# denyingmxd/CFPNet

Measured on AMD Instinct MI355X. Metric: depth maps/sec @ 480x640 bf16 (whole job; per_gpu = value / n_gpus); abs_rel vs CPU oracle, higher is better.
Workload: dtype bf16; 1 GPU; batch=8 480x640 RGB + 8x8-zone ToF, eval forward incl. the prob output [B,256,H/2,W/2] written in the storage dtype (bf16: 2 bytes/element); layers=hist2image combine1 image x2 (CFPNet), parallelism=single GPU

## Files before the change

cfpnet_amd/csrc/attention.hip:

```cpp
#include "common.h"

namespace {

struct KvP {
  const void* k; const void* v;
  float* kv; float* ksum; float* ws;
  int k_ld, v_ld;
  int NB, Hk, Wk, th, tw, gy, gx;
  int cy0, cy1, cx0, cx1;
  int count_pad, heads, d, nsplit;
  float inv_len;
  const int* rec;
};

template <int D> struct KvCfg;
template <> struct KvCfg<4>  { static constexpr int IC = 1; };
template <> struct KvCfg<8>  { static constexpr int IC = 2; };
template <> struct KvCfg<16> { static constexpr int IC = 2; };
template <> struct KvCfg<32> { static constexpr int IC = 2; };

template <typename T, int D, bool DEV>
__global__ __launch_bounds__(64) void kv_reduce_kernel(KvP p) {
  constexpr int IC = KvCfg<D>::IC;
  constexpr int TPK = D / IC;
  constexpr int KL = 64 / TPK;
  const T* __restrict__ K = reinterpret_cast<const T*>(p.k);
  const T* __restrict__ V = reinterpret_cast<const T*>(p.v);
  const int g = blockIdx.x, h = blockIdx.y, sp = blockIdx.z;
  const int lane = threadIdx.x;
  const int ip = lane % TPK, kl = lane / TPK;

  const int gpb = p.gy * p.gx;
  const int b = g / gpb, gi = g % gpb;
  const int ty = gi / p.gx, tx = gi % p.gx;
  int cy0 = p.cy0, cy1 = p.cy1, cx0 = p.cx0, cx1 = p.cx1;
  float inv_len = p.inv_len;
  if constexpr (DEV) {
    const int* __restrict__ rec = p.rec;
    cy0 = rec[4]; cy1 = rec[5]; cx0 = rec[6]; cx1 = rec[7];
    inv_len = 1.0f / (float)max(rec[8], 1);
  }
  const int y0 = max(max(ty * p.th, cy0), 0), y1 = min(min((ty + 1) * p.th, cy1), p.Hk);
  const int x0 = max(max(tx * p.tw, cx0), 0), x1 = min(min((tx + 1) * p.tw, cx1), p.Wk);
  const int rh = max(y1 - y0, 0), rw = max(x1 - x0, 0);
  const int S = rh * rw;
  const int per = (S + p.nsplit - 1) / p.nsplit;
  const int s_begin = sp * per, s_end = min(S, s_begin + per);

  float acc[IC][D];
  float ks[IC];
#pragma unroll
  for (int i = 0; i < IC; ++i) {
    ks[i] = 0.f;
#pragma unroll
    for (int j = 0; j < D; ++j) acc[i][j] = 0.f;
  }
  constexpr int KU = 4;
  const int rwd = max(rw, 1);
  const int step_q = KL / rwd, step_r = KL - step_q * rwd;
  const int s_first = min(s_begin + kl, max(s_end - 1, 0));
  int cy = s_first / rwd, cx = s_first - cy * rwd;
  const int ly = max(s_end - 1, 0) / rwd, lx = max(s_end - 1, 0) - ly * rwd;
  for (int s0 = s_begin + kl; s0 < s_end; s0 += KL * KU) {
    float kf[KU][IC], vf[KU][D];
#pragma unroll
    for (int u = 0; u < KU; ++u) {
      const bool in = s0 + u * KL < s_end;
      const int yy = y0 + (in ? cy : ly), xx = x0 + (in ? cx : lx);
      cx += step_r; cy += step_q;
      if (cx >= rwd) { cx -= rwd; ++cy; }
      const long long row = ((long long)b * p.Hk + yy) * p.Wk + xx;
      const T* kp = K + row * p.k_ld + h * D + ip * IC;
      const T* vp = V + row * p.v_ld + h * D;
#pragma unroll
      for (int i = 0; i < IC; ++i) kf[u][i] = to_f32<T>(kp[i]);
#pragma unroll
      for (int j = 0; j < D; ++j) vf[u][j] = to_f32<T>(vp[j]);
    }
#pragma unroll
    for (int u = 0; u < KU; ++u) {
      if (s0 + u * KL >= s_end) continue;
#pragma unroll
      for (int j = 0; j < D; ++j) vf[u][j] *= inv_len;
#pragma unroll
      for (int i = 0; i < IC; ++i) {
        const float kk = elu1(kf[u][i]);
        ks[i] += kk;
#pragma unroll
        for (int j = 0; j < D; ++j) acc[i][j] = fmaf(kk, vf[u][j], acc[i][j]);
      }
    }
  }
#pragma unroll
  for (int o = TPK; o < 64; o <<= 1) {
#pragma unroll
    for (int i = 0; i < IC; ++i) {
      ks[i] += __shfl_xor(ks[i], o, 64);
#pragma unroll
      for (int j = 0; j < D; ++j) acc[i][j] += __shfl_xor(acc[i][j], o, 64);
    }
  }
  if (kl == 0) {
    float padk = 0.f;
    if (p.count_pad && sp == 0) padk = (float)(p.th * p.tw - S);
    float* dkv; float* dks;
    if (p.nsplit == 1) {
      dkv = p.kv + ((long long)g * p.heads + h) * D * D;
      dks = p.ksum + ((long long)g * p.heads + h) * D;
    } else {
      float* base = p.ws + (((long long)g * p.heads + h) * p.nsplit + sp) * (D * D + D);
      dkv = base; dks = base + D * D;
    }
#pragma unroll
    for (int i = 0; i < IC; ++i) {
      dks[ip * IC + i] = ks[i] + padk;
#pragma unroll
      for (int j = 0; j < D; ++j) dkv[(ip * IC + i) * D + j] = acc[i][j];
    }
  }
}

__global__ __launch_bounds__(256) void kv_finalize_kernel(const float* __restrict__ ws, float* __restrict__ kv,
                                                          float* __restrict__ ksum, int nsplit, int d, long long items) {
  const int per = d * d + d;
  for (long long i = (long long)blockIdx.x * 256 + threadIdx.x; i < items * per; i += (long long)gridDim.x * 256) {
    const long long gh = (long long)((unsigned long long)i / (unsigned)per);
    const int e = (int)(i - gh * per);
    const float* base = ws + gh * nsplit * per + e;
    float s = 0.f;
    int j = 0;
    for (; j + 7 < nsplit; j += 8) {
      float t[8];
#pragma unroll
      for (int u = 0; u < 8; ++u) t[u] = base[(long long)(j + u) * per];
#pragma unroll
      for (int u = 0; u < 8; ++u) s += t[u];
    }
    for (; j < nsplit; ++j) s += base[(long long)j * per];
    if (e < d * d) kv[gh * d * d + e] = s; else ksum[gh * d + (e - d * d)] = s;
  }
}

struct ApP {
  const void* q; const float* kv; const float* ksum; void* out;
  int q_ld, out_ld, NB, Hq, Wq, qth, qtw, ggy, ggx;
  int ey0, ey1, ex0, ex1, heads;
  float v_length, eps;
  FastDiv fheads, fwq, fhq, fqth, fqtw;
  const int* rec;
};

template <typename T, int D, int JS, bool DEV>
__global__ __launch_bounds__(256) void attn_apply_kernel(ApP p) {
  constexpr int DJ = D / JS;
  const T* __restrict__ Q = reinterpret_cast<const T*>(p.q);
  T* __restrict__ O = reinterpret_cast<T*>(p.out);
  int ey0 = p.ey0, ey1 = p.ey1, ex0 = p.ex0, ex1 = p.ex1;
  float v_length = p.v_length;
  if constexpr (DEV) {
    const int* __restrict__ rec = p.rec;
    ey0 = rec[4]; ey1 = rec[5]; ex0 = rec[6]; ex1 = rec[7];
    v_length = (float)max(rec[8], 1);
  }
  const unsigned total = (unsigned)p.NB * p.Hq * p.Wq * p.heads * JS;
  for (unsigned i0 = blockIdx.x * 256u + threadIdx.x; i0 < total; i0 += gridDim.x * 256u) {
    const unsigned i = i0 / JS;
    const int js = (int)(i0 - i * JS);
    unsigned toku, hu, tu, xu, bu, yu;
    fd_rowcol(i, p.fheads, toku, hu);
    fd_rowcol(toku, p.fwq, tu, xu);
    fd_rowcol(tu, p.fhq, bu, yu);
    const int h = (int)hu, x = (int)xu, y = (int)yu, b = (int)bu;
    const long long tok = toku;
    T* op = O + tok * p.out_ld + h * D + js * DJ;
    float o[DJ];
    if (y >= ey0 && y < ey1 && x >= ex0 && x < ex1) {
#pragma unroll
      for (int j = 0; j < DJ; ++j) o[j] = 0.f;
    } else {
      const long long g = ((long long)b * p.ggy + fd_div((unsigned)y, p.fqth)) * p.ggx + fd_div((unsigned)x, p.fqtw);
      const float* kv = p.kv + (g * p.heads + h) * D * D + js * DJ;
      const float* ks = p.ksum + (g * p.heads + h) * D;
      const T* qp = Q + tok * p.q_ld + h * D;
      float z = 0.f;
#pragma unroll
      for (int j = 0; j < DJ; ++j) o[j] = 0.f;
#pragma unroll
      for (int ii = 0; ii < D; ++ii) {
        const float qv = elu1(to_f32<T>(qp[ii]));
        z = fmaf(qv, ks[ii], z);
#pragma unroll
        for (int j = 0; j < DJ; ++j) o[j] = fmaf(qv, kv[ii * D + j], o[j]);
      }
      const float zi = 1.f / (z + p.eps);
#pragma unroll
      for (int j = 0; j < DJ; ++j) o[j] = o[j] * zi * v_length;
    }
#pragma unroll
    for (int j = 0; j < DJ; ++j) op[j] = from_f32<T>(o[j]);
  }
}

int g_ap_split_below = 65536;
int g_kv_target_waves = 2048;
int pick_nsplit(int S, long long groups_heads) {
  long long want = (g_kv_target_waves + groups_heads - 1) / groups_heads;
  int by_keys = (S + 63) / 64;
  long long n = want < by_keys ? want : by_keys;
  if (n < 1) n = 1;
  if (n > 64) n = 64;
  return (int)n;
}

}

void cfp_attn_debug_set(int value) { g_kv_target_waves = value; }
void cfp_attn_apply_debug_set(int value) { g_ap_split_below = value; }

extern "C" size_t cfp_attn_kv_ws_floats(int NB, int Hk, int Wk, int th, int tw, int heads, int d) {
  if (NB <= 0 || Hk <= 0 || Wk <= 0 || th <= 0 || tw <= 0 || heads <= 0 || d <= 0) return 0;
  long long groups = (long long)NB * cdiv(Hk, th) * cdiv(Wk, tw);
  int S = (th < Hk ? th : Hk) * (tw < Wk ? tw : Wk);
  int ns = pick_nsplit(S, groups * heads);
  return (size_t)(groups * heads * ns * (d * d + d));
}

static int kv_reduce_impl(const void* k, int k_ld, const void* v, int v_ld, float* kv, float* ksum, float* ws,
                          int NB, int Hk, int Wk, int th, int tw, int cy0, int cy1, int cx0, int cx1,
                          int count_pad, float v_length, const int* rec, int heads, int d, int dtype, cfp_stream_t stream, const char* who) {
  CFP_REQUIRE(dtype_ok(dtype), CFP_EINVAL, std::string(who) + ": bad dtype");
  CFP_REQUIRE(k && v && kv && ksum, CFP_EINVAL, std::string(who) + ": null pointer");
  CFP_REQUIRE(NB > 0 && Hk > 0 && Wk > 0 && th > 0 && tw > 0 && heads > 0 && (d == 4 || d == 8 || d == 16 || d == 32) &&
                  k_ld >= heads * d && v_ld >= heads * d && v_length > 0.f,
              CFP_ESHAPE, std::string(who) + ": bad shape (head dim must be 4, 8, 16 or 32)");
  KvP p;
  p.rec = rec;
  p.k = k; p.v = v; p.kv = kv; p.ksum = ksum; p.ws = ws; p.k_ld = k_ld; p.v_ld = v_ld;
  p.NB = NB; p.Hk = Hk; p.Wk = Wk; p.th = th; p.tw = tw; p.gy = cdiv(Hk, th); p.gx = cdiv(Wk, tw);
  p.cy0 = cy0; p.cy1 = cy1; p.cx0 = cx0; p.cx1 = cx1; p.count_pad = count_pad; p.heads = heads; p.d = d;
  p.inv_len = 1.0f / v_length;
  long long groups = (long long)NB * p.gy * p.gx;
  int S = (th < Hk ? th : Hk) * (tw < Wk ? tw : Wk);
  p.nsplit = pick_nsplit(S, groups * heads);
  CFP_REQUIRE(p.nsplit == 1 || ws, CFP_EINVAL, std::string(who) + ": workspace required");
  CFP_REQUIRE(groups < (1ll << 31) && heads <= 65535, CFP_ESHAPE, std::string(who) + ": grid too large");
  hipStream_t s = reinterpret_cast<hipStream_t>(stream);
  dim3 grid((unsigned)groups, heads, p.nsplit);
#define KV_LAUNCH(T, D) do { if (rec) hipLaunchKernelGGL((kv_reduce_kernel<T, D, true>), grid, dim3(64), 0, s, p); \
                             else hipLaunchKernelGGL((kv_reduce_kernel<T, D, false>), grid, dim3(64), 0, s, p); } while (0)
#define KV_SWITCH(T) switch (d) { case 4: KV_LAUNCH(T, 4); break; case 8: KV_LAUNCH(T, 8); break; \
                                  case 16: KV_LAUNCH(T, 16); break; default: KV_LAUNCH(T, 32); break; }
  if (dtype == CFP_BF16) { KV_SWITCH(bf16_t) } else if (dtype == CFP_F16) { KV_SWITCH(f16_t) } else { KV_SWITCH(float) }
#undef KV_SWITCH
#undef KV_LAUNCH
  if (p.nsplit > 1) {
    long long items = groups * heads;
    long long total = items * (d * d + d);
    int blocks = (int)((total + 255) / 256 > 4096 ? 4096 : (total + 255) / 256);
    hipLaunchKernelGGL(kv_finalize_kernel, dim3(blocks), dim3(256), 0, s, ws, kv, ksum, p.nsplit, d, items);
  }
  return cfp_check_launch(who);
}

extern "C" int cfp_attn_kv_reduce(const void* k, int k_ld, const void* v, int v_ld, float* kv, float* ksum, float* ws,
                                  int NB, int Hk, int Wk, int th, int tw, int cy0, int cy1, int cx0, int cx1,
                                  int count_pad, float v_length, int heads, int d, int dtype, cfp_stream_t stream) {
  return kv_reduce_impl(k, k_ld, v, v_ld, kv, ksum, ws, NB, Hk, Wk, th, tw, cy0, cy1, cx0, cx1, count_pad, v_length, nullptr, heads, d, dtype,
                        stream, "cfp_attn_kv_reduce");
}

extern "C" int cfp_attn_kv_reduce_dev(const void* k, int k_ld, const void* v, int v_ld, float* kv, float* ksum, float* ws,
                                      int NB, int Hk, int Wk, int th, int tw, const int* rec, int count_pad, int heads, int d, int dtype,
                                      cfp_stream_t stream) {
  CFP_REQUIRE(rec && (reinterpret_cast<uintptr_t>(rec) & 3) == 0, CFP_EINVAL, "cfp_attn_kv_reduce_dev: bad record pointer");
  return kv_reduce_impl(k, k_ld, v, v_ld, kv, ksum, ws, NB, Hk, Wk, th, tw, 0, 0, 0, 0, count_pad, 1.f, rec, heads, d, dtype, stream,
                        "cfp_attn_kv_reduce_dev");
}

static int attn_apply_impl(const void* q, int q_ld, const float* kv, const float* ksum, void* out, int out_ld,
                           int NB, int Hq, int Wq, int qth, int qtw, int ey0, int ey1, int ex0, int ex1,
                           float v_length, const int* rec, float eps, int heads, int d, int dtype, cfp_stream_t stream, const char* who) {
  CFP_REQUIRE(dtype_ok(dtype), CFP_EINVAL, std::string(who) + ": bad dtype");
  CFP_REQUIRE(q && kv && ksum && out, CFP_EINVAL, std::string(who) + ": null pointer");
  CFP_REQUIRE(NB > 0 && Hq > 0 && Wq > 0 && qth > 0 && qtw > 0 && heads > 0 && (d == 4 || d == 8 || d == 16 || d == 32) &&
                  q_ld >= heads * d && out_ld >= heads * d, CFP_ESHAPE, std::string(who) + ": bad shape");
  ApP p;
  p.rec = rec;
  p.q = q; p.kv = kv; p.ksum = ksum; p.out = out; p.q_ld = q_ld; p.out_ld = out_ld;
  p.NB = NB; p.Hq = Hq; p.Wq = Wq; p.qth = qth; p.qtw = qtw; p.ggy = cdiv(Hq, qth); p.ggx = cdiv(Wq, qtw);
  p.ey0 = ey0; p.ey1 = ey1; p.ex0 = ex0; p.ex1 = ex1; p.heads = heads; p.v_length = v_length; p.eps = eps;
  long long total = (long long)NB * Hq * Wq * heads;
  CFP_REQUIRE(total < (1ll << 31), CFP_ESHAPE, std::string(who) + ": too many (token, head) pairs");
  p.fheads = make_fastdiv((unsigned)heads); p.fwq = make_fastdiv((unsigned)Wq); p.fhq = make_fastdiv((unsigned)Hq);
  p.fqth = make_fastdiv((unsigned)qth); p.fqtw = make_fastdiv((unsigned)qtw);
  const int js = total < g_ap_split_below ? (d >= 32 ? 8 : d >= 16 ? 4 : d >= 8 ? 2 : 1) : 1;
  CFP_REQUIRE(total * js < (1ll << 31), CFP_ESHAPE, std::string(who) + ": too many lanes");
  const long long lanes = total * js;
  int blocks = (int)((lanes + 255) / 256 > 8192 ? 8192 : (lanes + 255) / 256);
  hipStream_t s = reinterpret_cast<hipStream_t>(stream);
#define AP_LAUNCH(T, D, JS) do { if (rec) hipLaunchKernelGGL((attn_apply_kernel<T, D, JS, true>), dim3(blocks), dim3(256), 0, s, p); \
                                 else hipLaunchKernelGGL((attn_apply_kernel<T, D, JS, false>), dim3(blocks), dim3(256), 0, s, p); } while (0)
#define AP_SWITCH(T) switch (d) { case 4: AP_LAUNCH(T, 4, 1); break; \
                                  case 8: if (js > 1) AP_LAUNCH(T, 8, 2); else AP_LAUNCH(T, 8, 1); break; \
                                  case 16: if (js > 1) AP_LAUNCH(T, 16, 4); else AP_LAUNCH(T, 16, 1); break; \
                                  default: if (js > 1) AP_LAUNCH(T, 32, 8); else AP_LAUNCH(T, 32, 1); break; }
  if (dtype == CFP_BF16) { AP_SWITCH(bf16_t) } else if (dtype == CFP_F16) { AP_SWITCH(f16_t) } else { AP_SWITCH(float) }
#undef AP_SWITCH
#undef AP_LAUNCH
  return cfp_check_launch(who);
}

extern "C" int cfp_attn_apply(const void* q, int q_ld, const float* kv, const float* ksum, void* out, int out_ld,
                              int NB, int Hq, int Wq, int qth, int qtw, int ey0, int ey1, int ex0, int ex1,
                              float v_length, float eps, int heads, int d, int dtype, cfp_stream_t stream) {
  return attn_apply_impl(q, q_ld, kv, ksum, out, out_ld, NB, Hq, Wq, qth, qtw, ey0, ey1, ex0, ex1, v_length, nullptr, eps, heads, d, dtype,
                         stream, "cfp_attn_apply");
}

extern "C" int cfp_attn_apply_dev(const void* q, int q_ld, const float* kv, const float* ksum, void* out, int out_ld,
                                  int NB, int Hq, int Wq, int qth, int qtw, const int* rec, float eps, int heads, int d, int dtype,
                                  cfp_stream_t stream) {
  CFP_REQUIRE(rec && (reinterpret_cast<uintptr_t>(rec) & 3) == 0, CFP_EINVAL, "cfp_attn_apply_dev: bad record pointer");
  return attn_apply_impl(q, q_ld, kv, ksum, out, out_ld, NB, Hq, Wq, qth, qtw, 0, 0, 0, 0, 1.f, rec, eps, heads, d, dtype, stream,
                         "cfp_attn_apply_dev");
}
```

cfpnet_amd/csrc/loftr_tail.hip:

```cpp
#include "tail_core.h"

namespace {

template <typename H, int NT, int BSTAGE, int WAVES, typename AF>
__device__ __forceinline__ void tail_gemm(f32x4 (&acc)[NT], const H* __restrict__ W, int K, AF afrag, unsigned char* sB,
                                          int wave, int lane) {
  constexpr int N = NT * 16;
  constexpr int NBG = N / 8;
  constexpr int NBW = (NBG + WAVES - 1) / WAVES;
  constexpr int SST = N * 128;
  constexpr int STG = (3 * SST <= 2 * BSTAGE) ? 3 : 2;
  const int fr = lane & 15, fq = lane >> 4;
  const int rsub = lane >> 3;
  const int lc = (lane & 7) ^ rsub;
  const H* zsrc = reinterpret_cast<const H*>(g_zero16);
#pragma unroll
  for (int j = 0; j < NT; ++j) acc[j] = f32x4{0.f, 0.f, 0.f, 0.f};
  const int nk = (K + 63) >> 6;
  auto issue = [&](int ks, int st) {
    const int kk = ks * 64 + lc * 8;
    const bool kok = kk < K;
#pragma unroll
    for (int j = 0; j < NBW; ++j) {
      const int g = (j * WAVES + wave) % NBG;
      const int n = g * 8 + rsub;
      glds16(kok ? W + (long long)n * K + kk : zsrc, sB + st * SST + g * 1024);
    }
  };
  tail_ring_begin<STG, NBW>(nk, issue);
  for (int ks = 0; ks < nk; ++ks) {
    const unsigned char* cB = sB + tail_ring_step<STG, NBW>(ks, nk, issue) * SST;
#pragma unroll
    for (int sub = 0; sub < 2; ++sub) {
      const int k = ks * 64 + sub * 32;
      if (k < K) {
        const s16x8 a = afrag(k);
#pragma unroll
        for (int j = 0; j < NT; ++j) {
          const s16x8 b = *reinterpret_cast<const s16x8*>(cB + (j * 16 + fr) * 128 + (((sub * 4 + fq) ^ (fr & 7)) * 16));
          acc[j] = mfma16<H>(a, b, acc[j]);
        }
      }
    }
  }
}

template <typename H, int D, int HEADS, int WAVES>
__global__ __launch_bounds__(64 * WAVES) void loftr_tail_kernel(TailP<H, H> p) {
  constexpr int PA = D + 8, PH = 2 * D + 8;
  constexpr int WAVE_LDS = (2 * PA + PH) * 16 * 2;
  constexpr int BSTAGE = 2 * D * 128;
  extern __shared__ __attribute__((aligned(16))) unsigned char smem[];
  const int tid = threadIdx.x;
  const int lane = tid & 63;
  const int wave = __builtin_amdgcn_readfirstlane(tid >> 6);
  const int fr = lane & 15, fq = lane >> 4;
  unsigned char* sB = smem;
  H* tMsg = reinterpret_cast<H*>(smem + 2 * BSTAGE + wave * WAVE_LDS);
  H* tX = tMsg + 16 * PA;
  H* tH = tX + 16 * PA;
  const long long row0 = (long long)blockIdx.x * (16 * WAVES) + wave * 16;

  tail_tile_load<H, D, PA>(tX, p.x, p.x_ld, row0, p.rows, lane);

  const bool own_q = p.wq != nullptr;
  if (own_q) {
    asm volatile("s_waitcnt lgkmcnt(0)" ::: "memory");
    f32x4 acc[D / 16];
    tail_gemm<H, D / 16, BSTAGE, WAVES>(acc, p.wq, D, [&](int k) { return *reinterpret_cast<const s16x8*>(tX + fr * PA + k + fq * 8); }, sB, wave, lane);
#pragma unroll
    for (int j = 0; j < D / 16; ++j)
#pragma unroll
      for (int r = 0; r < 4; ++r) tH[(fq * 4 + r) * PH + j * 16 + fr] = from_f32<H>(acc[j][r]);
    asm volatile("s_waitcnt lgkmcnt(0)" ::: "memory");
  }

  tail_attn_apply<H, D, HEADS, PA, PH>(p, row0, tH, tMsg, fr, fq);
  asm volatile("s_waitcnt lgkmcnt(0)" ::: "memory");

  {
    f32x4 acc[D / 16];
    tail_gemm<H, D / 16, BSTAGE, WAVES>(acc, p.wm, D, [&](int k) { return *reinterpret_cast<const s16x8*>(tMsg + fr * PA + k + fq * 8); }, sB, wave, lane);
    tail_layernorm<D / 16, H>(acc, p.g1, p.b1, p.ln_eps, fr);
#pragma unroll
    for (int j = 0; j < D / 16; ++j)
#pragma unroll
      for (int r = 0; r < 4; ++r) tMsg[(fq * 4 + r) * PA + j * 16 + fr] = from_f32<H>(acc[j][r]);
  }
  asm volatile("s_waitcnt lgkmcnt(0)" ::: "memory");

  {
    f32x4 acc[2 * D / 16];
    tail_gemm<H, 2 * D / 16, BSTAGE, WAVES>(acc, p.w0, 2 * D, [&](int k) {
      const H* src = k < D ? tX + fr * PA + k : tMsg + fr * PA + (k - D);
      return *reinterpret_cast<const s16x8*>(src + fq * 8);
    }, sB, wave, lane);
#pragma unroll
    for (int j = 0; j < 2 * D / 16; ++j)
#pragma unroll
      for (int r = 0; r < 4; ++r) tH[(fq * 4 + r) * PH + j * 16 + fr] = from_f32<H>(fmaxf(acc[j][r], 0.f));
  }
  asm volatile("s_waitcnt lgkmcnt(0)" ::: "memory");

  {
    f32x4 acc[D / 16];
    tail_gemm<H, D / 16, BSTAGE, WAVES>(acc, p.w2, 2 * D, [&](int k) { return *reinterpret_cast<const s16x8*>(tH + fr * PH + k + fq * 8); }, sB, wave, lane);
    tail_layernorm<D / 16, H>(acc, p.g2, p.b2, p.ln_eps, fr);
#pragma unroll
    for (int j = 0; j < D / 16; ++j)
#pragma unroll
      for (int r = 0; r < 4; ++r) {
        const int row = fq * 4 + r, col = j * 16 + fr;
        tMsg[row * PA + col] = from_f32<H>(acc[j][r] + to_f32<H>(tX[row * PA + col]));
      }
  }
  asm volatile("s_waitcnt lgkmcnt(0)" ::: "memory");
  tail_tile_store<H, D, PA>(p.out, p.out_ld, tMsg, row0, p.rows, lane);
}

template <typename H, int D>
__global__ __launch_bounds__(256) void lkpm_tail_kernel(LkpmP<H, H> p) {
  constexpr int PA = D + 8, PH = 4 * D + 8;
  constexpr int WAVE_LDS = (PA + PH) * 16 * 2;
  constexpr int BSTAGE = 2 * D * 128;
  extern __shared__ __attribute__((aligned(16))) unsigned char smem[];
  const int tid = threadIdx.x;
  const int lane = tid & 63;
  const int wave = __builtin_amdgcn_readfirstlane(tid >> 6);
  const int fr = lane & 15, fq = lane >> 4;
  unsigned char* sB = smem;
  H* tA = reinterpret_cast<H*>(smem + 2 * BSTAGE + wave * WAVE_LDS);
  H* tH = tA + 16 * PA;
  const long long row0 = (long long)blockIdx.x * 64 + wave * 16;
  constexpr int XCH = D / 8;

  tail_tile_load<H, D, PA>(tA, p.t, p.t_ld, row0, p.rows, lane);
  asm volatile("s_waitcnt lgkmcnt(0)" ::: "memory");
  tail_row_layernorm<H, D, PA>(tA, p.lg, p.lb, p.ln_eps, fr, fq);
  asm volatile("s_waitcnt lgkmcnt(0)" ::: "memory");

#pragma unroll
  for (int half = 0; half < 2; ++half) {
    f32x4 acc[2 * D / 16];
    tail_gemm<H, 2 * D / 16, BSTAGE, 4>(acc, p.w1 + (long long)half * 2 * D * D, D,
                                     [&](int k) { return *reinterpret_cast<const s16x8*>(tA + fr * PA + k + fq * 8); }, sB, wave, lane);
#pragma unroll
    for (int j = 0; j < 2 * D / 16; ++j) {
      const float bj = p.b1[half * 2 * D + j * 16 + fr];
#pragma unroll
      for (int r = 0; r < 4; ++r)
        tH[(fq * 4 + r) * PH + half * 2 * D + j * 16 + fr] = from_f32<H>(act_c16<CFP_ACT_GELU>(acc[j][r] + bj));
    }
  }
  asm volatile("s_waitcnt lgkmcnt(0)" ::: "memory");

  constexpr int PF = D + 4;
  float* tF = reinterpret_cast<float*>(tH);
  {
    f32x4 acc[D / 16];
    tail_gemm<H, D / 16, BSTAGE, 4>(acc, p.w2, 4 * D, [&](int k) { return *reinterpret_cast<const s16x8*>(tH + fr * PH + k + fq * 8); }, sB, wave, lane);
    asm volatile("s_waitcnt lgkmcnt(0)" ::: "memory");
#pragma unroll
    for (int j = 0; j < D / 16; ++j) {
      const float bj = p.b2[j * 16 + fr];
#pragma unroll
      for (int r = 0; r < 4; ++r) tF[(fq * 4 + r) * PF + j * 16 + fr] = acc[j][r] + bj;
    }
  }
  asm volatile("s_waitcnt lgkmcnt(0)" ::: "memory");
  for (int i = lane; i < 16 * XCH; i += 64) {
    const int r = i / XCH, ch = i - r * XCH;
    const long long m = row0 + r;
    if (m < p.rows) {
      float a[8], b[8];
      Vec<float>::load(tF + r * PF + ch * 8, a);
      Vec<float>::load(tF + r * PF + ch * 8 + 4, a + 4);
      Vec<H>::load(p.xin + m * p.x_ld + ch * 8, b);
#pragma unroll
      for (int e = 0; e < 8; ++e) a[e] += b[e];
      Vec<H>::store(p.out + m * p.out_ld + ch * 8, a);
    }
  }
}

int g_tail16_waves = 0;

}

void cfp_tail16_debug_set(int value) { g_tail16_waves = value; }

extern "C" int cfp_loftr_tail(const void* q, int q_ld, const float* kv, const float* ksum, const void* x, int x_ld,
                              void* out, int out_ld, const void* w_q, const void* w_merge, const void* w_mlp0, const void* w_mlp2,
                              const float* ln1_g, const float* ln1_b, const float* ln2_g, const float* ln2_b, float ln_eps,
                              int NB, int Hq, int Wq, int qth, int qtw, float v_length, float eps, int heads, int D,
                              int dtype, cfp_stream_t stream) {
  const bool x3 = dtype == CFP_F32X3;
  const int vec = x3 ? 4 : 8;
  const bool rows_ok = (long long)NB * Hq * Wq < (1ll << 31);
  CFP_REQUIRE(x3 || is16(dtype), CFP_EINVAL, "cfp_loftr_tail: bf16 / f16 or CFP_F32X3 (the plain f32 parity mode uses the unfused kernels)");
  CFP_REQUIRE((q || w_q) && kv && ksum && x && out && w_merge && w_mlp0 && w_mlp2 && ln1_g && ln1_b && ln2_g && ln2_b, CFP_EINVAL,
              "cfp_loftr_tail: null pointer (q or w_q must be given)");
  CFP_REQUIRE(NB > 0 && Hq > 0 && Wq > 0 && qth > 0 && qtw > 0 && v_length > 0.f && (rows_ok || !x3), CFP_ESHAPE, "cfp_loftr_tail: bad grid");
  CFP_REQUIRE((D == 32 || D == 64 || D == 128) && (heads == 4 || heads == 8), CFP_ESHAPE, "cfp_loftr_tail: D must be 32/64/128 and heads 4/8");
  CFP_REQUIRE((w_q || (q_ld >= D && q_ld % vec == 0)) && x_ld >= D && out_ld >= D && x_ld % vec == 0 && out_ld % vec == 0, CFP_ESHAPE,
              "cfp_loftr_tail: pitches must be >= D and multiples of " + std::to_string(vec));
  CFP_REQUIRE(aligned16(q) && aligned16(w_q) && aligned16(x) && aligned16(out) && aligned16(w_merge) && aligned16(w_mlp0) && aligned16(w_mlp2) &&
                  aligned16(kv), CFP_EINVAL, "cfp_loftr_tail: pointers must be 16-byte aligned");
  CFP_REQUIRE(rows_ok, CFP_ESHAPE, "cfp_loftr_tail: too many rows");
  hipStream_t s = reinterpret_cast<hipStream_t>(stream);
  auto params = [&](auto t, auto w) {
    return tail_params<decltype(t), decltype(w)>(q, q_ld, kv, ksum, x, x_ld, out, out_ld, w_q, w_merge, w_mlp0, w_mlp2, ln1_g, ln1_b, ln2_g, ln2_b,
                                                 ln_eps, NB, Hq, Wq, qth, qtw, v_length, eps);
  };
  auto run = [&](auto tag) {
    using H = decltype(tag);
    const TailP<H, H> p = params(tag, tag);
    return tail_pick<32, 64, 128>(D, [&](auto d) { return tail_pick<4, 8>(heads, [&](auto h) {
      return tail_pick<1, 2, 4>(tail_waves(p.rows, g_tail16_waves), [&](auto w) {
        constexpr int D_ = d, W_ = w;
        constexpr size_t lds = 2 * (2 * D_ * 128) + W_ * ((2 * (D_ + 8) + 2 * D_ + 8) * 16 * 2);
        return tail_launch<loftr_tail_kernel<H, D_, h, W_>, lds>(p, W_, s);
      }); }); });
  };
  const int rc = x3 ? loftr_tail_x3_launch(params(float{}, f16_t{}), heads, D, s) : dtype == CFP_F16 ? run(f16_t{}) : run(bf16_t{});
  CFP_REQUIRE(rc == 0, CFP_EHIP, x3 ? "cfp_loftr_tail: f16x3 launch failed" : "cfp_loftr_tail: launch failed");
  return cfp_check_launch("cfp_loftr_tail");
}

extern "C" int cfp_lkpm_tail(const void* t, int t_ld, const void* xin, int x_ld, void* out, int out_ld, const void* w1, const float* b1,
                             const void* w2, const float* b2, const float* ln_g, const float* ln_b, float ln_eps, int rows, int D, int dtype,
                             cfp_stream_t stream) {
  const bool x3 = dtype == CFP_F32X3;
  const int vec = x3 ? 4 : 8;
  CFP_REQUIRE(x3 || is16(dtype), CFP_EINVAL, "cfp_lkpm_tail: bf16 / f16 or CFP_F32X3 (the plain f32 parity mode uses the unfused kernels)");
  CFP_REQUIRE(t && xin && out && w1 && b1 && w2 && b2 && ln_g && ln_b, CFP_EINVAL, "cfp_lkpm_tail: null pointer");
  CFP_REQUIRE(rows > 0 && (D == 32 || D == 64 || D == 128), CFP_ESHAPE, "cfp_lkpm_tail: D must be 32/64/128");
  CFP_REQUIRE(t_ld >= D && x_ld >= D && out_ld >= D && t_ld % vec == 0 && x_ld % vec == 0 && out_ld % vec == 0, CFP_ESHAPE,
              "cfp_lkpm_tail: pitches must be >= D and multiples of " + std::to_string(vec));
  CFP_REQUIRE(aligned16(t) && aligned16(xin) && aligned16(out) && aligned16(w1) && aligned16(w2), CFP_EINVAL, "cfp_lkpm_tail: pointers must be 16-byte aligned");
  hipStream_t s = reinterpret_cast<hipStream_t>(stream);
  auto params = [&](auto tt, auto w) {
    return lkpm_params<decltype(tt), decltype(w)>(t, t_ld, xin, x_ld, out, out_ld, w1, b1, w2, b2, ln_g, ln_b, ln_eps, rows);
  };
  auto run = [&](auto tag) {
    using H = decltype(tag);
    const LkpmP<H, H> p = params(tag, tag);
    return tail_pick<32, 64, 128>(D, [&](auto d) {
      constexpr int D_ = d;
      constexpr size_t lds = 2 * (2 * D_ * 128) + 4 * (((D_ + 8) + (4 * D_ + 8)) * 16 * 2);
      return tail_launch<lkpm_tail_kernel<H, D_>, lds>(p, 4, s);
    });
  };
  const int rc = x3 ? lkpm_tail_x3_launch(params(float{}, f16_t{}), D, s) : dtype == CFP_F16 ? run(f16_t{}) : run(bf16_t{});
  CFP_REQUIRE(rc == 0, CFP_EHIP, x3 ? "cfp_lkpm_tail: f16x3 launch failed" : "cfp_lkpm_tail: launch failed");
  return cfp_check_launch("cfp_lkpm_tail");
}
```

cfpnet_amd/csrc/tail_core.h:

```cpp
#pragma once
#include <type_traits>

#include "lds_dma.h"

template <int NST, int NBW, typename ISSUE>
__device__ __forceinline__ void tail_ring_begin(int n, ISSUE issue) {
  static_assert(NST == 2 || NST == 3, "wait ladder in tail_ring_step");
  asm volatile("s_waitcnt lgkmcnt(0)" ::: "memory");
  __builtin_amdgcn_s_barrier();
  asm volatile("" ::: "memory");
  issue(0, 0);
  if (NST > 2 && n > 1) issue(1, 1);
}
template <int NST, int NBW, typename ISSUE>
__device__ __forceinline__ int tail_ring_step(int i, int n, ISSUE issue) {
  constexpr int AHEAD = NST - 1;
  if (AHEAD > 1 && i + 1 < n) asm volatile("s_waitcnt vmcnt(%0)" ::"n"(NBW) : "memory");
  else asm volatile("s_waitcnt vmcnt(0)" ::: "memory");
  asm volatile("s_waitcnt lgkmcnt(0)" ::: "memory");
  __builtin_amdgcn_s_barrier();
  asm volatile("" ::: "memory");
  if (i + AHEAD < n) issue(i + AHEAD, (i + AHEAD) % NST);
  return i % NST;
}

template <int NT, typename ROUND_T>
__device__ __forceinline__ void tail_layernorm(f32x4 (&acc)[NT], const float* __restrict__ gamma, const float* __restrict__ beta, float eps, int fr) {
  constexpr float inv_n = 1.f / (float)(NT * 16);
  float g[NT], bt[NT];
#pragma unroll
  for (int j = 0; j < NT; ++j) { g[j] = gamma[j * 16 + fr]; bt[j] = beta[j * 16 + fr]; }
#pragma unroll
  for (int r = 0; r < 4; ++r) {
    float s = 0.f;
#pragma unroll
    for (int j = 0; j < NT; ++j) {
      if constexpr (!std::is_same<ROUND_T, float>::value) acc[j][r] = to_f32<ROUND_T>(from_f32<ROUND_T>(acc[j][r]));
      s += acc[j][r];
    }
    s = row16_sum(s);
    const float mean = s * inv_n;
    float qq = 0.f;
#pragma unroll
    for (int j = 0; j < NT; ++j) { const float dlt = acc[j][r] - mean; qq = fmaf(dlt, dlt, qq); }
    qq = row16_sum(qq);
    const float rstd = rsqrtf(qq * inv_n + eps);
#pragma unroll
    for (int j = 0; j < NT; ++j) acc[j][r] = (acc[j][r] - mean) * rstd * g[j] + bt[j];
  }
}

template <typename T, int D, int PA>
__device__ __forceinline__ void tail_tile_load(T* tile, const T* src, int ld, long long row0, int rows, int lane) {
  constexpr int E = 16 / sizeof(T), XCH = D / E;
  for (int i = lane; i < 16 * XCH; i += 64) {
    const int r = i / XCH, ch = i - r * XCH;
    const long long m = row0 + r;
    u32x4 v = {0u, 0u, 0u, 0u};
    if (m < rows) v = *reinterpret_cast<const u32x4*>(src + m * ld + ch * E);
    *reinterpret_cast<u32x4*>(tile + r * PA + ch * E) = v;
  }
}
template <typename T, int D, int PA>
__device__ __forceinline__ void tail_tile_store(T* dst, int ld, const T* tile, long long row0, int rows, int lane) {
  constexpr int E = 16 / sizeof(T), XCH = D / E;
  for (int i = lane; i < 16 * XCH; i += 64) {
    const int r = i / XCH, ch = i - r * XCH;
    const long long m = row0 + r;
    if (m < rows) *reinterpret_cast<u32x4*>(dst + m * ld + ch * E) = *reinterpret_cast<const u32x4*>(tile + r * PA + ch * E);
  }
}

template <typename T, int D, int PA>
__device__ __forceinline__ void tail_row_layernorm(T* tile, const float* gamma, const float* beta, float eps, int fr, int fq) {
  constexpr int Q = D / 4, E = Vec<T>::N;
  T* row = tile + fr * PA + fq * Q;
  float v[Q];
#pragma unroll
  for (int c = 0; c < Q; c += E) Vec<T>::load(row + c, v + c);
  float s = 0.f;
#pragma unroll
  for (int c = 0; c < Q; ++c) s += v[c];
  s += __shfl_xor(s, 16, 64); s += __shfl_xor(s, 32, 64);
  const float mean = s * (1.f / (float)D);
  float qq = 0.f;
#pragma unroll
  for (int c = 0; c < Q; ++c) { const float dl = v[c] - mean; qq = fmaf(dl, dl, qq); }
  qq += __shfl_xor(qq, 16, 64); qq += __shfl_xor(qq, 32, 64);
  const float rstd = rsqrtf(qq * (1.f / (float)D) + eps);
#pragma unroll
  for (int c = 0; c < Q; c += E) {
    float o[E];
#pragma unroll
    for (int e = 0; e < E; ++e) o[e] = (v[c + e] - mean) * rstd * gamma[fq * Q + c + e] + beta[fq * Q + c + e];
    Vec<T>::store(row + c, o);
  }
}

template <typename T, typename W> struct TailP {
  const T* q; const float* kv; const float* ksum; const T* x; T* out;
  const W* wq;
  const W* wm; const W* w0; const W* w2;
  const float* g1; const float* b1; const float* g2; const float* b2;
  int q_ld, x_ld, out_ld;
  int rows, Hq, Wq, qth, qtw, ggy, ggx;
  FastDiv fwq, fhq, fqth, fqtw;
  float v_length, eps, ln_eps;
};
template <typename T, typename W> struct LkpmP {
  const T* t; const T* xin; T* out;
  const W* w1; const W* w2;
  const float* lg; const float* lb; const float* b1; const float* b2;
  int t_ld, x_ld, out_ld, rows;
  float ln_eps;
};

template <typename T, int N, bool LDS>
__device__ __forceinline__ void tail_load_f32(const T* src, float* v) {
  constexpr int E = Vec<T>::N;
  if constexpr (N >= E) {
#pragma unroll
    for (int c = 0; c < N; c += E) {
      if constexpr (LDS) {
        const u32x4 raw = *(const __attribute__((address_space(3))) u32x4*)(src + c);
        Vec<T>::load(reinterpret_cast<const T*>(&raw), v + c);
      } else {
        Vec<T>::load(src + c, v + c);
      }
    }
  } else {
#pragma unroll
    for (int c = 0; c < N; ++c) v[c] = to_f32<T>(LDS ? *(const __attribute__((address_space(3))) T*)(src + c) : src[c]);
  }
}

template <typename T, int D, int HEADS, int PA, int PQ, typename W>
__device__ __forceinline__ void tail_attn_apply(const TailP<T, W>& p, long long row0, const T* tq, T* tMsg, int fr, int fq) {
  constexpr int d = D / HEADS;
  const bool own_q = p.wq != nullptr;
  const int r = fr;
  const long long m = row0 + r;
  const bool ok = m < p.rows;
  const long long mm = ok ? m : 0;
  const unsigned t = fd_div((unsigned)mm, p.fwq), xq = (unsigned)mm - t * (unsigned)p.Wq;
  const unsigned b = fd_div(t, p.fhq), yq = t - b * (unsigned)p.Hq;
  const long long g = ((long long)b * p.ggy + fd_div(yq, p.fqth)) * p.ggx + fd_div(xq, p.fqtw);
#pragma unroll
  for (int hs = 0; hs < HEADS / 4; ++hs) {
    const int h = fq + 4 * hs;
    const float* __restrict__ kv = p.kv + (g * HEADS + h) * d * d;
    const float* __restrict__ ks = p.ksum + (g * HEADS + h) * d;
    float qv[d];
    if (own_q) tail_load_f32<T, d, true>(tq + r * PQ + h * d, qv);
    else tail_load_f32<T, d, false>(p.q + mm * p.q_ld + h * d, qv);
    float o[d];
#pragma unroll
    for (int j = 0; j < d; ++j) o[j] = 0.f;
    float z = 0.f;
#pragma unroll
    for (int i = 0; i < d; ++i) {
      const float qe = elu1(qv[i]);
      z = fmaf(qe, ks[i], z);
#pragma unroll
      for (int j = 0; j < d; j += 4) {
        const f32x4 kk = *reinterpret_cast<const f32x4*>(kv + i * d + j);
        o[j] = fmaf(qe, kk[0], o[j]); o[j + 1] = fmaf(qe, kk[1], o[j + 1]);
        o[j + 2] = fmaf(qe, kk[2], o[j + 2]); o[j + 3] = fmaf(qe, kk[3], o[j + 3]);
      }
    }
    const float zi = 1.f / (z + p.eps);
#pragma unroll
    for (int j = 0; j < d; ++j) {
      const T v = from_f32<T>(o[j] * zi * p.v_length);
      tMsg[r * PA + h * d + j] = ok ? v : T(0);
    }
  }
}

template <typename T, typename W>
TailP<T, W> tail_params(const void* q, int q_ld, const float* kv, const float* ksum, const void* x, int x_ld, void* out, int out_ld, const void* w_q,
                        const void* w_merge, const void* w_mlp0, const void* w_mlp2, const float* ln1_g, const float* ln1_b, const float* ln2_g,
                        const float* ln2_b, float ln_eps, int NB, int Hq, int Wq, int qth, int qtw, float v_length, float eps) {
  TailP<T, W> p;
  p.q = (const T*)q; p.kv = kv; p.ksum = ksum; p.x = (const T*)x; p.out = (T*)out;
  p.wq = (const W*)w_q; p.wm = (const W*)w_merge; p.w0 = (const W*)w_mlp0; p.w2 = (const W*)w_mlp2;
  p.g1 = ln1_g; p.b1 = ln1_b; p.g2 = ln2_g; p.b2 = ln2_b;
  p.q_ld = q_ld; p.x_ld = x_ld; p.out_ld = out_ld;
  p.rows = NB * Hq * Wq; p.Hq = Hq; p.Wq = Wq; p.qth = qth; p.qtw = qtw; p.ggy = cdiv(Hq, qth); p.ggx = cdiv(Wq, qtw);
  p.fwq = make_fastdiv((unsigned)Wq); p.fhq = make_fastdiv((unsigned)Hq); p.fqth = make_fastdiv((unsigned)qth); p.fqtw = make_fastdiv((unsigned)qtw);
  p.v_length = v_length; p.eps = eps; p.ln_eps = ln_eps;
  return p;
}
template <typename T, typename W>
LkpmP<T, W> lkpm_params(const void* t, int t_ld, const void* xin, int x_ld, void* out, int out_ld, const void* w1, const float* b1, const void* w2,
                        const float* b2, const float* ln_g, const float* ln_b, float ln_eps, int rows) {
  LkpmP<T, W> p;
  p.t = (const T*)t; p.xin = (const T*)xin; p.out = (T*)out; p.w1 = (const W*)w1; p.w2 = (const W*)w2;
  p.lg = ln_g; p.lb = ln_b; p.b1 = b1; p.b2 = b2; p.t_ld = t_ld; p.x_ld = x_ld; p.out_ld = out_ld; p.rows = rows; p.ln_eps = ln_eps;
  return p;
}

inline int tail_waves(long long rows, int forced) {
  if (forced == 1 || forced == 2 || forced == 4) return forced;
  return rows <= 4800 ? 1 : rows < 8192 ? 2 : 4;
}

template <int... V, typename F>
int tail_pick(int v, F f) {
  int rc = -2;
  ((v == V ? (void)(rc = f(std::integral_constant<int, V>{})) : (void)0), ...);
  return rc;
}

template <auto KERNEL, size_t LDS, typename P>
int tail_launch(const P& p, int waves, hipStream_t s) {
  static_assert(LDS <= 160 * 1024, "LDS budget");
  static bool attr = false;
  if (!attr) { if (hipFuncSetAttribute((const void*)KERNEL, hipFuncAttributeMaxDynamicSharedMemorySize, 160 * 1024) != hipSuccess) return -1; attr = true; }
  hipLaunchKernelGGL(KERNEL, dim3((unsigned)cdiv(p.rows, 16 * waves)), dim3(64 * waves), LDS, s, p);
  return 0;
}

int loftr_tail_x3_launch(const TailP<float, f16_t>& p, int heads, int D, hipStream_t s);
int lkpm_tail_x3_launch(const LkpmP<float, f16_t>& p, int D, hipStream_t s);
```

cfpnet_amd/engine.py:

```python
from __future__ import annotations

import math
import os
from typing import Dict, List, Optional, Sequence, Tuple

import torch

from . import hip, ops, spec
from .geometry import FUSION_SCALES, FusionGeometry, gsa_keys, static_zone_key, zone_records as _zone_records
from .ops import Act

_BN_EPS = 1e-5


def _same_pad(size: int, k: int, s: int) -> Tuple[int, int]:
    total = max((math.ceil(size / s) - 1) * s + k - size, 0)
    return total // 2, total - total // 2


_STREAMS: Dict = {}
_CONCURRENT: Dict[str, list] = {}


def concurrent_streams(device, want: int = 4, pool: int = 16) -> list:
    import time
    key = str(torch.device(device))
    got = _CONCURRENT.get(key)
    if got is not None and len(got) >= want:
        return got[:want]
    cand = [torch.cuda.Stream(device=device) for _ in range(pool)]
    cycles = 1_000_000
    if not hasattr(torch.cuda, "_sleep"):
        _CONCURRENT[key] = cand[:max(want, 4)]
        return _CONCURRENT[key][:want]

    def spin(ids):
        torch.cuda.synchronize(device)
        t0 = time.perf_counter()
        for i in ids:
            with torch.cuda.stream(cand[i]):
                torch.cuda._sleep(cycles)
        torch.cuda.synchronize(device)
        return time.perf_counter() - t0

    spin([0])
    base = min(spin([0]) for _ in range(3))
    chosen = [0]
    for j in range(1, pool):
        if len(chosen) >= want:
            break
        if all(min(spin([k, j]) for _ in range(2)) < 1.5 * base for k in chosen):
            chosen.append(j)
    _CONCURRENT[key] = [cand[i] for i in chosen]
    return _CONCURRENT[key][:want]


def _shared_stream(device, role):
    key = (str(torch.device(device)), role)
    st = _STREAMS.get(key)
    if st is None:
        if isinstance(role, tuple) and role[0] == "lane":
            conc = concurrent_streams(device)
            st = conc[role[1] % len(conc)]
        else:
            st = torch.cuda.Stream(device=device)
        _STREAMS[key] = st
    return st


class Engine:
    def __init__(self, state_dict: Dict[str, torch.Tensor], *, layer_names: Sequence[str], n_bins: int = 256,
                 min_val: float = 1e-3, max_val: float = 10.0, norm: str = "linear", change_embedding: bool = True,
                 no_skip_inside: bool = False, stem_act: bool = False, dtype=None, device="cuda:0",
                 zone_sample_num: int = 16, base_resolution=spec.BASE_RESOLUTION, x3: Optional[bool] = None):
        if dtype is None:
            dtype, x3 = torch.float32, (True if x3 is None else x3)
        x3 = bool(x3)
        hip.load()
        self.base_resolution = tuple(base_resolution)
        self.fusion = spec.fusion_table(self.base_resolution)
        if not torch.cuda.is_available():
            raise RuntimeError("cfpnet_amd.Engine needs a GPU: the product path has no CPU fallback")
        assert dtype in (torch.bfloat16, torch.float16, torch.float32)
        self.layer_names = list(layer_names)
        self.n_bins, self.min_val, self.max_val = n_bins, float(min_val), float(max_val)
        self.norm = {"linear": 0, "softmax": 1, "sigmoid": 2}[norm]
        self.change_embedding, self.no_skip_inside, self.stem_act = change_embedding, no_skip_inside, stem_act
        self.dtype, self.device = dtype, torch.device(device)
        assert not x3 or dtype == torch.float32, "x3 is a matrix-math mode of float32 storage"
        self.x3 = bool(x3)
        self.cdt = hip.F32X3 if self.x3 else ops.DT[dtype]
        self.tickets = self.x3 and os.environ.get("CFP_SPLITK_TICKETS", "0") == "1"
        self.zone_sample_num = zone_sample_num
        self.weights2 = os.environ.get("CFP_WEIGHTS2", "0") == "1"
        self.diffuse_cin = os.environ.get("CFP_DIFFUSE_CIN", "1") == "1"
        self.mbconv_fused = os.environ.get("CFP_MBCONV_FUSED", "0") == "1"
        self.se2 = dtype in (torch.bfloat16, torch.float16) and os.environ.get("CFP_SE2", "1") == "1"
        self.se2_x3 = os.environ.get("CFP_SE2_X3", "1") if self.x3 else "0"
        self._dbg_round = {}
        for item in filter(None, os.environ.get("CFP_DEBUG_ROUND", "").split(",")):
            n, d = item.split(":")
            self._dbg_round[n] = {"f16": torch.float16, "bf16": torch.bfloat16}[d]
        self.up_fused = os.environ.get("CFP_UP_FUSED", "4")
        self.up_fused_x3 = os.environ.get("CFP_UP_FUSED_X3", "")
        self.cat_pad = os.environ.get("CFP_CAT_PAD", "1") == "1" and not self.up_fused_x3
        self.lkpm_fused = os.environ.get("CFP_LKPM_FUSED", "1") != "0"
        self.tail_q = os.environ.get("CFP_TAIL_Q", "1") == "1"
        self.lkpm_min_rows = int(os.environ.get("CFP_LKPM_MIN_ROWS", "30000"))
        self.sr_ln_fused = os.environ.get("CFP_SR_LN_FUSED", "1") == "1"
        self.head_fused = os.environ.get("CFP_HEAD_FUSED", "1") != "0"
        self.head_conv0 = os.environ.get("CFP_HEAD_CONV0", "1") != "0"
        self.er_fused = os.environ.get("CFP_ER_FUSED", "12")
        hl = os.environ.get("CFP_HEAD_HILO", "00")
        self.head_hilo = (hl[0] == "1", hl[1] == "1")
        self.half = dtype in (torch.bfloat16, torch.float16)
        self.ve = 8 if self.half else 4
        self.P: Dict[str, torch.Tensor] = {}
        self._plans: Dict[tuple, dict] = {}
        self._graph = None
        self._splitk_ws: Optional[torch.Tensor] = None
        self._capturing = False
        self._side = _shared_stream(self.device, "side")
        self._lane = 0
        self.use_side_stream = os.environ.get("CFP_NO_SIDE_STREAM", "0") != "1"
        self._lane_streams: Dict[int, Tuple[torch.cuda.Stream, torch.cuda.Stream]] = {}
        self._lanes_active = 1
        self._slots = None
        self._slot_next = 0
        self._lane_ws: Dict[int, torch.Tensor] = {}
        self.load_state_dict(state_dict)

    def _dev(self, t: torch.Tensor, dtype=None) -> torch.Tensor:
        return t.detach().to(device=self.device, dtype=dtype or torch.float32).contiguous()

    def _pack_conv(self, w: torch.Tensor, w2: bool = False) -> torch.Tensor:
        w = w.detach().float()
        if w.dim() == 2:
            w = w[:, :, None, None]
        elif w.dim() == 3:
            w = w[:, :, :, None]
        co, ci, kh, kw = w.shape
        if kh * kw > 1:
            w = ops.round_taps(w, self.dtype)
        cip = (ci + 7) // 8 * 8
        if cip != ci:
            w = torch.nn.functional.pad(w, (0, 0, 0, 0, 0, cip - ci))
        flat = w.permute(0, 2, 3, 1).reshape(co, kh * kw * cip)
        if w2 and self.weights2 and self.half and kh * kw == 1:
            return ops.pack_w2(flat, self.dtype).to(self.device)
        if kh * kw == 1 and self.diffuse_cin and self.dtype == torch.float16:
            flat = ops.round_taps(flat.reshape(co, 1, kh * kw * cip), self.dtype).reshape(co, -1)
        if self.x3:
            return ops.pack_w_x3(self._dev(flat))
        return self._dev(flat, self.dtype)

    def _fold_bn(self, sd, bn: Optional[str], bias: Optional[torch.Tensor], co: int, eps: float):
        if bn is None:
            scale = torch.ones(co)
            shift = bias.detach().float().clone() if bias is not None else torch.zeros(co)
        else:
            g, b = sd[bn + ".weight"].float(), sd[bn + ".bias"].float()
            m, v = sd[bn + ".running_mean"].float(), sd[bn + ".running_var"].float()
            scale = g / torch.sqrt(v + eps)
            shift = b - m * scale
            if bias is not None:
                shift = shift + bias.detach().float() * scale
        return self._dev(scale), self._dev(shift)

    def _conv(self, sd, name: str, wkey: str, bkey: Optional[str] = None, bn: Optional[str] = None, eps: float = _BN_EPS, w2: bool = True):
        w = sd[wkey]
        self.P[name + ".w"] = self._pack_conv(w, w2)
        s, t = self._fold_bn(sd, bn, sd[bkey] if bkey else None, w.shape[0], eps)
        self.P[name + ".s"], self.P[name + ".t"] = s, t

    def _loftr_pack(self, sd, p: str, self_attn: bool):
        D = sd[p + ".q_proj.weight"].shape[0]
        if self_attn:
            self.P[p + ".qkv"] = self._pack_conv(torch.cat([sd[p + ".q_proj.weight"], sd[p + ".k_proj.weight"], sd[p + ".v_proj.weight"]], 0), True)
        else:
            self.P[p + ".q"] = self._pack_conv(sd[p + ".q_proj.weight"], True)
        self.P[p + ".kv"] = self._pack_conv(torch.cat([sd[p + ".k_proj.weight"], sd[p + ".v_proj.weight"]], 0), True)
        self.P[p + ".q1"] = self._pack_conv(sd[p + ".q_proj.weight"])
        self.P[p + ".merge"] = self._pack_conv(sd[p + ".merge.weight"])
        self.P[p + ".mlp0"] = self._pack_conv(sd[p + ".mlp.0.weight"])
        self.P[p + ".mlp2"] = self._pack_conv(sd[p + ".mlp.2.weight"])
        for n in ("norm1", "norm2"):
            self.P[f"{p}.{n}.g"], self.P[f"{p}.{n}.b"] = self._dev(sd[f"{p}.{n}.weight"]), self._dev(sd[f"{p}.{n}.bias"])

    def load_state_dict(self, sd: Dict[str, torch.Tensor]):
        self.P.clear()
        self._graph = None
        e = "img_encoder"
        EPS = spec.ENC_BN_EPS
        self._conv(sd, "stem", f"{e}.conv0.0.weight", bn=f"{e}.conv0.1", eps=EPS)
        self.rgb_hilo = self.half and os.environ.get("CFP_RGB_HILO", "1") == "1"
        if self.rgb_hilo:
            w = self.P["stem.w"].reshape(-1, 9, 8).clone()
            w[:, :, 3:6] = w[:, :, 0:3]
            self.P["stem.w"] = w.reshape(w.shape[0], 72).contiguous()
        for b in spec.ENC_BLOCKS:
            q = f"{e}.{b.prefix}"
            if b.kind == "cn":
                self._conv(sd, q + ".conv", q + ".conv.weight", bn=q + ".bn1", eps=EPS)
            elif b.kind == "er":
                self._conv(sd, q + ".exp", q + ".conv_exp.weight", bn=q + ".bn1", eps=EPS)
                self._conv(sd, q + ".pwl", q + ".conv_pwl.weight", bn=q + ".bn2", eps=EPS)
                if self.half and not self.weights2:
                    self.P[q + ".pwl.wp"] = ops.pad_pw_w(self.P[q + ".pwl.w"])
            else:
                self._conv(sd, q + ".pw", q + ".conv_pw.weight", bn=q + ".bn1", eps=EPS)
                if self.half and self.mbconv_fused and b.stride == 1 and not self.weights2:
                    self.P[q + ".pw.wimg"] = ops.pack_mbconv_pw(self.P[q + ".pw.w"].float().cpu(), self.dtype).to(self.device)
                wd = ops.round_taps(sd[q + ".conv_dw.weight"].float(), self.dtype)
                self.P[q + ".dw.w"] = self._dev(wd.reshape(wd.shape[0], 9).t(), self.dtype)
                self.P[q + ".dw.s"], self.P[q + ".dw.t"] = self._fold_bn(sd, q + ".bn2", None, wd.shape[0], EPS)
                self.P[q + ".se.wr"] = self._dev(sd[q + ".se.conv_reduce.weight"].reshape(b.se_rd, b.mid))
                self.P[q + ".se.br"] = self._dev(sd[q + ".se.conv_reduce.bias"])
                self.P[q + ".se.we_t"] = self._dev(sd[q + ".se.conv_expand.weight"].reshape(b.mid, b.se_rd).t())
                self.P[q + ".se.be"] = self._dev(sd[q + ".se.conv_expand.bias"])
                self._conv(sd, q + ".pwl", q + ".conv_pwl.weight", bn=q + ".bn3", eps=EPS, w2=False)
                self.P[q + ".pwl.w32"] = self._dev(sd[q + ".conv_pwl.weight"].reshape(b.cout, b.mid))
        parts, layout, off = [], [], 0
        for ex in (1, 2, 3):
            q = f"hist_encoder.hist_extractor{ex}.pointnet_encoder"
            for j in (1, 2, 3):
                w = sd[f"{q}.conv{j}.weight"].detach().float()
                w = w.reshape(w.shape[0], -1)
                co, ci = w.shape
                sc, sh = self._fold_bn(sd, f"{q}.bn{j}", sd[f"{q}.conv{j}.bias"], co, _BN_EPS)
                row = []
                for t in (w.reshape(-1), sc.cpu(), sh.cpu()):
                    row.append(off)
                    parts.append(t.reshape(-1).cpu())
                    off += (t.numel() + 3) // 4 * 4
                    if t.numel() % 4:
                        parts.append(torch.zeros(4 - t.numel() % 4))
                layout.append((row[0], row[1], row[2], ci, co))
        self.P["hist.blob"] = self._dev(torch.cat(parts))
        self._hist_layout = layout
        d = "decoder"
        self._conv(sd, d + ".conv4", d + ".conv4.weight", d + ".conv4.bias")
        for i in (1, 2, 3, 4):
            q = f"{d}.up{i}._net"
            if self.x3 and self.cat_pad:
                wfull = sd[q + ".0.weight"]
                cpad = (wfull.shape[1] + 31) // 32 * 32
                self.P[f"{d}.up{i}.a.wpad"] = self._pack_conv(torch.nn.functional.pad(wfull.detach().float(), (0, 0, 0, 0, 0, cpad - wfull.shape[1])))
            self._conv(sd, f"{d}.up{i}.a", q + ".0.weight", q + ".0.bias", bn=q + ".1")
            if self.x3 and str(i) in self.up_fused_x3:
                wfull = sd[q + ".0.weight"].detach().float()
                cup = wfull.shape[1] - spec.DEC_ENC_CH[i]
                self.P[f"{d}.up{i}.a.wcat"] = ops.pack_w_x3_cat(self._dev(wfull.permute(0, 2, 3, 1).contiguous()), cup)
            self._conv(sd, f"{d}.up{i}.b", q + ".3.weight", q + ".3.bias", bn=q + ".4")
        for n in ("conv3", "conv2", "conv1", "conv0"):
            self._conv(sd, f"{d}.{n}", f"{d}.{n}.weight", f"{d}.{n}.bias")
        if self.half and not self.weights2:
            self.P[d + ".conv1.wp"] = ops.pad_pw_w(self.P[d + ".conv1.w"])
        for name in self.fusion:
            q = f"{d}.{name}"
            self.P[q + ".pe"] = self._dev(sd[q + ".positional_encodings"])
# ... 50 lines not shown
    def _buf(self, plan, key: str, shape, dtype, zero: bool = False) -> torch.Tensor:
        bufs = plan["bufs"]
        if key not in bufs:
            bufs[key] = (torch.zeros if zero else torch.empty)(shape, dtype=dtype, device=self.device)
        assert tuple(bufs[key].shape) == tuple(shape), key
        return bufs[key]

    def _f32(self, plan, key: str, n: int) -> torch.Tensor:
        bufs = plan["bufs"]
        if key not in bufs:
            bufs[key] = torch.empty(max(n, 1), dtype=torch.float32, device=self.device)
        assert bufs[key].numel() >= n, key
        return bufs[key]

    def _cv(self, name, x: Act, out: Act, B, H, W, k, stride=1, pads=None, act=hip.ACT_NONE, residual=None):
        if pads is None:
            p = (k - 1) // 2
            pt = pl = p
            Ho, Wo = (H + 2 * p - k) // stride + 1, (W + 2 * p - k) // stride + 1
        else:
            (pt, pb), (pl, pr) = pads
            Ho, Wo = (H + pt + pb - k) // stride + 1, (W + pl + pr - k) // stride + 1
        ops.conv2d(x, self.P[name + ".w"], self.P[name + ".s"], self.P[name + ".t"], out, B, H, W, k, k, stride, pt, pl,
                   Ho, Wo, act, residual, self._ws(B * Ho * Wo, out.C, k * k * x.C))
        return Ho, Wo

    def _lin(self, wname, x: Act, out: Act, rows, act=hip.ACT_NONE, residual=None, st: Optional[str] = None, ln=None):
        ops.linear(x, self.P[wname], self.P[st + ".s"] if st else None, self.P[st + ".t"] if st else None, out, rows, act, residual,
                   None if ln is not None else self._ws(rows, out.C, x.C), ln)

    def _ws(self, M: int, Cout: int, K: int) -> Optional[torch.Tensor]:
        need = ops.conv2d_ws_bytes(M, Cout, K, self.cdt)
        if need == 0:
            return None
        if self.tickets:
            need += hip.CONV_TICKET_BYTES
        ws = self._lane_ws.get(self._lane)
        if ws is None or ws.numel() * 4 < need:
            if self._capturing:
                raise RuntimeError("split-K workspace must be sized by a warm-up forward before graph capture")
            if self.tickets:
                ws = ops.ticket_ws(need - hip.CONV_TICKET_BYTES, self.device)
            else:
                ws = torch.empty((need + 3) // 4, dtype=torch.float32, device=self.device)
            self._lane_ws[self._lane] = ws
        return ws

    def _dbg(self, name: str, a: Act):
        if self._dbg_round:
            for pat, dt in self._dbg_round.items():
                if name == pat or (pat.endswith("*") and name.startswith(pat[:-1])):
                    t = a.torch()
                    t.copy_(t.to(dt).to(t.dtype))

    def _encoder(self, plan, rgb: torch.Tensor, B, H, W, taps):
        e = "img_encoder"
        x8 = self._act(plan, "rgb8", B * H * W, 8)
        (ops.rgb_to_nhwc8_hilo if self.rgb_hilo else ops.rgb_to_nhwc8)(rgb, x8, B, H, W)
        pads = (_same_pad(H, 3, 2), _same_pad(W, 3, 2))
        h, w = math.ceil(H / 2), math.ceil(W / 2)
        x = self._act(plan, "stem", B * h * w, spec.ENC_STEM_OUT)
        self._cv("stem", x8, x, B, H, W, 3, 2, pads, hip.ACT_SILU if self.stem_act else hip.ACT_NONE)
        self._dbg("stem", x)
        tap_acts: List[Act] = []
        for bi, b in enumerate(spec.ENC_BLOCKS):
            q = f"{e}.{b.prefix}"
            ho, wo = math.ceil(h / b.stride), math.ceil(w / b.stride)
            pads = (_same_pad(h, 3, b.stride), _same_pad(w, 3, b.stride))
            if bi in spec.ENC_TAPS:
                out = plan["tap_dst"][spec.ENC_TAPS[bi]]
            else:
                out = self._act(plan, f"enc{bi}", B * ho * wo, b.cout)
            res = x if b.skip else None
            if b.kind == "cn":
                self._cv(q + ".conv", x, out, B, h, w, 3, b.stride, pads, hip.ACT_SILU, res)
            elif b.kind == "er":
                if (self.half and (q + ".pwl.wp") in self.P and ("1" if b.stride == 1 else "2") in self.er_fused and taps is None
                        and not self._dbg_round and ops.conv3x3_pw_fused_variant(x.C, b.mid, b.cout, b.stride, ops.DT[self.dtype]) >= 0):
                    ops.conv3x3_pw_fused(x, self.P[q + ".exp.w"], self.P[q + ".exp.s"], self.P[q + ".exp.t"], hip.ACT_SILU, self.P[q + ".pwl.wp"],
                                         self.P[q + ".pwl.s"], self.P[q + ".pwl.t"], out, B, h, w, b.stride, pads[0][0], pads[1][0], ho, wo,
                                         hip.ACT_NONE, res)
                else:
                    mid = self._act(plan, f"enc{bi}.mid", B * ho * wo, b.mid)
                    self._cv(q + ".exp", x, mid, B, h, w, 3, b.stride, pads, hip.ACT_SILU)
                    self._dbg(f"enc{bi}.mid", mid)
                    self._cv(q + ".pwl", mid, out, B, ho, wo, 1, 1, None, hip.ACT_NONE, res)
            else:
                mid2 = self._act(plan, f"enc{bi}.dw", B * ho * wo, b.mid)
                mbp = ops.mbconv_plan(B, h, w, x.C, b.mid) if (q + ".pw.wimg") in self.P else None
                if mbp is not None:
                    ns = mbp[0]
                    part = self._f32(plan, f"enc{bi}.sum", B * ns * b.mid)
                    ops.mbconv_expand_dw(x, self.P[q + ".pw.wimg"], self.P[q + ".pw.s"], self.P[q + ".pw.t"], self.P[q + ".dw.w"],
                                         self.P[q + ".dw.s"], self.P[q + ".dw.t"], mid2, part, B, h, w)
                elif ((self.se2 or self.se2_x3 == "1" or (self.se2_x3 == "auto" and not ops.PLAN_IN_FLIGHT)) and b.se_rd <= 64
                      and ops.dwconv3x3_se_parts(B, ho, wo, b.mid, b.stride, ops.DT[self.dtype]) > 0):
                    mid = self._act(plan, f"enc{bi}.mid", B * h * w, b.mid)
                    self._cv(q + ".pw", x, mid, B, h, w, 1, 1, None, hip.ACT_SILU)
                    K = ops.dwconv3x3_se_parts(B, ho, wo, b.mid, b.stride, ops.DT[self.dtype])
                    hpart = self._f32(plan, f"enc{bi}.hpart", B * K * b.se_rd)
                    ops.dwconv3x3_se(mid, self.P[q + ".dw.w"], self.P[q + ".dw.s"], self.P[q + ".dw.t"], mid2, self.P[q + ".se.wr"], hpart,
                                     B, h, w, b.stride, pads[0][0], pads[1][0], ho, wo, hip.ACT_SILU)
                    if self.x3:
                        wb = self._buf(plan, f"enc{bi}.wb", (B, b.cout, (b.mid + 31) // 32 * 64), torch.float16, zero=True)
                    else:
                        wb = self._buf(plan, f"enc{bi}.wb", (B, b.cout, b.mid), self.dtype)
                    ops.se_gate_fold2(hpart, K, 1.0 / (ho * wo), self.P[q + ".se.br"], self.P[q + ".se.we_t"], self.P[q + ".se.be"],
                                      self.P[q + ".pwl.w32"], wb, B, b.cout, b.mid, b.se_rd, x3=self.x3)
                    ops.conv2d(mid2, wb, self.P[q + ".pwl.s"], self.P[q + ".pwl.t"], out, B, ho, wo, 1, 1, 1, 0, 0, ho, wo, hip.ACT_NONE,
                               res, self._piw_ws(plan, bi, B, ho * wo, b.cout, b.mid), per_image_weights=True)
                    x, h, w = out, ho, wo
                    if bi in spec.ENC_TAPS:
                        tap_acts.append(out)
                        if taps is not None:
                            taps[f"enc{spec.ENC_TAPS[bi]}"] = self._nchw(out, B, h, w)
                    continue
                else:
                    mid = self._act(plan, f"enc{bi}.mid", B * h * w, b.mid)
                    self._cv(q + ".pw", x, mid, B, h, w, 1, 1, None, hip.ACT_SILU)
                    ns = ops.dwconv3x3_strips(B, ho, wo, b.mid, b.stride, ops.DT[self.dtype])
                    part = self._f32(plan, f"enc{bi}.sum", B * ns * b.mid)
                    self._dbg(f"enc{bi}.mid", mid)
                    ops.dwconv3x3_sum(mid, self.P[q + ".dw.w"], self.P[q + ".dw.s"], self.P[q + ".dw.t"], mid2, part, B, h, w, b.stride,
                                      pads[0][0], pads[1][0], ho, wo, hip.ACT_SILU)
                    self._dbg(f"enc{bi}.dw", mid2)
                if self.x3:
                    wb = self._buf(plan, f"enc{bi}.wb", (B, b.cout, (b.mid + 31) // 32 * 64), torch.float16, zero=True)
                else:
                    wb = self._buf(plan, f"enc{bi}.wb", (B, b.cout, b.mid), self.dtype)
                ops.se_gate_fold(part, ns, 1.0 / (ho * wo), self.P[q + ".se.wr"], self.P[q + ".se.br"], self.P[q + ".se.we_t"],
                                 self.P[q + ".se.be"], self.P[q + (".pwl.w32" if self.x3 else ".pwl.w")], wb, B, b.cout, b.mid, b.se_rd)
                ops.conv2d(mid2, wb, self.P[q + ".pwl.s"], self.P[q + ".pwl.t"], out, B, ho, wo, 1, 1, 1, 0, 0, ho, wo, hip.ACT_NONE,
                           res, self._piw_ws(plan, bi, B, ho * wo, b.cout, b.mid), per_image_weights=True)
            self._dbg(f"enc{bi}", out)
            x, h, w = out, ho, wo
            if bi in spec.ENC_TAPS:
                tap_acts.append(out)
                if taps is not None:
                    taps[f"enc{spec.ENC_TAPS[bi]}"] = self._nchw(out, B, h, w)
        return tap_acts

    def _hist_encoder(self, plan, hist: torch.Tensor, R: int, taps):
        outs = [self._act(plan, f"hist.{ex}", R, c) for ex, c in zip((1, 2, 3), spec.HIST_CHANNELS)]
        self._hist_pe_fused = taps is None and os.environ.get("CFP_NO_PE_FUSE", "0") != "1"
        pe = [self.P[f"decoder.cross_atten{ex}.pe2"] for ex in (1, 2, 3)] if self._hist_pe_fused else (None, None, None)
        ops.hist_encoder(hist.reshape(-1), self.P["hist.blob"], self._hist_layout, outs, R, pe, self.zone_sample_num)
        if taps is not None:
            for ex, o in enumerate(outs):
                taps[f"hist{ex}"] = o.torch().float().cpu()
        return outs

    def _kv_state(self, plan, tag, p, src: Act, rows_s, D, heads, kvmode: dict):
        d = D // heads
        kvb = self._act(plan, f"{tag}.kvsrc", rows_s, 2 * D)
        self._lin(p + ".kv", src, kvb, rows_s)
        G = kvmode["groups"]
        kv = self._f32(plan, f"{tag}.kv", G * heads * d * d)
        ks = self._f32(plan, f"{tag}.ks", G * heads * d)
        nws = ops.attn_kv_ws_floats(kvmode["NB"], kvmode["Hk"], kvmode["Wk"], kvmode["th"], kvmode["tw"], heads, d)
        ws = self._f32(plan, f"{tag}.kvws", nws)
        ops.attn_kv_reduce(kvb.slice(0, D), kvb.slice(D, D), kv, ks, ws, kvmode["NB"], kvmode["Hk"], kvmode["Wk"], kvmode["th"], kvmode["tw"],
                           kvmode["clip"], kvmode["count_pad"], kvmode["v_length"], heads, d)
        return kv, ks

    def _loftr(self, plan, tag, p, xb: Act, rows_q, src: Optional[Act], rows_s, heads, out: Act, kvmode: dict, apmode: dict, pre=None):
        D = xb.C // 2
        d = D // heads
        x = xb.slice(0, D)
        qb = self._act(plan, f"{tag}.qkv", rows_q, 3 * D)
        fused_tail = self.half or (self.x3 and os.environ.get("CFP_X3_TAIL", "1") != "0")
        tail_q = fused_tail and self.tail_q
        if pre is not None and tail_q:
            kv, ks = pre
            ops.loftr_tail(None, kv, ks, x, out, self.P[p + ".q1"], self.P[p + ".merge"], self.P[p + ".mlp0"], self.P[p + ".mlp2"],
                           (self.P[p + ".norm1.g"], self.P[p + ".norm1.b"]), (self.P[p + ".norm2.g"], self.P[p + ".norm2.b"]),
                           apmode["NB"], apmode["Hq"], apmode["Wq"], apmode["qth"], apmode["qtw"], kvmode["v_length"], heads)
            return
        if src is None and tail_q:
            self._lin(p + ".kv", x, qb.slice(D, 2 * D), rows_q)
            kA, vA = qb.slice(D, D), qb.slice(2 * D, D)
        elif src is None:
            self._lin(p + ".qkv", x, qb, rows_q)
            kA, vA = qb.slice(D, D), qb.slice(2 * D, D)
        else:
            if not tail_q:
                self._lin(p + ".q", x, qb.slice(0, D), rows_q)
            kvb = self._act(plan, f"{tag}.kvsrc", rows_s, 2 * D)
            self._lin(p + ".kv", src, kvb, rows_s)
            kA, vA = kvb.slice(0, D), kvb.slice(D, D)
        G = kvmode["groups"]
        kv = self._f32(plan, f"{tag}.kv", G * heads * d * d)
        ks = self._f32(plan, f"{tag}.ks", G * heads * d)
        nws = ops.attn_kv_ws_floats(kvmode["NB"], kvmode["Hk"], kvmode["Wk"], kvmode["th"], kvmode["tw"], heads, d)
        ws = self._f32(plan, f"{tag}.kvws", nws)
        ops.attn_kv_reduce(kA, vA, kv, ks, ws, kvmode["NB"], kvmode["Hk"], kvmode["Wk"], kvmode["th"], kvmode["tw"],
                           kvmode["clip"], kvmode["count_pad"], kvmode["v_length"], heads, d)
        if fused_tail:
            ops.loftr_tail(None if tail_q else qb.slice(0, D), kv, ks, x, out, self.P[p + ".q1"] if tail_q else None,
                           self.P[p + ".merge"], self.P[p + ".mlp0"], self.P[p + ".mlp2"],
                           (self.P[p + ".norm1.g"], self.P[p + ".norm1.b"]), (self.P[p + ".norm2.g"], self.P[p + ".norm2.b"]),
                           apmode["NB"], apmode["Hq"], apmode["Wq"], apmode["qth"], apmode["qtw"], kvmode["v_length"], heads)
            return
        msg = self._act(plan, f"{tag}.msg", rows_q, D)
        ops.attn_apply(qb.slice(0, D), kv, ks, msg, apmode["NB"], apmode["Hq"], apmode["Wq"], apmode["qth"], apmode["qtw"],
                       (0, 0, 0, 0), kvmode["v_length"], heads, d)
        self._lin(p + ".merge", msg, xb.slice(D, D), rows_q, ln=(self.P[p + ".norm1.g"], self.P[p + ".norm1.b"], 1e-5))
        hid = self._act(plan, f"{tag}.hid", rows_q, 2 * D)
        self._lin(p + ".mlp0", xb, hid, rows_q, hip.ACT_RELU)
        self._lin(p + ".mlp2", hid, out, rows_q, residual=x, ln=(self.P[p + ".norm2.g"], self.P[p + ".norm2.b"], 1e-5))

    def _piw_ws(self, plan, bi: int, B: int, hw: int, cout: int, k: int):
        if not self.x3:
            return None
        _, sp = ops.conv2d_plan(B * hw, cout, k, hip.F32X3, hw, B, 1, 1)
        if sp <= 1:
            return None
        if not self.tickets:
            return self._f32(plan, f"enc{bi}.piw_ws", sp * B * hw * cout)
        bufs, key = plan["bufs"], f"enc{bi}.piw_ws"
        if key not in bufs:
            bufs[key] = ops.ticket_ws(sp * B * hw * cout * 4, self.device)
        return bufs[key]

    def _fusion(self, plan, name: str, x: Act, feat1: Act, zone_valid: torch.Tensor, geo: FusionGeometry, B, H, W, out: Act,
                pos_offset, taps, rec: Optional[torch.Tensor] = None):
        D, (Hm, Wm), lk = self.fusion[name]
        p = f"decoder.{name}"
        ws = spec.window_size((Hm, Wm))
        M = B * H * W
        Z = geo.zone_num * geo.zone_num
        N = self.zone_sample_num
        tok = [self._act(plan, f"{name}.tokA", M, 2 * D), self._act(plan, f"{name}.tokB", M, 2 * D)]
        cur = 0
        if torch.is_tensor(pos_offset):
            assert pos_offset.dtype == torch.int32 and pos_offset.numel() == 2 and pos_offset.is_cuda
            d0 = tok[0].slice(0, D)
            hip.call("cfp_add_rowtable_dev", x.ptr, x.ld, self.P[p + ".pe"].data_ptr(), d0.ptr, d0.ld, M, x.C, H, W, Hm, Wm,
                     pos_offset.data_ptr(), x.dt, hip.current_stream())
        else:
            oy, ox = pos_offset
            ops.add_rowtable(x, self.P[p + ".pe"], tok[0].slice(0, D), M, H, W, Wm, oy, ox)
        emb0 = None
        if not self.change_embedding:
            emb0 = self._act(plan, f"{name}.emb0", M, D)
            ops.copy_rows(tok[0].slice(0, D), emb0, M)
        if self._hist_pe_fused:
            src = feat1
        else:
            src = self._act(plan, f"{name}.src", B * Z * N, D)
            ops.add_rowtable(feat1, self.P[p + ".pe2"], src, B * Z * N, 1, N, N, 0, 0)
        gh, gw = geo.grid_h, geo.grid_w
        Mz = B * gh * gw
        y0, y1, x0, x1 = geo.clipped(H, W)
        rect = (geo.sy_wo, geo.sx_wo, geo.tzh, geo.tzw)

        last = len(self.layer_names) - 1
        direct_out = False
        for i, ln in enumerate(self.layer_names):
            l = f"{p}.layers.{i}"
            tag = f"{name}.L{i}"
            final_dst = out if (i == last and taps is None and os.environ.get("CFP_NO_DIRECT_OUT", "0") != "1") else None
            if ln == "hist2image":
                zin = self._act(plan, f"{name}.zin", Mz, 2 * D)
                zsrc = tok[cur].slice(0, D) if self.change_embedding else emb0
                if rec is None:
                    ops.resize_bilinear(zsrc, H, W, rect, zin.slice(0, D), gh, gw, (0, 0, gh, gw), B)
                else:
                    ops.resize_bilinear(zsrc, H, W, None, zin.slice(0, D), gh, gw, (0, 0, gh, gw), B, rec=rec, rec_side=0)
                zout = self._act(plan, f"{name}.zout", Mz, D)
                self._loftr(plan, f"{name}.x2i", l, zin, Mz, src, B * Z * N, spec.X2I_HEADS, zout,
                            dict(groups=B * Z, NB=B * Z, Hk=1, Wk=N, th=1, tw=N, clip=(0, 1, 0, N), count_pad=False, v_length=float(N)),
                            dict(NB=B, Hq=gh, Wq=gw, qth=geo.p1, qtw=geo.p2), pre=plan.get("x2i_kv", {}).get((name, i)))
                if rec is None:
                    ops.resize_bilinear(zout, gh, gw, (0, 0, gh, gw), tok[cur].slice(0, D), H, W, rect, B, zone_valid=zone_valid,
                                        zn=geo.zone_num, p1=geo.p1, p2=geo.p2, accumulate=not self.no_skip_inside)
                else:
                    ops.resize_bilinear(zout, gh, gw, (0, 0, gh, gw), tok[cur].slice(0, D), H, W, None, B, zone_valid=zone_valid,
                                        zn=geo.zone_num, p1=geo.p1, p2=geo.p2, accumulate=not self.no_skip_inside, rec=rec, rec_side=1)
            elif ln == "image":
                nh, nw = math.ceil(H / ws), math.ceil(W / ws)
                self._loftr(plan, f"{name}.lsa", l + ".lga.encoder_layer", tok[cur], M, None, 0, spec.TWINS_HEADS, tok[cur ^ 1].slice(0, D),
                            dict(groups=B * nh * nw, NB=B, Hk=H, Wk=W, th=ws, tw=ws, clip=(0, H, 0, W), count_pad=True, v_length=float(ws * ws)),
                            dict(NB=B, Hq=H, Wq=W, qth=ws, qtw=ws))
                cur ^= 1
                hk, wk = gsa_keys(H, W, ws)
                keys = self._act(plan, f"{name}.gsa.keys", B * hk * wk, D)
                if self.x3 and self.sr_ln_fused:
                    ops.conv2d(tok[cur].slice(0, D), self.P[l + ".gsa.sr.w"], self.P[l + ".gsa.sr.s"], self.P[l + ".gsa.sr.t"], keys,
                               B, H, W, ws, ws, ws, 0, 0, hk, wk, ws=self._ws(B * hk * wk, D, ws * ws * D),
                               ln=(self.P[l + ".gsa.norm.g"], self.P[l + ".gsa.norm.b"], 1e-5))
                else:
                    kraw = self._act(plan, f"{name}.gsa.kraw", B * hk * wk, D)
                    ops.conv2d(tok[cur].slice(0, D), self.P[l + ".gsa.sr.w"], self.P[l + ".gsa.sr.s"], self.P[l + ".gsa.sr.t"], kraw,
                               B, H, W, ws, ws, ws, 0, 0, hk, wk, ws=self._ws(B * hk * wk, D, ws * ws * D))
                    ops.layernorm(kraw, self.P[l + ".gsa.norm.g"], self.P[l + ".gsa.norm.b"], 1e-5, keys, B * hk * wk)
                S = hk * wk
                self._loftr(plan, f"{name}.gsa", l + ".gsa.encoder_layer", tok[cur], M, keys, B * S, spec.TWINS_HEADS,
                            final_dst if final_dst is not None else tok[cur ^ 1].slice(0, D),
                            dict(groups=B, NB=B, Hk=1, Wk=S, th=1, tw=S, clip=(0, 1, 0, S), count_pad=False, v_length=float(S)),
                            dict(NB=B, Hq=H, Wq=W, qth=H, qtw=W))
                cur ^= 1
                direct_out = final_dst is not None
            elif ln == "combine1":
                t = l + ".transformer_path"
                heads = spec.X2I_HEADS
                d = D // heads
                xin = tok[cur]
                qb = self._act(plan, f"{name}.dapm.qkv", M, 3 * D)
                self._lin(t + ".qkv", xin.slice(0, D), qb, M)
                n_in = (y1 - y0) * (x1 - x0)
                kv = self._f32(plan, f"{name}.dapm.kv", B * heads * d * d)
                ks = self._f32(plan, f"{name}.dapm.ks", B * heads * d)
                wsb = self._f32(plan, f"{name}.dapm.ws", ops.attn_kv_ws_floats(B, H, W, H, W, heads, d))
                if rec is None:
                    ops.attn_kv_reduce(qb.slice(D, D), qb.slice(2 * D, D), kv, ks, wsb, B, H, W, H, W, (y0, y1, x0, x1), False,
                                       float(max(n_in, 1)), heads, d)
                    ops.attn_apply(qb.slice(0, D), kv, ks, xin.slice(D, D), B, H, W, H, W, (y0, y1, x0, x1), float(max(n_in, 1)), heads, d)
                else:
                    ops.attn_kv_reduce(qb.slice(D, D), qb.slice(2 * D, D), kv, ks, wsb, B, H, W, H, W, None, False, None, heads, d, rec=rec)
                    ops.attn_apply(qb.slice(0, D), kv, ks, xin.slice(D, D), B, H, W, H, W, None, None, heads, d, rec=rec)
                c1 = self._act(plan, f"{name}.dapm.c1", M, D)
                self._cv(t + ".conv1", xin, c1, B, H, W, 3)
                self._cv(t + ".conv2", c1, tok[cur ^ 1].slice(0, D), B, H, W, 3, residual=xin.slice(0, D))
                cur ^= 1
                k = l + ".large_kernel_path"
                xin = tok[cur]
                t1 = self._act(plan, f"{name}.lk.t1", M, D)
                if (k + ".dw.tb") in self.P:
                    ops.dwconv_large_mfma(xin.slice(0, D), self.P[k + ".dw.tb"], self.P[k + ".dw.s"], self.P[k + ".dw.t"], t1, B, H, W, lk,
                                          hip.ACT_RELU)
                else:
                    ops.dwconv_large(xin.slice(0, D), self.P[k + ".dw.w"], self.P[k + ".dw.s"], self.P[k + ".dw.t"], t1, B, H, W, lk, hip.ACT_RELU)
                lk_dst = final_dst if final_dst is not None else tok[cur ^ 1].slice(0, D)
                if ((self.half and not self.weights2) or (self.x3 and os.environ.get("CFP_X3_TAIL", "1") != "0")) and self.lkpm_fused and D in (32, 64, 128) and M >= self.lkpm_min_rows:
                    ops.lkpm_tail(t1, xin.slice(0, D), lk_dst, self.P[k + ".pw1.w"], self.P[k + ".pw1.t"], self.P[k + ".pw2.w"], self.P[k + ".pw2.t"],
                                  self.P[k + ".norm.g"], self.P[k + ".norm.b"], M)
                else:
                    t2 = self._act(plan, f"{name}.lk.t2", M, D)
                    ops.layernorm(t1, self.P[k + ".norm.g"], self.P[k + ".norm.b"], 1e-6, t2, M)
                    h4 = self._act(plan, f"{name}.lk.h4", M, 4 * D)
                    self._lin(k + ".pw1.w", t2, h4, M, hip.ACT_GELU, None, k + ".pw1")
                    self._lin(k + ".pw2.w", h4, lk_dst, M, hip.ACT_NONE, xin.slice(0, D), k + ".pw2")
                cur ^= 1
                direct_out = final_dst is not None
            else:
                raise NotImplementedError(ln)
            if taps is not None:
                taps[f"{p}.layers.{i}"] = tok[cur].slice(0, D).torch().float().cpu().reshape(B, H * W, D)
        if not direct_out:
            ops.copy_rows(tok[cur].slice(0, D), out, M)

    def _nchw(self, a: Act, B, H, W) -> torch.Tensor:
        return a.torch().float().cpu().reshape(B, H, W, a.C).permute(0, 3, 1, 2).contiguous()

    @torch.no_grad()
    def forward_lanes(self, input_data: dict, lanes: int, *, return_prob: bool = True, pos_offsets: Optional[dict] = None,
                      uncertainty: bool = False):
        rgb = input_data["rgb"]
        B = rgb.shape[0]
        lanes = max(1, min(lanes, B))
        if lanes == 1:
            return self.forward(input_data, return_prob=return_prob, pos_offsets=pos_offsets, uncertainty=uncertainty)
        dev = self.device
        add = input_data["additional"]
        H, W = rgb.shape[-2:]
        edges = torch.empty(B, self.n_bins + 1, dtype=torch.float32, device=dev)
        pred = torch.empty(B, 1, H // 2, W // 2, dtype=torch.float32, device=dev)
        prob = torch.empty(B, self.n_bins, H // 2, W // 2, dtype=self.dtype, device=dev) if return_prob else None
        unc = torch.empty(B, 3, H // 2, W // 2, dtype=torch.float32, device=dev) if uncertainty else None
        main = torch.cuda.current_stream(dev)
        bounds = [B * i // lanes for i in range(lanes + 1)]
        for i in range(lanes):
            if i not in self._lane_streams and i > 0:
                self._lane_streams[i] = (_shared_stream(dev, ("lane", i)), _shared_stream(dev, ("lane-side", i)))
        rgb_d = rgb.to(device=dev, dtype=torch.float32).contiguous()
        hist_d = add["hist_data"].to(device=dev, dtype=torch.float32).contiguous()
        mask_d = add["mask"].to(device=dev).to(torch.uint8).contiguous()
        self._lanes_active = lanes
        for i in range(lanes):
            b0, b1 = bounds[i], bounds[i + 1]
            sub = {"rgb": rgb_d[b0:b1], "additional": {"hist_data": hist_d[b0:b1], "mask": mask_d[b0:b1],
                                                       "rect_data": add.get("rect_data"), "patch_info": add["patch_info"]}}
            outs = (edges[b0:b1], pred[b0:b1], prob[b0:b1] if prob is not None else None) + ((unc[b0:b1],) if uncertainty else ())
            if i == 0:
                self.forward(sub, return_prob=return_prob, pos_offsets=pos_offsets, lane=0, out=outs, uncertainty=uncertainty)
            else:
                st = self._lane_streams[i][0]
                st.wait_stream(main)
                with torch.cuda.stream(st):
                    self.forward(sub, return_prob=return_prob, pos_offsets=pos_offsets, lane=i, out=outs, uncertainty=uncertainty)
        for i in range(1, lanes):
            main.wait_stream(self._lane_streams[i][0])
        self._lane = 0
        self._lanes_active = 1
        return (edges, pred, prob, unc) if uncertainty else (edges, pred, prob)

    def capture(self, input_data: dict, *, return_prob: bool = True, pos_offsets: Optional[dict] = None, lanes: int = 1,
                inflight: int = 1, adopt_inputs: bool = False, uncertainty: bool = False, dynamic_zones: bool = False):
        if dynamic_zones and inflight > 1:
            raise ValueError("capture(dynamic_zones=True) with inflight > 1: each in-flight slot would need its own zone record; use inflight=1")
        dev = self.device
        add = input_data["additional"]
        B = input_data["rgb"].shape[0]
        H, W = input_data["rgb"].shape[-2:]
        lanes = max(1, min(lanes, B))
        zones = None
        if dynamic_zones:
            host = _zone_records(add["patch_info"], H, W)
            zones = {"buf": torch.from_numpy(host).to(dev), "host": host.tobytes(), "key": static_zone_key(add["patch_info"]), "hw": (H, W),
                     "seen": {}, "pinned": {}}
        zrec = zones["buf"] if zones else None
        self._slots = None
        self._slot_next = 0
        if inflight > 1:
            return self._capture_inflight(input_data, inflight, return_prob, pos_offsets, uncertainty)
        if adopt_inputs:
            assert lanes == 1, "adopt_inputs: single-graph capture only"
            m = add["mask"]
            for t, dts in ((input_data["rgb"], (torch.float32,)), (add["hist_data"], (torch.float32,)), (m, (torch.uint8, torch.bool))):
                assert t.device == dev and t.dtype in dts and t.is_contiguous(), "adopt_inputs: device tensors in the kernels' own types"
            static = {"rgb": input_data["rgb"], "additional": {"hist_data": add["hist_data"], "mask": m.view(torch.uint8) if m.dtype == torch.bool else m,
                                                               "rect_data": add.get("rect_data"), "patch_info": add["patch_info"]}}
        else:
            static = {"rgb": input_data["rgb"].to(device=dev, dtype=torch.float32).contiguous().clone(),
                      "additional": {"hist_data": add["hist_data"].to(device=dev, dtype=torch.float32).contiguous().clone(),
                                     "mask": add["mask"].to(device=dev).to(torch.uint8).contiguous().clone(),
                                     "rect_data": add.get("rect_data"), "patch_info": add["patch_info"]}}
        edges = torch.empty(B, self.n_bins + 1, dtype=torch.float32, device=dev)
        pred = torch.empty(B, 1, H // 2, W // 2, dtype=torch.float32, device=dev)
        prob = torch.empty(B, self.n_bins, H // 2, W // 2, dtype=self.dtype, device=dev) if return_prob else None
        unc = torch.empty(B, 3, H // 2, W // 2, dtype=torch.float32, device=dev) if uncertainty else None
# ... 386 lines not shown
```

cfpnet_amd/hip.py:

```python
from __future__ import annotations

import ctypes as C
import os
from typing import Optional

_HERE = os.path.dirname(os.path.abspath(__file__))
LIB_PATH = os.environ.get("CFP_HIP_LIB") or os.path.join(_HERE, "libcfpnet_hip.so")

F32, BF16, F16 = 0, 1, 2
F32X3 = 3
ACT_NONE, ACT_RELU, ACT_LRELU, ACT_SILU, ACT_GELU, ACT_SIGMOID = range(6)
TOF_SAMPLE_UNIFORM, TOF_SAMPLE_ICDF = 0, 1
HEAD_WOUT_HILO, HEAD_RAM_HILO = 1, 2
UNC_STD, UNC_ENTROPY, UNC_PMAX = 0, 1, 2
SPARS_STD, SPARS_ENTROPY, SPARS_PMAX, SPARS_ORACLE_RMSE, SPARS_ORACLE_ABSREL = range(5)
RENDER_DEPTH, RENDER_GT, RENDER_ABS_ERR, RENDER_REL_ERR = range(4)
REGION_ALL, REGION_FOV_IN, REGION_FOV_OUT, REGION_ZONE_VALID, REGION_ZONE_INVALID = range(5)
CONV_PER_IMAGE, CONV_W2, CONV_IN_FLIGHT, CONV_X3, CONV_WS_TICKETS = 1, 2, 4, 8, 16
CONV_TICKET_BYTES = 4096

_p, _i, _f, _sz, _ll = C.c_void_p, C.c_int, C.c_float, C.c_size_t, C.c_longlong

SIGNATURES = {
    "cfp_version": (_i, []),
    "cfp_last_error": (C.c_char_p, []),
    "cfp_conv2d_nhwc": (_i, [_p, _i, _p, _p, _p, _p, _i, _p, _i] + [_i] * 14 + [_p, _sz, _p]),
    "cfp_conv2d_nhwc_ex": (_i, [_p, _i, _p, _p, _p, _p, _i, _p, _i] + [_i] * 14 + [_p, _p, _f, _i, _p, _sz, _p]),
    "cfp_conv2d_nhwc_moments": (_i, [_p, _i, _p, _p, _p, _i] + [_i] * 13 + [_p, _sz, _p, _sz, _p, _p, _p]),
    "cfp_conv2d_ws_bytes": (_sz, [_i, _i, _i, _i]),
    "cfp_pack_w_x3_elems": (_sz, [_ll, _i]),
    "cfp_pack_w_x3": (_i, [_p, _p, _ll, _i, _p]),
    "cfp_conv2d_plan": (_i, [_i] * 8 + [_p, _p]),
    "cfp_debug_set": (_i, [_i, _i]),
    "cfp_conv2d_variant": (_i, [_i, _i]),
    "cfp_dwconv3x3_nhwc": (_i, [_p, _i, _p, _p, _p, _p, _i] + [_i] * 11 + [_p]),
    "cfp_dwconv3x3_strips": (_i, [_i] * 6),
    "cfp_dwconv3x3_launch_slots": (_i, [_i] * 10),
    "cfp_dwconv3x3_sum_nhwc": (_i, [_p, _i, _p, _p, _p, _p, _i, _p] + [_i] * 11 + [_p]),
    "cfp_se_fold": (_i, [_p, _p, _p, _p, _p, _i, _i, _i, _i, _i, _p]),
    "cfp_se_gate_fold": (_i, [_p, _i, _f, _p, _p, _p, _p, _p, _p, _i, _i, _i, _i, _i, _p]),
    "cfp_dwconv3x3_se_parts": (_i, [_i, _i, _i, _i, _i, _i]),
    "cfp_dwconv3x3_se_nhwc": (_i, [_p, _i, _p, _p, _p, _p, _i, _p, _i, _p] + [_i] * 11 + [_p]),
    "cfp_se_gate_fold2": (_i, [_p, _i, _f, _p, _p, _p, _p, _p, _i, _i, _i, _i, _i, _p]),
    "cfp_dwconv_large_nhwc": (_i, [_p, _i, _p, _p, _p, _p, _i] + [_i] * 7 + [_p]),
    "cfp_dwconv_large_toeplitz_elems": (_sz, [_i, _i]),
    "cfp_dwconv_large_toeplitz": (_i, [_p, _p, _i, _i, _i, _i, _p]),
    "cfp_dwconv_large_mfma_nhwc": (_i, [_p, _i, _p, _p, _p, _p, _i] + [_i] * 7 + [_p]),
    "cfp_channel_sum": (_i, [_p, _i, _p, _i, _i, _i, _i, _i, _p]),
    "cfp_se_hidden": (_i, [_p, _i, _f, _p, _p, _p, _i, _i, _i, _p]),
    "cfp_se_scale": (_i, [_p, _i, _p, _p, _p, _i, _i, _i, _i, _i, _p]),
    "cfp_scale_channels": (_i, [_p, _i, _p, _i, _i, _i, _i, _p]),
    "cfp_layernorm": (_i, [_p, _i, _p, _p, _f, _p, _i, _p, _i, _i, _i, _i, _p]),
    "cfp_attn_kv_ws_floats": (_sz, [_i] * 7),
    "cfp_attn_kv_reduce": (_i, [_p, _i, _p, _i, _p, _p, _p] + [_i] * 10 + [_f, _i, _i, _i, _p]),
    "cfp_attn_apply": (_i, [_p, _i, _p, _p, _p, _i] + [_i] * 9 + [_f, _f, _i, _i, _i, _p]),
    "cfp_loftr_tail": (_i, [_p, _i, _p, _p, _p, _i, _p, _i, _p, _p, _p, _p, _p, _p, _p, _p, _f] + [_i] * 5 + [_f, _f, _i, _i, _i, _p]),
    "cfp_resize_bilinear": (_i, [_p, _i] + [_i] * 6 + [_p, _i] + [_i] * 6 + [_p] + [_i] * 7 + [_p]),
    "cfp_resize_bilinear_dev": (_i, [_p, _i, _i, _i, _p, _i, _i, _i, _p, _i, _p] + [_i] * 6 + [_i, _p]),
    "cfp_attn_kv_reduce_dev": (_i, [_p, _i, _p, _i, _p, _p, _p] + [_i] * 5 + [_p, _i, _i, _i, _i, _p]),
    "cfp_attn_apply_dev": (_i, [_p, _i, _p, _p, _p, _i] + [_i] * 5 + [_p, _f, _i, _i, _i, _p]),
    "cfp_add_rowtable": (_i, [_p, _i, _p, _p, _i] + [_i] * 8 + [_p]),
    "cfp_upsample_cat_conv3x3": (_i, [_p, _i, _i, _i, _i, _p, _i, _i, _p, _p, _p, _p, _i] + [_i] * 6 + [_p]),
    "cfp_copy_rows": (_i, [_p, _i, _p, _i, _i, _i, _i, _p]),
    "cfp_copy_rows2": (_i, [_p, _i, _p, _i, _i, _p, _i, _p, _i, _i, _i, _i, _p]),
    "cfp_rgb_to_nhwc8": (_i, [_p, _p, _i, _i, _i, _i, _p]),
    "cfp_rgb_to_nhwc8_hilo": (_i, [_p, _p, _i, _i, _i, _i, _p]),
    "cfp_scalar_to_rows8": (_i, [_p, _p, _i, _i, _p]),
    "cfp_silog_ws_bytes": (_sz, [_i, _i, _i]),
    "cfp_silog_loss_fwd": (_i, [_p, _i, _i, _p, _p, _i, _i, _i, _i, _p, _sz, _p, _p]),
    "cfp_silog_loss_bwd": (_i, [_p, _p, _f, _i, _i, _i, _i, _i, _i, _p, _p]),
    "cfp_adamw_step": (_i, [_p, _p, _p, _p, C.c_longlong, _f, _f, _f, _f, _f, _i, _p, _p]),
    "cfp_grad_clip_ws_bytes": (_sz, []),
    "cfp_grad_clip_factor": (_i, [_p, C.c_longlong, _f, _p, _sz, _p, _p]),
    "cfp_tof_hist_sim": (_i, [_p, C.c_longlong, _i, _i, _i, _i, _i, _i, _i, _p, _i, _f, _i, C.c_double, _i, _p, _p, _i, _i, _p, _p, _p, _p, _p, _p]),
    "cfp_tof_sample_points": (_i, [_p, _p, _p, _p, C.c_longlong, _i, _i, _p, _p]),
    "cfp_eval_metrics_ws_bytes": (_sz, [_i]),
    "cfp_eval_metrics": (_i, [_p, _i, _i, _p, _i, _i, _i, _i, _i, _f, _f, _p, _sz, _p, _p]),
    "cfp_unc_sparsification_ws_bytes": (_sz, [_i, _i, _i, _i]),
    "cfp_unc_sparsification": (_i, [_p, _p, _i, _i, _p, _i, _i, _i, _i, _i, _f, _f, _i, _p, _sz, _p, _p, _p, _p]),
    "cfp_eval_metrics_regions_ws_bytes": (_sz, [_i]),
    "cfp_eval_metrics_regions": (_i, [_p, _i, _i, _p, _i, _i, _i, _i, _i, _f, _f, _p, _p, _i, C.POINTER(C.c_float), _i, _p, _sz, _p, _p]),
    "cfp_depth_unproject": (_i, [_p, _i, _i, _i, _i, _i, _i, _f, _f, _p, _p, _p, _p]),
    "cfp_points_compact_ws_bytes": (_sz, [_i, _i, _i, _i]),
    "cfp_points_compact": (_i, [_p, _p, _i, _i, _i, _i, _f, _f, _p, _i, _i, _ll, _f, _f, _i, _p, _p, _p, _p, _p, _sz, _p]),
    "cfp_normal_metrics_ws_bytes": (_sz, [_i, _i, _i]),
    "cfp_normal_metrics": (_i, [_p, _i, _i, _p, _i, _i, _i, _i, _f, _f, _p, _p, _sz, _p, _p, _p, _p]),
    "cfp_render_depth": (_i, [_p, _i, _i, _p, _i, _i, _i, _i, _f, _f, _i, _f, _f, _p, _p, _ll, _i, _p, _f, _p]),
    "cfp_render_zones": (_i, [_p, _p, _p, _i, _i, _i, _i, _i, _f, _f, _p, _i, _p, _ll, _i, _p]),
    "cfp_render_rgb": (_i, [_p, C.POINTER(C.c_float), C.POINTER(C.c_float), _i, _i, _i, _p, _ll, _i, _p]),
    "cfp_conv2d_wgrad_ws_bytes": (_sz, [_i, _i, _i]),
    "cfp_grad_absmax": (_i, [_p, _i, _ll, _i, _p, _p]),
    "cfp_grad_scale": (_i, [_p, _i, _i, _i, _i, _i, _i, _p, _p, _p, _i, _p]),
    "cfp_conv2d_wgrad_x3": (_i, [_p, _i, _p, _i, _p] + [_i] * 12 + [_f, _p, _p, _sz, _p, _p]),
    "cfp_conv2d_dgrad_x3_ws_bytes": (_sz, [_i] * 6),
    "cfp_conv2d_dgrad_x3": (_i, [_p, _i, _p, _p, _i, _p, _i] + [_i] * 12 + [_p, _p, _sz, _p]),
    "cfp_pack_w_x3_blocks": (_i, [_ll, _i]),
    "cfp_pack_w_x3_batch": (_i, [_p, _p, _p, _i, _i, _p]),
    "cfp_conv2d_wgrad": (_i, [_p, _i, _p, _i, _p] + [_i] * 12 + [_f, _i, _p, _sz, _p]),
    "cfp_conv2d_wgrad_bias": (_i, [_p, _i, _p, _i, _p, _p] + [_i] * 12 + [_f, _f, _i, _p, _sz, _p]),
    "cfp_conv2d_wgrad_deferred": (_i, [_p, _i, _p, _i, _p, _p] + [_i] * 12 + [_f, _f, _i, _p, _sz, _p, _p]),
    "cfp_wgrad_reduce_jobs": (_i, [_p, _i, _p]),
    "cfp_conv2d_weight_flip": (_i, [_p, _p, _i, _i, _i, _i, _i, _p]),
    "cfp_weight_flip_blocks": (_i, [_ll]),
    "cfp_conv2d_weight_flip_batch": (_i, [_p, _p, _p, _i, _i, _i, _p]),
    "cfp_conv2d_dgrad": (_i, [_p, _i, _p, _p, _i] + [_i] * 14 + [_p, _sz, _p]),
    "cfp_bn_ws_bytes": (_sz, [_i]),
    "cfp_bn_train_stats": (_i, [_p, _i, C.c_longlong, _i, _i, _p, _p, _f, _f] + [_p] * 7 + [_p, _sz, _p]),
    "cfp_bn_train_stats_partials": (_i, [_p, _i, C.c_longlong, C.c_longlong, _i, _p, _p, _f, _f] + [_p] * 7 + [_p]),
    "cfp_scale_shift_act": (_i, [_p, _i, _p, _p, _i, _p, _i, C.c_longlong, _i, _i, _p]),
    "cfp_scale_shift_act_res": (_i, [_p, _i, _p, _p, _i, _p, _i, _p, _i, C.c_longlong, _i, _i, _p]),
    "cfp_bn_train_bwd": (_i, [_p, _i, _p, _i, C.c_longlong, _i, _i, _p, _p, _p, _p, _i, _p, _p, _p, _i, _p, _sz, _p]),
    "cfp_colsum": (_i, [_p, _i, C.c_longlong, _i, _i, _p, _p, _sz, _p]),
    "cfp_act_bwd": (_i, [_p, _i, _p, _i, _i, _p, _i, C.c_longlong, _i, _i, _p]),
    "cfp_layernorm_bwd_ws_bytes": (_sz, [C.c_longlong, _i]),
    "cfp_layernorm_bwd": (_i, [_p, _i, _p, _i, _p, _f, _p, _i, _i, _p, _p, C.c_longlong, _i, _i, _p, _sz, _p]),
    "cfp_layernorm_bwd_deferred": (_i, [_p, _i, _p, _i, _p, _f, _p, _i, _i, _p, _p, C.c_longlong, _i, _i, _p, _sz, _p, _p]),
    "cfp_axpby": (_i, [_p, _i, _p, _i, _f, _f, _p, _i, C.c_longlong, _i, _i, _p]),
    "cfp_rowtable_grad": (_i, [_p, _i, _p, _i, _i, _i, _i, _i, _i, _i, _f, _i, _p]),
    "cfp_se_train_ws_floats": (_sz, [_i, _i, _i]),
    "cfp_se_train_fwd": (_i, [_p, _i, _f] + [_p] * 7 + [_i, _i, _i, _p]),
    "cfp_se_train_bwd": (_i, [_p] * 12 + [_f, _f, _i, _i, _i, _p]),
    "cfp_channel_dot": (_i, [_p, _i, _p, _i, _p, _i, _i, _i, _i, _p]),
    "cfp_bcast_fma": (_i, [_p, _i, _p, _p, _p, _i, _i, _i, _i, _i, _p]),
    "cfp_dwconv3x3_dgrad": (_i, [_p, _i, _p, _p, _i] + [_i] * 11 + [_p]),
    "cfp_dwconv3x3_wgrad_ws_bytes": (_sz, [_i]),
    "cfp_dwconv3x3_wgrad": (_i, [_p, _i, _p, _i, _p] + [_i] * 9 + [_f, _i, _p, _sz, _p]),
    "cfp_dwconv3x3_wgrad_deferred": (_i, [_p, _i, _p, _i, _p] + [_i] * 9 + [_f, _i, _p, _sz, _p, _p]),
    "cfp_index_rows": (_i, [_p, _i, _p, _p, _i, C.c_longlong, _i, _i, _i, _p]),
    "cfp_resize_bilinear_bwd": (_i, [_p, _i, _p, _i, _i, _i, _i, _i, _i, _i, _i, _i, _p]),
    "cfp_bin_centers": (_i, [_p, _f, _f, _p, _p, _i, _i, _p]),
    "cfp_bin_centers_bwd": (_i, [_p, _f, _f, _p, _i, _i, _p]),
    "cfp_softmax_expect_ws_bytes": (_sz, [_i, _i, _i]),
    "cfp_softmax_expect": (_i, [_p, _i, _p, _p, _p, _p, _i, _p, _i, _i, _i, _i, _p, _sz, _p]),
    "cfp_linattn_state_bytes": (_sz, [_i, _i, _i]),
    "cfp_linattn_ws_bytes": (_sz, [_i, _i, _i, _i, _i]),
    "cfp_linattn_fwd": (_i, [_p, _i, _p, _i, _p, _i, _p, _i, _p, _i, _i, _i, _i, _i, _f, _i, _p, _sz, _p]),
    "cfp_linattn_bwd": (_i, [_p, _i, _p, _i, _p, _i, _p, _i, _p, _p, _i, _p, _i, _p, _i, _i, _i, _i, _i, _i, _f, _i, _p, _sz, _p]),
    "cfp_linattn_fwd_dev": (_i, [_p, _i, _p, _i, _p, _i, _p, _i, _p, _i, _i, _i, _i, _i, _f, _i, _p, _sz, _p, _p]),
    "cfp_linattn_bwd_dev": (_i, [_p, _i, _p, _i, _p, _i, _p, _i, _p, _p, _i, _p, _i, _p, _i, _i, _i, _i, _i, _i, _f, _i, _p, _sz, _p, _p]),
    "cfp_zone_crop": (_i, [_p, _i, _p, _p, _i] + [_i] * 7 + [_i, _p]),
    "cfp_zone_crop_bwd": (_i, [_p, _i, _p, _p, _i] + [_i] * 7 + [_i, _p]),
    "cfp_zone_paste": (_i, [_p, _i, _p, _i, _p, _p, _i] + [_i] * 7 + [_i, _p]),
    "cfp_zone_paste_bwd": (_i, [_p, _i, _p, _p, _i] + [_i] * 7 + [_i, _p]),
    "cfp_zone_rect_rows": (_i, [_p, _i, _p, _p, _i] + [_i] * 6 + [_i, _p]),
    "cfp_dwconv_large_wgrad_ws_bytes": (_sz, [_i, _i, _i, _i, _i]),
    "cfp_dwconv_large_wgrad": (_i, [_p, _i, _p, _i, _p, _i, _i, _i, _i, _i, _f, _i, _p, _sz, _p]),
    "cfp_row_normalize": (_i, [_p, _p, _p, _i, _i, _p]),
    "cfp_add_rowtable_dev": (_i, [_p, _i, _p, _p, _i, _i, _i, _i, _i, _i, _i, _p, _i, _p]),
    "cfp_rowtable_grad_dev": (_i, [_p, _i, _p, _i, _i, _i, _i, _i, _i, _p, _f, _i, _p]),
    "cfp_nyu_augment": (_i, [_p, _p, _i, _i, _i, _p, _p, _p, _i, _i, C.POINTER(C.c_float), C.POINTER(C.c_float), _p, _p, _p]),
    "cfp_nyu_rotate": (_i, [_p, _p, _p, _p, _i, _i, _i, _p, _p]),
    "cfp_bin_regressor": (_i, [_p, _i, _f] + [_p] * 7 + [_f, _f, _i, _p, _p, _i, _i, _i, _i, _p]),
    "cfp_bin_softmax": (_i, [_p, _i, _p, _p, _p, _i, _i, _i, _i, _p]),
    "cfp_bin_softmax_stats": (_i, [_p, _i, _p, _p, _p, _p, _i, _i, _i, _i, _p]),
    "cfp_conv3x3_mean": (_i, [_p, _i, _p, _i, _p, _p, _p, _i, _i, _i, _i, _i, _i, _p]),
    "cfp_lkpm_tail": (_i, [_p, _i, _p, _i, _p, _i, _p, _p, _p, _p, _p, _p, _f, _i, _i, _i, _p]),
    "cfp_mbconv_plan": (_i, [_i, _i, _i, _i, _i, _p, _p]),
    "cfp_mbconv_expand_dw": (_i, [_p, _i, _p, _p, _p, _p, _p, _p, _p, _i, _p, _i, _i, _i, _i, _i, _i, _p]),
    "cfp_conv3x3_pw_fused_variant": (_i, [_i] * 5),
    "cfp_conv3x3_chunk_variant": (_i, [_i] * 4),
    "cfp_conv3x3_pw_fused": (_i, [_p, _i, _p, _p, _p, _i, _p, _p, _p, _i, _p, _i, _p, _i] + [_i] * 12 + [_p]),
    "cfp_hist_encoder": (_i, [_p, _p, _p, _p, _p, _p, _p, _p, _p, _i, _i, _i, _p]),
    "cfp_depth_head_fused": (_i, [_p, _i, _p, _p, _p, _p, _p, _p, _p, _p, _p, _i, _i, _i, _i, _i, _p]),
    "cfp_bin_head_fused": (_i, [_p, _i, _p, _p, _p, _p, _p, _i, _i, _i, _i, _p]),
    "cfp_depth_head_conv0_fused": (_i, [_p, _i, _p, _p, _p, _p, _p, _p, _p, _p, _p, _p, _p, _i, _i, _i, _i, _i, _p]),
    "cfp_depth_head_fused_stats": (_i, [_p, _i, _p, _p, _p, _p, _p, _p, _p, _p, _p, _p, _i, _i, _i, _i, _i, _p]),
    "cfp_bin_head_fused_stats": (_i, [_p, _i, _p, _p, _p, _p, _p, _p, _i, _i, _i, _i, _p]),
}

class WgradJob(C.Structure):
    _fields_ = [("slabs", C.c_void_p), ("dw", C.c_void_p), ("db", C.c_void_p), ("n", C.c_longlong), ("n_dw", C.c_longlong),
                ("nsplit", C.c_int), ("ew", C.c_int), ("beta", C.c_float), ("beta_b", C.c_float)]


_lib: Optional[C.CDLL] = None


def load() -> C.CDLL:
    global _lib
    if _lib is not None:
        return _lib
    if not os.path.exists(LIB_PATH):
        raise RuntimeError(
            f"{LIB_PATH} not found: build the HIP extension first "
            f"(`python -c 'import __graft_entry__ as g; g.build()'` or `make -C cfpnet_amd/csrc`). "
            "There is no CPU fallback for the product path.")
    import torch
    lib = C.CDLL(LIB_PATH)
    for name, (res, args) in SIGNATURES.items():
        fn = getattr(lib, name)
        fn.restype = res
        fn.argtypes = args
    _lib = lib
    return lib


def last_error() -> str:
    return load().cfp_last_error().decode()


def call(name: str, *args):
    rc = getattr(load(), name)(*args)
    if rc != 0:
        raise RuntimeError(f"{name} failed ({rc}): {last_error()}")


def ptr(t) -> int:
    return 0 if t is None else t.data_ptr()


def current_stream() -> int:
    import torch
# ... 2 lines not shown
```

cfpnet_amd/ops.py:

```python
from __future__ import annotations

import os
from dataclasses import dataclass
from typing import Optional, Tuple

import torch

from . import hip

DT = {torch.float32: hip.F32, torch.bfloat16: hip.BF16, torch.float16: hip.F16}


@dataclass
class Act:
    buf: torch.Tensor
    c0: int
    C: int

    @property
    def rows(self) -> int:
        return self.buf.shape[0]

    @property
    def ld(self) -> int:
# ... 172 lines not shown
    hip.call("cfp_dwconv_large_nhwc", x.ptr, x.ld, w.data_ptr(), scale.data_ptr(), shift.data_ptr(), out.ptr, out.ld,
             B, H, W, x.C, k, act, x.dt, _s())


def _bracket16(w: torch.Tensor, dtype):
    r16 = w.to(dtype)
    r = r16.float()
    bits = r16.view(torch.int16).to(torch.int32)
    toward_inf = torch.where(r >= 0, bits + 1, bits - 1)
    toward_ninf = torch.where(r > 0, bits - 1, bits + 1)
    toward_ninf = torch.where(r16.view(torch.int16) == 0, torch.full_like(bits, -32767), toward_ninf)
    toward_inf = torch.where(r16.view(torch.int16) == -32768, torch.ones_like(bits), toward_inf)
    nxt_up = toward_inf.to(torch.int16).view(dtype).float()
    nxt_dn = toward_ninf.to(torch.int16).view(dtype).float()
    up = torch.where(r >= w, r, nxt_up)
    down = torch.where(r <= w, r, nxt_dn)
    return down, up


def pack_w_x3(w2d: torch.Tensor) -> torch.Tensor:
    assert w2d.is_cuda and w2d.dtype == torch.float32 and w2d.dim() == 2 and w2d.is_contiguous()
    rows, k = w2d.shape
    out = torch.empty(rows, (k + 31) // 32 * 64, dtype=torch.float16, device=w2d.device)
    hip.call("cfp_pack_w_x3", w2d.data_ptr(), out.data_ptr(), rows, k, _s())
    if os.environ.get("CFP_X3_DIAG_TWO_TERM", "0") == "1":
        out.view(rows, -1, 2, 32)[:, :, 1, :] = 0
    return out


def pack_w2(w2d: torch.Tensor, dtype) -> torch.Tensor:
    w2d = w2d.detach().float()
    co, k = w2d.shape
    kp = (k + 63) // 64 * 64
    hi = w2d.to(dtype)
    lo = (w2d - hi.float()).to(dtype)
    out = torch.zeros(co, 2 * kp, dtype=dtype)
    out[:, :k] = hi
    out[:, kp:kp + k] = lo
    return out.contiguous()


def round_taps(w: torch.Tensor, dtype, bracket: bool = True) -> torch.Tensor:
    w = w.detach().float()
    if dtype == torch.float32 or w.shape[-1] * w.shape[-2] == 1:
        return w
    kh, kw = w.shape[-2], w.shape[-1]
    order = [r * kw + (c if r % 2 == 0 else kw - 1 - c) for r in range(kh) for c in range(kw)]
    flat = w.reshape(-1, kh * kw)
    if not bracket:
        out = torch.empty_like(flat)
        e = torch.zeros_like(flat[:, 0])
        for t in order:
            v = flat[:, t] + e
            q = v.to(dtype).float()
            e = v - q
            out[:, t] = q
        return out.reshape(w.shape)
    down, up = _bracket16(flat, dtype)
    import numpy as np
    f, dn, upn = flat.numpy(), down.numpy(), up.numpy()
    out = np.empty_like(f)
    e = np.zeros(f.shape[0], dtype=np.float32)
    for t in order:
        v = f[:, t] + e
        take_down = np.abs(v - dn[:, t]) <= np.abs(upn[:, t] - v)
        q = np.where(take_down, dn[:, t], upn[:, t])
        e = v - q
        out[:, t] = q
    return torch.from_numpy(out).reshape(w.shape)


def toeplitz_bands(w: torch.Tensor, dtype) -> torch.Tensor:
    w = w.detach().float().cpu()
    if w.dim() == 4:
        w = w[:, 0]
    w = round_taps(w, dtype)
    C, k, _ = w.shape
    halo = (k - 1) // 2
    lm = (halo + 7) // 8 * 8
    nh = (16 + lm + halo + 31) // 32
    lane = torch.arange(64)
    h = torch.arange(nh)
    e = torch.arange(8)
    kx = 32 * h[:, None, None] + 8 * (lane[None, :, None] // 16) + e[None, None, :] - (lm - halo) - (lane[None, :, None] % 16)
    ok = (kx >= 0) & (kx < k)
    g = w[:, :, kx.clamp(0, k - 1)]
    g = torch.where(ok[None, None], g, torch.zeros(()))
    assert g.numel() == int(hip.load().cfp_dwconv_large_toeplitz_elems(C, k))
    return g.contiguous().to(dtype)


def toeplitz_bands_x3(w: torch.Tensor) -> torch.Tensor:
    w = w.detach().float().cpu()
    if w.dim() == 4:
        w = w[:, 0]
    hi = w.to(torch.float16)
    lo = (w - hi.float()).to(torch.float16)
    return torch.stack([toeplitz_bands(hi.float(), torch.float16), toeplitz_bands(lo.float(), torch.float16)]).contiguous()


def toeplitz_bands_dev(w: torch.Tensor, dtype, flip: bool = False) -> torch.Tensor:
    C, k, _ = w.shape
    assert w.dtype == torch.float32 and w.is_contiguous()
    out = torch.empty(int(hip.load().cfp_dwconv_large_toeplitz_elems(C, k)), dtype=dtype, device=w.device)
    hip.call("cfp_dwconv_large_toeplitz", w.data_ptr(), out.data_ptr(), C, k, int(flip), DT[dtype], _s())
    return out


def dwconv_large_mfma(x: Act, tb: torch.Tensor, scale, shift, out: Act, B, H, W, k, act):
    x3 = x.buf.dtype == torch.float32 and tb.dtype == torch.float16
    assert not x3 or tb.shape[0] == 2
    hip.call("cfp_dwconv_large_mfma_nhwc", x.ptr, x.ld, tb.data_ptr(), scale.data_ptr(), shift.data_ptr(), out.ptr, out.ld,
             B, H, W, x.C, k, act, hip.F32X3 if x3 else x.dt, _s())


def channel_sum(x: Act, partial: torch.Tensor, B, HW, nsplit):
    assert partial.dtype == torch.float32 and partial.numel() >= B * nsplit * x.C
    hip.call("cfp_channel_sum", x.ptr, x.ld, partial.data_ptr(), B, HW, x.C, nsplit, x.dt, _s())


def se_hidden(partial, nsplit, inv_hw, wr, br, hidden, B, C, R):
    hip.call("cfp_se_hidden", partial.data_ptr(), nsplit, float(inv_hw), wr.data_ptr(), br.data_ptr(), hidden.data_ptr(),
             B, C, R, _s())


def se_scale(x: Act, hidden, we_t, be, B, HW, R):
    assert we_t.shape == (R, x.C)
    hip.call("cfp_se_scale", x.ptr, x.ld, hidden.data_ptr(), we_t.data_ptr(), be.data_ptr(), B, HW, x.C, R, x.dt, _s())


def scale_channels(x: Act, gate, B, HW):
    hip.call("cfp_scale_channels", x.ptr, x.ld, gate.data_ptr(), B, HW, x.C, x.dt, _s())


def layernorm(x: Act, gamma, beta, eps, out: Act, rows, residual: Optional[Act] = None):
    hip.call("cfp_layernorm", x.ptr, x.ld, gamma.data_ptr(), beta.data_ptr(), float(eps),
             residual.ptr if residual else 0, residual.ld if residual else 0, out.ptr, out.ld, rows, x.C, x.dt, _s())


def attn_kv_ws_floats(NB, Hk, Wk, th, tw, heads, d) -> int:
    return int(hip.load().cfp_attn_kv_ws_floats(NB, Hk, Wk, th, tw, heads, d))


def attn_kv_reduce(k: Act, v: Act, kv, ksum, ws, NB, Hk, Wk, th, tw, clip, count_pad, v_length, heads, d, rec=None):
    if rec is not None:
        hip.call("cfp_attn_kv_reduce_dev", k.ptr, k.ld, v.ptr, v.ld, kv.data_ptr(), ksum.data_ptr(), hip.ptr(ws),
                 NB, Hk, Wk, th, tw, _rec_ptr(rec), int(count_pad), heads, d, k.dt, _s())
        return
    cy0, cy1, cx0, cx1 = clip
    hip.call("cfp_attn_kv_reduce", k.ptr, k.ld, v.ptr, v.ld, kv.data_ptr(), ksum.data_ptr(), hip.ptr(ws),
             NB, Hk, Wk, th, tw, cy0, cy1, cx0, cx1, int(count_pad), float(v_length), heads, d, k.dt, _s())


def attn_apply(q: Act, kv, ksum, out: Act, NB, Hq, Wq, qth, qtw, excl, v_length, heads, d, eps=1e-6, rec=None):
    if rec is not None:
        hip.call("cfp_attn_apply_dev", q.ptr, q.ld, kv.data_ptr(), ksum.data_ptr(), out.ptr, out.ld,
                 NB, Hq, Wq, qth, qtw, _rec_ptr(rec), float(eps), heads, d, q.dt, _s())
        return
    ey0, ey1, ex0, ex1 = excl
    hip.call("cfp_attn_apply", q.ptr, q.ld, kv.data_ptr(), ksum.data_ptr(), out.ptr, out.ld,
             NB, Hq, Wq, qth, qtw, ey0, ey1, ex0, ex1, float(v_length), float(eps), heads, d, q.dt, _s())


def loftr_tail(q: Optional[Act], kv, ksum, x: Act, out: Act, w_q, w_merge, w_mlp0, w_mlp2, ln1, ln2, NB, Hq, Wq, qth, qtw, v_length,
               heads, eps=1e-6, ln_eps=1e-5):
    D = x.C
    x3 = x.buf.dtype == torch.float32 and w_merge.dtype == torch.float16
    assert (q is None) != (w_q is None), "loftr_tail: give either q or w_q"
    k1, k2 = (2 * D, 4 * D) if x3 else (D, 2 * D)
    assert out.C == D and w_merge.shape == (D, k1) and w_mlp0.shape == (2 * D, k2) and w_mlp2.shape == (D, k2)
    assert q is None or q.C == D
    assert w_q is None or w_q.shape == (D, k1)
    hip.call("cfp_loftr_tail", q.ptr if q is not None else None, q.ld if q is not None else 0, kv.data_ptr(), ksum.data_ptr(), x.ptr, x.ld,
             out.ptr, out.ld, w_q.data_ptr() if w_q is not None else None, w_merge.data_ptr(),
             w_mlp0.data_ptr(), w_mlp2.data_ptr(), ln1[0].data_ptr(), ln1[1].data_ptr(), ln2[0].data_ptr(), ln2[1].data_ptr(),
             float(ln_eps), NB, Hq, Wq, qth, qtw, float(v_length), float(eps), heads, D, hip.F32X3 if x3 else x.dt, _s())


def _rec_ptr(rec) -> int:
    assert rec.dtype == torch.int32 and rec.numel() == 9 and rec.is_cuda and rec.is_contiguous(), "zone record: int32[9] on the device"
    return rec.data_ptr()


def resize_bilinear(src: Act, Hs, Ws, srect, dst: Act, Hd, Wd, drect, B, zone_valid=None, zn=0, p1=0, p2=0,
                    accumulate=False, rec=None, rec_side=0):
    assert src.C == dst.C
    if rec is not None:
        assert (drect if rec_side == 0 else srect) == ((0, 0, Hd, Wd) if rec_side == 0 else (0, 0, Hs, Ws)), "resize_bilinear(rec=): the fixed side is the whole map"
        hip.call("cfp_resize_bilinear_dev", src.ptr, src.ld, Hs, Ws, dst.ptr, dst.ld, Hd, Wd, _rec_ptr(rec), int(rec_side),
                 hip.ptr(zone_valid), zn, p1, p2, int(accumulate), B, src.C, src.dt, _s())
        return
    sy0, sx0, sh, sw = srect
    dy0, dx0, dh, dw = drect
    hip.call("cfp_resize_bilinear", src.ptr, src.ld, Hs, Ws, sy0, sx0, sh, sw, dst.ptr, dst.ld, Hd, Wd, dy0, dx0, dh, dw,
             hip.ptr(zone_valid), zn, p1, p2, int(accumulate), B, src.C, src.dt, _s())


def add_rowtable(x: Act, table, out: Act, rows, H, W, Wt, oy, ox):
    assert table.dtype == torch.float32 and table.shape[1] == x.C
    hip.call("cfp_add_rowtable", x.ptr, x.ld, table.data_ptr(), out.ptr, out.ld, rows, x.C, H, W, Wt, oy, ox, x.dt, _s())


def copy_rows(x: Act, out: Act, rows):
    hip.call("cfp_copy_rows", x.ptr, x.ld, out.ptr, out.ld, rows, x.C, x.dt, _s())


def upsample_cat_conv3x3(low: Act, Hs, Ws, skip: Act, w, scale, shift, out: Act, B, H, W, act, x3: bool = False):
    if x3:
        assert low.dt == skip.dt == out.dt == hip.F32 and w.dtype == torch.float16 and w.shape[-1] == 9 * (low.C + (skip.C + 31) // 32 * 32) * 2
        hip.call("cfp_upsample_cat_conv3x3", low.ptr, low.ld, Hs, Ws, low.C, skip.ptr, skip.ld, skip.C, w.data_ptr(),
                 hip.ptr(scale), hip.ptr(shift), out.ptr, out.ld, B, H, W, out.C, act, hip.F32X3, _s())
        return
    assert w.shape[-1] == 9 * (low.C + skip.C) and low.dt == skip.dt == out.dt
    hip.call("cfp_upsample_cat_conv3x3", low.ptr, low.ld, Hs, Ws, low.C, skip.ptr, skip.ld, skip.C, w.data_ptr(),
             hip.ptr(scale), hip.ptr(shift), out.ptr, out.ld, B, H, W, out.C, act, out.dt, _s())


def pack_w_x3_cat(w: torch.Tensor, cup: int) -> torch.Tensor:
    co, kh, kw, cin = w.shape
    assert kh == 3 and kw == 3 and cup % 32 == 0 and 0 < cup < cin
    csk = cin - cup
    pad = (csk + 31) // 32 * 32 - csk
    wp = torch.nn.functional.pad(w, (0, pad)) if pad else w
    return pack_w_x3(wp.reshape(co, 9 * (cup + csk + pad)).contiguous())


def copy_rows2(x0: Act, out0: Act, x1: Act, out1: Act, rows):
    assert x0.dt == x1.dt == out0.dt == out1.dt and out0.C == x0.C and out1.C == x1.C
    hip.call("cfp_copy_rows2", x0.ptr, x0.ld, out0.ptr, out0.ld, x0.C, x1.ptr, x1.ld, out1.ptr, out1.ld, x1.C, rows, x0.dt, _s())


def rgb_to_nhwc8(rgb: torch.Tensor, out: Act, B, H, W):
    assert rgb.dtype == torch.float32 and rgb.is_contiguous() and out.C == 8 and out.ld == 8
    hip.call("cfp_rgb_to_nhwc8", rgb.data_ptr(), out.ptr, B, H, W, out.dt, _s())


def rgb_to_nhwc8_hilo(rgb: torch.Tensor, out: Act, B, H, W):
    assert rgb.dtype == torch.float32 and rgb.is_contiguous() and out.C == 8 and out.ld == 8
    hip.call("cfp_rgb_to_nhwc8_hilo", rgb.data_ptr(), out.ptr, B, H, W, out.dt, _s())


def scalar_to_rows8(x: torch.Tensor, out: Act, rows):
    assert x.dtype == torch.float32 and x.is_contiguous() and out.C == 8 and out.ld == 8
    hip.call("cfp_scalar_to_rows8", x.data_ptr(), out.ptr, rows, out.dt, _s())


def bin_regressor(partial, nsplit, inv_hw, w1x1, w0, b0, w1, b1, w2, b2, min_val, max_val, norm, edges, centers, B, C,
                  hidden, nbins):
    hip.call("cfp_bin_regressor", partial.data_ptr(), nsplit, float(inv_hw), w1x1.data_ptr(), w0.data_ptr(), b0.data_ptr(),
             w1.data_ptr(), b1.data_ptr(), w2.data_ptr(), b2.data_ptr(), float(min_val), float(max_val), norm,
             edges.data_ptr(), centers.data_ptr(), B, C, hidden, nbins, _s())


def _check_stats(stats, B, HW):
    assert stats.dtype == torch.float32 and stats.is_contiguous() and stats.numel() == B * 3 * HW, "stats: float32 [B, 3, HW]"


def bin_softmax(logits: Act, centers, prob, pred, B, HW, nbins, stats=None):
    if stats is None:
        hip.call("cfp_bin_softmax", logits.ptr, logits.ld, centers.data_ptr(), hip.ptr(prob), pred.data_ptr(), B, HW, nbins,
                 logits.dt, _s())
        return
    _check_stats(stats, B, HW)
    hip.call("cfp_bin_softmax_stats", logits.ptr, logits.ld, centers.data_ptr(), hip.ptr(prob), pred.data_ptr(), stats.data_ptr(), B, HW,
             nbins, logits.dt, _s())


def bin_head_fused(x: Act, w, bias, centers, prob, pred, B, HW, stats=None):
    x3 = x.buf.dtype == torch.float32 and w.dtype == torch.float16
    assert not x3 or (tuple(w.shape) == (256, (x.C + 31) // 32 * 64) and (prob is None or prob.dtype == torch.float32))
    if stats is None:
        hip.call("cfp_bin_head_fused", x.ptr, x.ld, w.data_ptr(), bias.data_ptr(), centers.data_ptr(), hip.ptr(prob),
                 pred.data_ptr(), B, HW, x.C, hip.F32X3 if x3 else x.dt, _s())
        return
    _check_stats(stats, B, HW)
    hip.call("cfp_bin_head_fused_stats", x.ptr, x.ld, w.data_ptr(), bias.data_ptr(), centers.data_ptr(), hip.ptr(prob),
             pred.data_ptr(), stats.data_ptr(), B, HW, x.C, hip.F32X3 if x3 else x.dt, _s())


def permute_wout(w: torch.Tensor, dtype, hilo: bool = True, diffuse: bool = False) -> torch.Tensor:
    w = w.detach().float().reshape(w.shape[0], -1)
    assert w.shape == (256, 128)
    src = pw_k_order(128)
    wp = w[:, src]
    hi = (round_taps(w.reshape(256, 1, 128), dtype).reshape(256, 128)[:, src] if diffuse else wp).to(dtype)
    planes = [hi]
    if hilo:
        planes.append((wp - hi.float()).to(dtype))
    return torch.stack(planes).contiguous()


def pw_k_order(K: int) -> torch.Tensor:
    pos = torch.arange((K + 31) // 32 * 32)
    kb, q, e = pos // 32, (pos % 32) // 8, pos % 8
    src = 32 * kb + 16 * (e // 4) + 4 * q + (e % 4)
    return torch.where(src < K, src, torch.full_like(src, -1))


def pad_pw_w(w: torch.Tensor) -> torch.Tensor:
    co, K = w.shape
    out = torch.zeros((co + 15) // 16 * 16, (K + 31) // 32 * 32, dtype=w.dtype, device=w.device)
    out[:co, :K] = w
    return out.contiguous()


def conv3x3_pw_fused_variant(Cin: int, Cmid: int, Cout: int, stride: int, dt: int) -> int:
    return int(hip.load().cfp_conv3x3_pw_fused_variant(Cin, Cmid, Cout, stride, dt))


def conv3x3_pw_fused(x: Act, w1: torch.Tensor, s1, t1, act1, w2_pad: torch.Tensor, s2, t2, out: Act, B, H, W, stride, pad_t, pad_l, Ho, Wo,
                     act2=hip.ACT_NONE, residual: Optional[Act] = None):
    mid = w1.shape[0]
    assert x.rows >= B * H * W and out.rows >= B * Ho * Wo and x.dt == out.dt
    assert w1.dtype == x.buf.dtype and tuple(w1.shape) == (mid, 9 * x.C) and w1.is_contiguous()
    assert w2_pad.dtype == x.buf.dtype and tuple(w2_pad.shape) == ((out.C + 15) // 16 * 16, (mid + 31) // 32 * 32) and w2_pad.is_contiguous()
    hip.call("cfp_conv3x3_pw_fused", x.ptr, x.ld, w1.data_ptr(), hip.ptr(s1), hip.ptr(t1), act1, w2_pad.data_ptr(), hip.ptr(s2), hip.ptr(t2), act2,
             residual.ptr if residual else 0, residual.ld if residual else 0, out.ptr, out.ld, B, H, W, x.C, mid, out.C, stride, pad_t, pad_l,
             Ho, Wo, x.dt, _s())


def depth_head_fused(x: Act, w3, scale3, shift3, wout_perm: torch.Tensor, bias_out, centers, prob, pred, B, H, W, ram_out: Optional[Act] = None,
                     ram_hilo: bool = True, probe: int = 0, stats=None):
    assert x.C == 128 and w3.shape == (128, 9 * 128) and wout_perm.shape[1:] == (256, 128) and wout_perm.dtype == x.buf.dtype
    flags = (hip.HEAD_WOUT_HILO if wout_perm.shape[0] == 2 else 0) | (hip.HEAD_RAM_HILO if ram_hilo else 0) | (probe << 8)
    if ram_out is not None:
        assert ram_out.ld == 128 and ram_out.C == 128
    if stats is None:
        hip.call("cfp_depth_head_fused", x.ptr, x.ld, w3.data_ptr(), hip.ptr(scale3), hip.ptr(shift3), wout_perm.data_ptr(), bias_out.data_ptr(),
                 centers.data_ptr(), hip.ptr(prob), pred.data_ptr(), ram_out.ptr if ram_out is not None else 0, B, H, W, flags, x.dt, _s())
        return
    _check_stats(stats, B, H * W)
# ... 66 lines not shown
```

include/cfpnet_hip.h:

```cpp
#ifndef CFPNET_HIP_H
#define CFPNET_HIP_H

#include <stddef.h>
#include <stdint.h>

#ifdef __cplusplus
extern "C" {
#endif

typedef void* cfp_stream_t;

enum { CFP_OK = 0, CFP_EINVAL = -1, CFP_ESHAPE = -2, CFP_EHIP = -3 };
enum { CFP_F32 = 0, CFP_BF16 = 1, CFP_F16 = 2 };
enum { CFP_F32X3 = 3 };
enum { CFP_TOF_SAMPLE_UNIFORM = 0, CFP_TOF_SAMPLE_ICDF = 1 };
enum { CFP_ACT_NONE = 0, CFP_ACT_RELU = 1, CFP_ACT_LRELU = 2, CFP_ACT_SILU = 3, CFP_ACT_GELU = 4, CFP_ACT_SIGMOID = 5 };

int cfp_version(void);
const char* cfp_last_error(void);

int cfp_conv2d_nhwc(const void* in, int in_ld, const void* w, const float* scale, const float* shift,
                    const void* residual, int res_ld, void* out, int out_ld,
                    int B, int H, int W, int Cin, int Cout, int KH, int KW, int stride,
                    int pad_t, int pad_l, int Ho, int Wo, int act, int dtype,
                    void* ws, size_t ws_bytes, cfp_stream_t stream);

enum { CFP_CONV_PER_IMAGE = 1, CFP_CONV_W2 = 2, CFP_CONV_IN_FLIGHT = 4, CFP_CONV_X3 = 8, CFP_CONV_WS_TICKETS = 16 };
#define CFP_CONV_TICKET_BYTES 4096
int cfp_conv2d_nhwc_ex(const void* in, int in_ld, const void* w, const float* scale, const float* shift,
                       const void* residual, int res_ld, void* out, int out_ld,
                       int B, int H, int W, int Cin, int Cout, int KH, int KW, int stride,
                       int pad_t, int pad_l, int Ho, int Wo, int act, int dtype,
                       const float* ln_gamma, const float* ln_beta, float ln_eps, int per_image_weights,
                       void* ws, size_t ws_bytes, cfp_stream_t stream);

size_t cfp_pack_w_x3_elems(long long rows, int K);
int cfp_pack_w_x3(const float* w, void* out, long long rows, int K, cfp_stream_t stream);

size_t cfp_conv2d_ws_bytes(int M, int Cout, int K, int dtype);

int cfp_conv2d_plan(int M, int Cout, int K, int KH, int stride, int dtype, int rows_per_batch, int B, int* variant,
                    int* splits);

int cfp_conv3x3_chunk_variant(int M, int Cin, int Cout, int in_flight);

int cfp_conv2d_variant(int M, int Cout);

int cfp_debug_set(int key, int value);

int cfp_dwconv3x3_nhwc(const void* in, int in_ld, const void* w, const float* scale, const float* shift,
                       void* out, int out_ld, int B, int H, int W, int C, int stride, int pad_t, int pad_l,
                       int Ho, int Wo, int act, int dtype, cfp_stream_t stream);

int cfp_dwconv3x3_strips(int B, int Ho, int Wo, int C, int stride, int dtype);
int cfp_dwconv3x3_launch_slots(int B, int H, int W, int Ho, int Wo, int C, int stride, int in_ld, int out_ld, int dtype);
int cfp_dwconv3x3_sum_nhwc(const void* in, int in_ld, const void* w, const float* scale, const float* shift,
                           void* out, int out_ld, float* partial, int B, int H, int W, int C, int stride,
                           int pad_t, int pad_l, int Ho, int Wo, int act, int dtype, cfp_stream_t stream);

int cfp_dwconv_large_nhwc(const void* in, int in_ld, const float* w, const float* scale, const float* shift,
                          void* out, int out_ld, int B, int H, int W, int C, int k, int act, int dtype,
                          cfp_stream_t stream);

size_t cfp_dwconv_large_toeplitz_elems(int C, int k);
int cfp_dwconv_large_toeplitz(const float* w, void* out, int C, int k, int flip, int dtype, cfp_stream_t stream);
int cfp_dwconv_large_mfma_nhwc(const void* in, int in_ld, const void* toeplitz, const float* scale, const float* shift,
                               void* out, int out_ld, int B, int H, int W, int C, int k, int act, int dtype,
                               cfp_stream_t stream);

int cfp_channel_sum(const void* in, int in_ld, float* partial, int B, int HW, int C, int nsplit, int dtype,
                    cfp_stream_t stream);

int cfp_se_hidden(const float* partial, int nsplit, float inv_hw, const float* w_reduce, const float* b_reduce,
                  float* hidden, int B, int C, int R, cfp_stream_t stream);

int cfp_se_scale(void* x, int ld, const float* hidden, const float* w_expand_t, const float* b_expand,
                 int B, int HW, int C, int R, int dtype, cfp_stream_t stream);

int cfp_se_fold(const void* w_proj, void* w_out, const float* hidden, const float* w_expand_t, const float* b_expand,
                int B, int Cout, int C, int R, int dtype, cfp_stream_t stream);

int cfp_mbconv_plan(int B, int H, int W, int Cin, int mid, int* tiles_per_image, int* KP);
int cfp_mbconv_expand_dw(const void* x, int x_ld, const void* wpw, const float* s1, const float* t1, const void* wdw,
                         const float* s2, const float* t2, void* out, int out_ld, float* partial, int B, int H, int W, int Cin,
                         int mid, int dtype, cfp_stream_t stream);

int cfp_conv3x3_pw_fused_variant(int Cin, int Cmid, int Cout, int stride, int dtype);
int cfp_conv3x3_pw_fused(const void* in, int in_ld, const void* w1, const float* scale1, const float* shift1, int act1,
                         const void* w2_pad, const float* scale2, const float* shift2, int act2, const void* residual, int res_ld,
                         void* out, int out_ld, int B, int H, int W, int Cin, int Cmid, int Cout, int stride, int pad_t, int pad_l,
                         int Ho, int Wo, int dtype, cfp_stream_t stream);

int cfp_se_gate_fold(const float* partial, int nsplit, float inv_hw, const float* w_reduce, const float* b_reduce,
                     const float* w_expand_t, const float* b_expand, const void* w_proj, void* w_out,
                     int B, int Cout, int C, int R, int dtype, cfp_stream_t stream);

int cfp_dwconv3x3_se_parts(int B, int Ho, int Wo, int C, int stride, int dtype);
int cfp_dwconv3x3_se_nhwc(const void* in, int in_ld, const void* w, const float* scale, const float* shift, void* out, int out_ld,
                          const float* w_reduce, int R, float* hpart, int B, int H, int W, int C, int stride, int pad_t, int pad_l,
                          int Ho, int Wo, int act, int dtype, cfp_stream_t stream);

int cfp_se_gate_fold2(const float* hpart, int K, float inv_hw, const float* b_reduce, const float* w_expand_t, const float* b_expand,
                      const float* w_proj, void* w_out, int B, int Cout, int C, int R, int dtype, cfp_stream_t stream);

int cfp_scale_channels(void* x, int ld, const float* gate, int B, int HW, int C, int dtype, cfp_stream_t stream);

int cfp_layernorm(const void* in, int in_ld, const float* gamma, const float* beta, float eps,
                  const void* residual, int res_ld, void* out, int out_ld, int rows, int C, int dtype,
                  cfp_stream_t stream);

size_t cfp_attn_kv_ws_floats(int NB, int Hk, int Wk, int th, int tw, int heads, int d);
int cfp_attn_kv_reduce(const void* k, int k_ld, const void* v, int v_ld, float* kv, float* ksum, float* ws,
                       int NB, int Hk, int Wk, int th, int tw, int cy0, int cy1, int cx0, int cx1,
                       int count_pad, float v_length, int heads, int d, int dtype, cfp_stream_t stream);

int cfp_attn_kv_reduce_dev(const void* k, int k_ld, const void* v, int v_ld, float* kv, float* ksum, float* ws,
                           int NB, int Hk, int Wk, int th, int tw, const int* rec, int count_pad, int heads, int d, int dtype,
                           cfp_stream_t stream);

int cfp_attn_apply(const void* q, int q_ld, const float* kv, const float* ksum, void* out, int out_ld,
                   int NB, int Hq, int Wq, int qth, int qtw, int ey0, int ey1, int ex0, int ex1,
                   float v_length, float eps, int heads, int d, int dtype, cfp_stream_t stream);

int cfp_attn_apply_dev(const void* q, int q_ld, const float* kv, const float* ksum, void* out, int out_ld,
                       int NB, int Hq, int Wq, int qth, int qtw, const int* rec, float eps, int heads, int d, int dtype,
                       cfp_stream_t stream);

int cfp_loftr_tail(const void* q, int q_ld, const float* kv, const float* ksum, const void* x, int x_ld,
                   void* out, int out_ld, const void* w_q, const void* w_merge, const void* w_mlp0, const void* w_mlp2,
                   const float* ln1_g, const float* ln1_b, const float* ln2_g, const float* ln2_b, float ln_eps,
                   int NB, int Hq, int Wq, int qth, int qtw, float v_length, float eps, int heads, int D,
                   int dtype, cfp_stream_t stream);

int cfp_resize_bilinear(const void* src, int src_ld, int Hs, int Ws, int sy0, int sx0, int sh, int sw,
                        void* dst, int dst_ld, int Hd, int Wd, int dy0, int dx0, int dh, int dw,
                        const uint8_t* zone_valid, int zn, int p1, int p2, int accumulate,
                        int B, int C, int dtype, cfp_stream_t stream);

int cfp_resize_bilinear_dev(const void* src, int src_ld, int Hs, int Ws, void* dst, int dst_ld, int Hd, int Wd,
                            const int* rec, int rec_side, const uint8_t* zone_valid, int zn, int p1, int p2,
                            int accumulate, int B, int C, int dtype, cfp_stream_t stream);

int cfp_add_rowtable(const void* in, int in_ld, const float* table, void* out, int out_ld, int rows, int C,
                     int H, int W, int Wt, int oy, int ox, int dtype, cfp_stream_t stream);

int cfp_upsample_cat_conv3x3(const void* low, int low_ld, int Hs, int Ws, int Cup, const void* skip, int skip_ld, int Cskip,
                             const void* w, const float* scale, const float* shift, void* out, int out_ld, int B, int H, int W,
                             int Cout, int act, int dtype, cfp_stream_t stream);

int cfp_copy_rows(const void* in, int in_ld, void* out, int out_ld, int rows, int C, int dtype, cfp_stream_t stream);
int cfp_copy_rows2(const void* in0, int in0_ld, void* out0, int out0_ld, int C0, const void* in1, int in1_ld, void* out1, int out1_ld,
                   int C1, int rows, int dtype, cfp_stream_t stream);

int cfp_rgb_to_nhwc8(const float* rgb, void* out, int B, int H, int W, int dtype, cfp_stream_t stream);
int cfp_rgb_to_nhwc8_hilo(const float* rgb, void* out, int B, int H, int W, int dtype, cfp_stream_t stream);
int cfp_scalar_to_rows8(const float* in, void* out, int rows, int dtype, cfp_stream_t stream);

int cfp_hist_encoder(const float* hist, const float* blob, const int* layout, void* out0, void* out1, void* out2,
                     const float* pe0, const float* pe1, const float* pe2, int n_pe, int R, int dtype, cfp_stream_t stream);

int cfp_lkpm_tail(const void* t, int t_ld, const void* xin, int x_ld, void* out, int out_ld, const void* w1, const float* b1,
                  const void* w2, const float* b2, const float* ln_g, const float* ln_b, float ln_eps, int rows, int D, int dtype,
                  cfp_stream_t stream);

int cfp_bin_regressor(const float* partial, int nsplit, float inv_hw, const float* w1x1_t,
                      const float* w0_t, const float* b0, const float* w1_t, const float* b1,
                      const float* w2_t, const float* b2, float min_val, float max_val, int norm,
                      float* edges, float* centers, int B, int C, int hidden, int nbins, cfp_stream_t stream);

int cfp_conv3x3_mean(const float* partial, int nsplit, const void* in, int in_ld, const float* w, const float* bias, float* msum,
                     int B, int H, int W, int C, int Cout, int dtype, cfp_stream_t stream);

int cfp_bin_softmax(const void* logits, int ld, const float* centers, void* prob, float* pred,
                    int B, int HW, int nbins, int dtype, cfp_stream_t stream);

enum { CFP_UNC_STD = 0, CFP_UNC_ENTROPY = 1, CFP_UNC_PMAX = 2 };
int cfp_bin_softmax_stats(const void* logits, int ld, const float* centers, void* prob, float* pred, float* stats,
                          int B, int HW, int nbins, int dtype, cfp_stream_t stream);

enum { CFP_HEAD_WOUT_HILO = 1, CFP_HEAD_RAM_HILO = 2 };
int cfp_depth_head_fused(const void* x, int x_ld, const void* w3, const float* scale3, const float* shift3,
                         const void* wout_perm, const float* bias_out, const float* centers, void* prob, float* pred,
                         void* ram_out, int B, int H, int W, int flags, int dtype, cfp_stream_t stream);
int cfp_depth_head_fused_stats(const void* x, int x_ld, const void* w3, const float* scale3, const float* shift3,
                               const void* wout_perm, const float* bias_out, const float* centers, void* prob, float* pred,
                               float* stats, void* ram_out, int B, int H, int W, int flags, int dtype, cfp_stream_t stream);

int cfp_depth_head_conv0_fused(const void* t, int t_ld, const void* w0, const float* scale0, const float* shift0, const void* w3,
                               const float* scale3, const float* shift3, const void* wout_perm, const float* bias_out,
                               const float* centers, void* prob, float* pred, int B, int H, int W, int flags, int dtype,
                               cfp_stream_t stream);

int cfp_bin_head_fused(const void* x, int x_ld, const void* w, const float* bias, const float* centers,
                       void* prob, float* pred, int B, int HW, int Cin, int dtype, cfp_stream_t stream);
int cfp_bin_head_fused_stats(const void* x, int x_ld, const void* w, const float* bias, const float* centers,
                             void* prob, float* pred, float* stats, int B, int HW, int Cin, int dtype, cfp_stream_t stream);


size_t cfp_silog_ws_bytes(int B, int Ht, int Wt);
int cfp_silog_loss_fwd(const float* pred, int Hp, int Wp, const float* target, const unsigned char* mask, int Ht, int Wt,
                       int B, int interpolate, void* ws, size_t ws_bytes, float* stats, cfp_stream_t stream);
int cfp_silog_loss_bwd(const void* ws, const float* stats, float grad_loss, int Hp, int Wp, int Ht, int Wt, int B,
                       int interpolate, float* grad_pred, cfp_stream_t stream);

int cfp_adamw_step(float* param, const float* grad, float* exp_avg, float* exp_avg_sq, long long n, float lr,
                   float beta1, float beta2, float eps, float weight_decay, int step, const float* grad_scale,
                   cfp_stream_t stream);
size_t cfp_grad_clip_ws_bytes(void);
int cfp_grad_clip_factor(const float* grad, long long n, float max_norm, void* ws, size_t ws_bytes, float* out,
                         cfp_stream_t stream);


int cfp_tof_hist_sim(const float* depth, long long img_stride, int B, int H, int W, int zone_num, int zone_px, int sy0,
                     int sx0, const int* offsets, int offset_bound, float max_distance, int bins, double bin_width,
                     int floor_count, const float* w0, const float* w1, int nsamp, int sample_mode, double* fh, float* rect,
                     unsigned char* mask, float* pts, int* hist_out, cfp_stream_t stream);
int cfp_tof_sample_points(const double* fh, const unsigned char* mask, const float* w0, const float* w1, long long nzones,
                          int nsamp, int sample_mode, float* pts, cfp_stream_t stream);

size_t cfp_eval_metrics_ws_bytes(int B);
int cfp_eval_metrics(const float* pred, int Hp, int Wp, const float* gt, int H, int W, int B, int interpolate, int mode,
                     float lo, float hi, void* ws, size_t ws_bytes, double* out, cfp_stream_t stream);

enum { CFP_SPARS_STD = 0, CFP_SPARS_ENTROPY, CFP_SPARS_PMAX, CFP_SPARS_ORACLE_RMSE, CFP_SPARS_ORACLE_ABSREL };
size_t cfp_unc_sparsification_ws_bytes(int B, int H, int W, int steps);
int cfp_unc_sparsification(const float* pred, const float* unc, int Hp, int Wp, const float* gt, int H, int W, int B,
                           int interpolate, int mode, float lo, float hi, int steps, void* ws, size_t ws_bytes,
                           double* curves , double* summary ,
                           double* n_valid , cfp_stream_t stream);

enum { CFP_REGION_ALL = 0, CFP_REGION_FOV_IN, CFP_REGION_FOV_OUT, CFP_REGION_ZONE_VALID, CFP_REGION_ZONE_INVALID };
size_t cfp_eval_metrics_regions_ws_bytes(int B);
int cfp_eval_metrics_regions(const float* pred, int Hp, int Wp, const float* gt, int H, int W, int B, int interpolate, int mode,
                             float lo, float hi, const float* rect , const unsigned char* mask , int Z,
                             const float* edges , int n_edges, void* ws, size_t ws_bytes,
                             double* out , cfp_stream_t stream);

int cfp_depth_unproject(const float* pred, int Hp, int Wp, int H, int W, int B, int interpolate, float lo, float hi,
                        const float* K , float* points ,
                        float* normals , cfp_stream_t stream);

size_t cfp_points_compact_ws_bytes(int B, int H, int W, int stride);
int cfp_points_compact(const float* points, const float* normals, int H, int W, int B, int stride, float z_near, float z_far,
                       const float* unc, int Hu, int Wu, long long unc_stride, float unc_lo, float unc_hi, int cap,
                       float* out_points , float* out_normals ,
                       int* out_index , int* counts , void* ws, size_t ws_bytes, cfp_stream_t stream);

enum { CFP_NORMAL_MEAN = 0, CFP_NORMAL_MEDIAN, CFP_NORMAL_RMSE, CFP_NORMAL_FRAC_11_25, CFP_NORMAL_FRAC_22_5, CFP_NORMAL_FRAC_30,
       CFP_NORMAL_N_VALID };
size_t cfp_normal_metrics_ws_bytes(int B, int H, int W);
int cfp_normal_metrics(const float* pred, int Hp, int Wp, const float* gt, int H, int W, int B, int interpolate, float lo, float hi,
                       const float* K , void* ws, size_t ws_bytes, double* out ,
                       int* hist , float* angle_map , cfp_stream_t stream);

enum { CFP_RENDER_DEPTH = 0, CFP_RENDER_GT = 1, CFP_RENDER_ABS_ERR = 2, CFP_RENDER_REL_ERR = 3 };
int cfp_render_depth(const float* pred, int Hp, int Wp, const float* gt, int H, int W, int B, int interpolate, float lo, float hi,
                     int what, float vmin, float vmax, const unsigned char* lut , unsigned char* out,
                     long long image_stride, int pitch, unsigned short* u16_out , float u16_scale,
                     cfp_stream_t stream);
int cfp_render_zones(const float* hist , const float* rect , const unsigned char* mask ,
                     int Z, int S, int H, int W, int B, float vmin, float vmax, const unsigned char* lut , int alpha,
                     unsigned char* out, long long image_stride, int pitch, cfp_stream_t stream);
int cfp_render_rgb(const float* rgb , const float* mean , const float* std , int H,
                   int W, int B, unsigned char* out, long long image_stride, int pitch, cfp_stream_t stream);


size_t cfp_conv2d_wgrad_ws_bytes(int Cout, int K, int M);
int cfp_conv2d_wgrad(const void* x, int x_ld, const void* dy, int dy_ld, float* dw, int B, int H, int W, int Cin, int Cout,
                     int KH, int KW, int stride, int pad_t, int pad_l, int Ho, int Wo, float beta, int dtype, void* ws,
                     size_t ws_bytes, cfp_stream_t stream);
int cfp_conv2d_wgrad_bias(const void* x, int x_ld, const void* dy, int dy_ld, float* dw, float* db, int B, int H, int W, int Cin,
                          int Cout, int KH, int KW, int stride, int pad_t, int pad_l, int Ho, int Wo, float beta, float beta_b,
                          int dtype, void* ws, size_t ws_bytes, cfp_stream_t stream);
typedef struct cfp_wgrad_job {
  const float* slabs; float* dw; float* db;
  long long n, n_dw;
  int nsplit, ew;
  float beta, beta_b;
} cfp_wgrad_job;
int cfp_conv2d_wgrad_deferred(const void* x, int x_ld, const void* dy, int dy_ld, float* dw, float* db, int B, int H, int W, int Cin,
                              int Cout, int KH, int KW, int stride, int pad_t, int pad_l, int Ho, int Wo, float beta, float beta_b,
                              int dtype, void* ws, size_t ws_bytes, cfp_wgrad_job* job, cfp_stream_t stream);
int cfp_wgrad_reduce_jobs(const cfp_wgrad_job* jobs, int njobs, cfp_stream_t stream);
int cfp_dwconv3x3_wgrad_deferred(const void* x, int x_ld, const void* dy, int dy_ld, float* dw, int B, int H, int W, int C, int stride,
                                 int pad_t, int pad_l, int Ho, int Wo, float beta, int dtype, void* ws, size_t ws_bytes,
// ... 131 lines not shown
```

Measured before the change: 3899 maps/s.

## Fuse K/V projection into linear-attention KV reduction and add fused x2i tail

Adds a kernel that loads the input token tile into LDS, projects it to K and V with MFMA inside the kernel, and feeds the result directly into the shared KV-reduction body, so the projected K/V activations are never written to or read back from global memory. The existing reduction is refactored into a shared header used by both paths. It also adds a fused x2i LoFTR tail entry that works on the zone grid, apparently folding the resize steps in. The fused path is limited to bf16/f16, certain head configurations and an LDS budget, and when those do not hold the model falls back to the old path.

```diff
diff --git a/cfpnet_amd/csrc/attention.hip b/cfpnet_amd/csrc/attention.hip
--- a/cfpnet_amd/csrc/attention.hip
+++ b/cfpnet_amd/csrc/attention.hip
@@ -1,123 +1,15 @@
-#include "common.h"
+#include "kv_reduce_core.h"
 
 namespace {
-
-struct KvP {
-  const void* k; const void* v;
-  float* kv; float* ksum; float* ws;
-  int k_ld, v_ld;
-  int NB, Hk, Wk, th, tw, gy, gx;
-  int cy0, cy1, cx0, cx1;
-  int count_pad, heads, d, nsplit;
-  float inv_len;
-  const int* rec;
-};
-
-template <int D> struct KvCfg;
-template <> struct KvCfg<4>  { static constexpr int IC = 1; };
-template <> struct KvCfg<8>  { static constexpr int IC = 2; };
-template <> struct KvCfg<16> { static constexpr int IC = 2; };
-template <> struct KvCfg<32> { static constexpr int IC = 2; };
 
 template <typename T, int D, bool DEV>
 __global__ __launch_bounds__(64) void kv_reduce_kernel(KvP p) {
-  constexpr int IC = KvCfg<D>::IC;
-  constexpr int TPK = D / IC;
-  constexpr int KL = 64 / TPK;
-  const T* __restrict__ K = reinterpret_cast<const T*>(p.k);
-  const T* __restrict__ V = reinterpret_cast<const T*>(p.v);
   const int g = blockIdx.x, h = blockIdx.y, sp = blockIdx.z;
   const int lane = threadIdx.x;
-  const int ip = lane % TPK, kl = lane / TPK;
-
-  const int gpb = p.gy * p.gx;
-  const int b = g / gpb, gi = g % gpb;
-  const int ty = gi / p.gx, tx = gi % p.gx;
-  int cy0 = p.cy0, cy1 = p.cy1, cx0 = p.cx0, cx1 = p.cx1;
-  float inv_len = p.inv_len;
-  if constexpr (DEV) {
-    const int* __restrict__ rec = p.rec;
-    cy0 = rec[4]; cy1 = rec[5]; cx0 = rec[6]; cx1 = rec[7];
-    inv_len = 1.0f / (float)max(rec[8], 1);
-  }
-  const int y0 = max(max(ty * p.th, cy0), 0), y1 = min(min((ty + 1) * p.th, cy1), p.Hk);
-  const int x0 = max(max(tx * p.tw, cx0), 0), x1 = min(min((tx + 1) * p.tw, cx1), p.Wk);
-  const int rh = max(y1 - y0, 0), rw = max(x1 - x0, 0);
-  const int S = rh * rw;
-  const int per = (S + p.nsplit - 1) / p.nsplit;
-  const int s_begin = sp * per, s_end = min(S, s_begin + per);
-
-  float acc[IC][D];
-  float ks[IC];
-#pragma unroll
-  for (int i = 0; i < IC; ++i) {
-    ks[i] = 0.f;
-#pragma unroll
-    for (int j = 0; j < D; ++j) acc[i][j] = 0.f;
-  }
-  constexpr int KU = 4;
-  const int rwd = max(rw, 1);
-  const int step_q = KL / rwd, step_r = KL - step_q * rwd;
-  const int s_first = min(s_begin + kl, max(s_end - 1, 0));
-  int cy = s_first / rwd, cx = s_first - cy * rwd;
-  const int ly = max(s_end - 1, 0) / rwd, lx = max(s_end - 1, 0) - ly * rwd;
-  for (int s0 = s_begin + kl; s0 < s_end; s0 += KL * KU) {
-    float kf[KU][IC], vf[KU][D];
-#pragma unroll
-    for (int u = 0; u < KU; ++u) {
-      const bool in = s0 + u * KL < s_end;
-      const int yy = y0 + (in ? cy : ly), xx = x0 + (in ? cx : lx);
-      cx += step_r; cy += step_q;
-      if (cx >= rwd) { cx -= rwd; ++cy; }
-      const long long row = ((long long)b * p.Hk + yy) * p.Wk + xx;
-      const T* kp = K + row * p.k_ld + h * D + ip * IC;
-      const T* vp = V + row * p.v_ld + h * D;
-#pragma unroll
-      for (int i = 0; i < IC; ++i) kf[u][i] = to_f32<T>(kp[i]);
-#pragma unroll
-      for (int j = 0; j < D; ++j) vf[u][j] = to_f32<T>(vp[j]);
-    }
-#pragma unroll
-    for (int u = 0; u < KU; ++u) {
-      if (s0 + u * KL >= s_end) continue;
-#pragma unroll
-      for (int j = 0; j < D; ++j) vf[u][j] *= inv_len;
-#pragma unroll
-      for (int i = 0; i < IC; ++i) {
-        const float kk = elu1(kf[u][i]);
-        ks[i] += kk;
-#pragma unroll
-        for (int j = 0; j < D; ++j) acc[i][j] = fmaf(kk, vf[u][j], acc[i][j]);
-      }
-    }
-  }
-#pragma unroll
-  for (int o = TPK; o < 64; o <<= 1) {
-#pragma unroll
-    for (int i = 0; i < IC; ++i) {
-      ks[i] += __shfl_xor(ks[i], o, 64);
-#pragma unroll
-      for (int j = 0; j < D; ++j) acc[i][j] += __shfl_xor(acc[i][j], o, 64);
-    }
-  }
-  if (kl == 0) {
-    float padk = 0.f;
-    if (p.count_pad && sp == 0) padk = (float)(p.th * p.tw - S);
-    float* dkv; float* dks;
-    if (p.nsplit == 1) {
-      dkv = p.kv + ((long long)g * p.heads + h) * D * D;
-      dks = p.ksum + ((long long)g * p.heads + h) * D;
-    } else {
-      float* base = p.ws + (((long long)g * p.heads + h) * p.nsplit + sp) * (D * D + D);
-      dkv = base; dks = base + D * D;
-    }
-#pragma unroll
-    for (int i = 0; i < IC; ++i) {
-      dks[ip * IC + i] = ks[i] + padk;
-#pragma unroll
-      for (int j = 0; j < D; ++j) dkv[(ip * IC + i) * D + j] = acc[i][j];
-    }
-  }
+  const KvGeom q = kv_group_geom<DEV>(p, g, sp);
+  constexpr int TPK = D / KvCfg<D>::IC;
+  KvGlobalKeys<T> keys(p, q, lane / TPK, 64 / TPK);
+  kv_reduce_body<T, D>(p, q, g, h, sp, lane, keys);
 }
 
 __global__ __launch_bounds__(256) void kv_finalize_kernel(const float* __restrict__ ws, float* __restrict__ kv,
@@ -215,6 +107,7 @@
 }
 
 void cfp_attn_debug_set(int value) { g_kv_target_waves = value; }
+int kv_pick_nsplit(int S, long long groups_heads) { return pick_nsplit(S, groups_heads); }
 void cfp_attn_apply_debug_set(int value) { g_ap_split_below = value; }
 
 extern "C" size_t cfp_attn_kv_ws_floats(int NB, int Hk, int Wk, int th, int tw, int heads, int d) {
@@ -225,17 +118,14 @@
   return (size_t)(groups * heads * ns * (d * d + d));
 }
 
-static int kv_reduce_impl(const void* k, int k_ld, const void* v, int v_ld, float* kv, float* ksum, float* ws,
-                          int NB, int Hk, int Wk, int th, int tw, int cy0, int cy1, int cx0, int cx1,
-                          int count_pad, float v_length, const int* rec, int heads, int d, int dtype, cfp_stream_t stream, const char* who) {
-  CFP_REQUIRE(dtype_ok(dtype), CFP_EINVAL, std::string(who) + ": bad dtype");
-  CFP_REQUIRE(k && v && kv && ksum, CFP_EINVAL, std::string(who) + ": null pointer");
-  CFP_REQUIRE(NB > 0 && Hk > 0 && Wk > 0 && th > 0 && tw > 0 && heads > 0 && (d == 4 || d == 8 || d == 16 || d == 32) &&
-                  k_ld >= heads * d && v_ld >= heads * d && v_length > 0.f,
+int kv_fill_params(KvP& p, float* kv, float* ksum, float* ws, int NB, int Hk, int Wk, int th, int tw, int cy0, int cy1, int cx0, int cx1,
+                   int count_pad, float v_length, const int* rec, int heads, int d, const char* who) {
+  CFP_REQUIRE(kv && ksum, CFP_EINVAL, std::string(who) + ": null pointer");
+  CFP_REQUIRE(NB > 0 && Hk > 0 && Wk > 0 && th > 0 && tw > 0 && heads > 0 && (d == 4 || d == 8 || d == 16 || d == 32) && v_length > 0.f,
               CFP_ESHAPE, std::string(who) + ": bad shape (head dim must be 4, 8, 16 or 32)");
-  KvP p;
   p.rec = rec;
-  p.k = k; p.v = v; p.kv = kv; p.ksum = ksum; p.ws = ws; p.k_ld = k_ld; p.v_ld = v_ld;
+  p.k = nullptr; p.v = nullptr; p.k_ld = 0; p.v_ld = 0;
+  p.kv = kv; p.ksum = ksum; p.ws = ws;
   p.NB = NB; p.Hk = Hk; p.Wk = Wk; p.th = th; p.tw = tw; p.gy = cdiv(Hk, th); p.gx = cdiv(Wk, tw);
   p.cy0 = cy0; p.cy1 = cy1; p.cx0 = cx0; p.cx1 = cx1; p.count_pad = count_pad; p.heads = heads; p.d = d;
   p.inv_len = 1.0f / v_length;
@@ -244,8 +134,28 @@
   p.nsplit = pick_nsplit(S, groups * heads);
   CFP_REQUIRE(p.nsplit == 1 || ws, CFP_EINVAL, std::string(who) + ": workspace required");
   CFP_REQUIRE(groups < (1ll << 31) && heads <= 65535, CFP_ESHAPE, std::string(who) + ": grid too large");
+  return CFP_OK;
+}
+
+void kv_finalize_launch(const KvP& p, hipStream_t s) {
+  long long items = (long long)p.NB * p.gy * p.gx * p.heads;
+  long long total = items * (p.d * p.d + p.d);
+  int blocks = (int)((total + 255) / 256 > 4096 ? 4096 : (total + 255) / 256);
+  hipLaunchKernelGGL(kv_finalize_kernel, dim3(blocks), dim3(256), 0, s, p.ws, p.kv, p.ksum, p.nsplit, p.d, items);
+}
+
+static int kv_reduce_impl(const void* k, int k_ld, const void* v, int v_ld, float* kv, float* ksum, float* ws,
+                          int NB, int Hk, int Wk, int th, int tw, int cy0, int cy1, int cx0, int cx1,
+                          int count_pad, float v_length, const int* rec, int heads, int d, int dtype, cfp_stream_t stream, const char* who) {
+  CFP_REQUIRE(dtype_ok(dtype), CFP_EINVAL, std::string(who) + ": bad dtype");
+  CFP_REQUIRE(k && v && kv && ksum, CFP_EINVAL, std::string(who) + ": null pointer");
+  CFP_REQUIRE(heads > 0 && d > 0 && k_ld >= heads * d && v_ld >= heads * d, CFP_ESHAPE, std::string(who) + ": bad shape (head dim must be 4, 8, 16 or 32)");
+  KvP p;
+  const int rc = kv_fill_params(p, kv, ksum, ws, NB, Hk, Wk, th, tw, cy0, cy1, cx0, cx1, count_pad, v_length, rec, heads, d, who);
+  if (rc != CFP_OK) return rc;
+  p.k = k; p.v = v; p.k_ld = k_ld; p.v_ld = v_ld;
   hipStream_t s = reinterpret_cast<hipStream_t>(stream);
-  dim3 grid((unsigned)groups, heads, p.nsplit);
+  dim3 grid((unsigned)((long long)NB * p.gy * p.gx), heads, p.nsplit);
 #define KV_LAUNCH(T, D) do { if (rec) hipLaunchKernelGGL((kv_reduce_kernel<T, D, true>), grid, dim3(64), 0, s, p); \
                              else hipLaunchKernelGGL((kv_reduce_kernel<T, D, false>), grid, dim3(64), 0, s, p); } while (0)
 #define KV_SWITCH(T) switch (d) { case 4: KV_LAUNCH(T, 4); break; case 8: KV_LAUNCH(T, 8); break; \
@@ -253,12 +163,7 @@
   if (dtype == CFP_BF16) { KV_SWITCH(bf16_t) } else if (dtype == CFP_F16) { KV_SWITCH(f16_t) } else { KV_SWITCH(float) }
 #undef KV_SWITCH
 #undef KV_LAUNCH
-  if (p.nsplit > 1) {
-    long long items = groups * heads;
-    long long total = items * (d * d + d);
-    int blocks = (int)((total + 255) / 256 > 4096 ? 4096 : (total + 255) / 256);
-    hipLaunchKernelGGL(kv_finalize_kernel, dim3(blocks), dim3(256), 0, s, ws, kv, ksum, p.nsplit, d, items);
-  }
+  if (p.nsplit > 1) kv_finalize_launch(p, s);
   return cfp_check_launch(who);
 }
 
diff --git a/cfpnet_amd/csrc/attn_kv_project.hip b/cfpnet_amd/csrc/attn_kv_project.hip
--- /dev/null
+++ b/cfpnet_amd/csrc/attn_kv_project.hip
@@ -0,0 +1,149 @@
+#include "kv_reduce_core.h"
+
+namespace {
+
+struct KvProjP {
+  KvP r;
+  const void* x;
+  const void* w;
+  int x_ld;
+  int rows16;
+};
+
+template <typename H, int DM, int HEADS, bool DEV>
+__global__ __launch_bounds__(64 * HEADS) void kv_project_reduce_kernel(KvProjP pp) {
+  constexpr int d = DM / HEADS;
+  constexpr int PX = DM + 8, PKV = 2 * DM + 8;
+  constexpr int XCH = DM / 8;
+  constexpr int NT = 2 * DM / 16;
+  constexpr int CW = NT < HEADS ? NT : HEADS;
+  constexpr int RW = HEADS / CW;
+  constexpr int NJ = NT / CW;
+  constexpr int NKB = DM / 32;
+  extern __shared__ __attribute__((aligned(16))) unsigned char smem[];
+  const KvP& p = pp.r;
+  H* tX = reinterpret_cast<H*>(smem);
+  H* tKV = tX + pp.rows16 * 16 * PX;
+  const int tid = threadIdx.x;
+  const int lane = tid & 63;
+  const int wave = __builtin_amdgcn_readfirstlane(tid >> 6);
+  const int fr = lane & 15, fq = lane >> 4;
+  const int g = blockIdx.x, sp = blockIdx.y;
+  const KvGeom q = kv_group_geom<DEV>(p, g, sp);
+  const int n = max(q.s_end - q.s_begin, 0);
+  const int nt16 = (n + 15) >> 4;
+
+  if (n > 0) {
+    const int cg = wave % CW, rg = wave / CW;
+    const H* __restrict__ W = reinterpret_cast<const H*>(pp.w);
+    s16x8 bw[NJ][NKB];
+#pragma unroll
+    for (int j = 0; j < NJ; ++j)
+#pragma unroll
+      for (int kb = 0; kb < NKB; ++kb)
+        bw[j][kb] = *reinterpret_cast<const s16x8*>(W + (long long)((cg + j * CW) * 16 + fr) * DM + kb * 32 + fq * 8);
+    const H* __restrict__ X = reinterpret_cast<const H*>(pp.x);
+    const int rwd = max(q.rw, 1);
+    for (int i = tid; i < nt16 * 16 * XCH; i += 64 * HEADS) {
+      const int r = i / XCH, ch = i - r * XCH;
+      u32x4 v = {0u, 0u, 0u, 0u};
+      if (r < n) {
+        const int s = q.s_begin + r;
+        const int sy = s / rwd, sx = s - sy * rwd;
+        const long long row = ((long long)q.b * p.Hk + q.y0 + sy) * p.Wk + q.x0 + sx;
+        v = *reinterpret_cast<const u32x4*>(X + row * pp.x_ld + ch * 8);
+      }
+      *reinterpret_cast<u32x4*>(tX + r * PX + ch * 8) = v;
+    }
+    __syncthreads();
+    for (int rt = rg; rt < nt16; rt += RW) {
+      f32x4 acc[NJ];
+#pragma unroll
+      for (int j = 0; j < NJ; ++j) acc[j] = f32x4{0.f, 0.f, 0.f, 0.f};
+#pragma unroll
+      for (int kb = 0; kb < NKB; ++kb) {
+        const s16x8 a = *reinterpret_cast<const s16x8*>(tX + (rt * 16 + fr) * PX + kb * 32 + fq * 8);
+#pragma unroll
+        for (int j = 0; j < NJ; ++j) acc[j] = mfma16<H>(a, bw[j][kb], acc[j]);
+      }
+#pragma unroll
+      for (int j = 0; j < NJ; ++j)
+#pragma unroll
+        for (int r = 0; r < 4; ++r) tKV[(rt * 16 + fq * 4 + r) * PKV + (cg + j * CW) * 16 + fr] = from_f32<H>(acc[j][r] * 1.f + 0.f);
+    }
+  }
+  __syncthreads();
+
+  constexpr int TPK = d / KvCfg<d>::IC;
+  KvTileKeys<H> keys(tKV, PKV, DM, q, lane / TPK, 64 / TPK);
+  kv_reduce_body<H, d>(p, q, g, wave, sp, lane, keys);
+}
+
+size_t proj_lds_bytes(int rows16, int DM) { return (size_t)rows16 * 16 * ((DM + 8) + (2 * DM + 8)) * 2; }
+constexpr size_t kProjLdsBudget = 52 * 1024;
+
+int proj_rows16(int NB, int Hk, int Wk, int th, int tw, int heads) {
+  const long long groups = (long long)NB * cdiv(Hk, th) * cdiv(Wk, tw);
+  const int S = (th < Hk ? th : Hk) * (tw < Wk ? tw : Wk);
+  const int ns = kv_pick_nsplit(S, groups * heads);
+  return cdiv(cdiv(S, ns), 16);
+}
+
+bool proj_fits(int NB, int Hk, int Wk, int th, int tw, int heads, int d, int dtype) {
+  if (!is16(dtype) || NB <= 0 || Hk <= 0 || Wk <= 0 || th <= 0 || tw <= 0 || (heads != 4 && heads != 8)) return false;
+  const int DM = heads * d;
+  if (DM != 32 && DM != 64 && DM != 128) return false;
+  return proj_lds_bytes(proj_rows16(NB, Hk, Wk, th, tw, heads), DM) <= kProjLdsBudget;
+}
+
+int project_reduce_impl(const void* x, int x_ld, const void* w_kv, float* kv, float* ksum, float* ws, int NB, int Hk, int Wk, int th, int tw,
+                        int cy0, int cy1, int cx0, int cx1, int count_pad, float v_length, const int* rec, int heads, int d, int dtype,
+                        cfp_stream_t stream, const char* who) {
+  CFP_REQUIRE(is16(dtype), CFP_EINVAL, std::string(who) + ": bf16 / f16 storage only");
+  CFP_REQUIRE(x && w_kv && kv && ksum, CFP_EINVAL, std::string(who) + ": null pointer");
+  CFP_REQUIRE(aligned16(x) && aligned16(w_kv), CFP_EINVAL, std::string(who) + ": x and the weights must be 16-byte aligned");
+  CFP_REQUIRE(proj_fits(NB, Hk, Wk, th, tw, heads, d, dtype), CFP_ESHAPE,
+              std::string(who) + ": the problem does not fit (cfp_attn_kv_project_fits): D = heads * d in 32 / 64 / 128, heads 4 / 8, a split's rows within the LDS budget");
+  const int DM = heads * d;
+  CFP_REQUIRE(x_ld >= DM && x_ld % 8 == 0, CFP_ESHAPE, std::string(who) + ": the token pitch must be >= D and a multiple of 8");
+  KvProjP pp;
+  const int rc = kv_fill_params(pp.r, kv, ksum, ws, NB, Hk, Wk, th, tw, cy0, cy1, cx0, cx1, count_pad, v_length, rec, heads, d, who);
+  if (rc != CFP_OK) return rc;
+  pp.x = x; pp.w = w_kv; pp.x_ld = x_ld;
+  pp.rows16 = proj_rows16(NB, Hk, Wk, th, tw, heads);
+  CFP_REQUIRE(pp.r.nsplit <= 65535, CFP_ESHAPE, std::string(who) + ": grid too large");
+  const size_t lds = proj_lds_bytes(pp.rows16, DM);
+  hipStream_t s = reinterpret_cast<hipStream_t>(stream);
+  const dim3 grid((unsigned)((long long)NB * pp.r.gy * pp.r.gx), pp.r.nsplit);
+#define KVP_LAUNCH(T, DM_, HD) do { if (rec) hipLaunchKernelGGL((kv_project_reduce_kernel<T, DM_, HD, true>), grid, dim3(64 * HD), lds, s, pp); \
+                                    else hipLaunchKernelGGL((kv_project_reduce_kernel<T, DM_, HD, false>), grid, dim3(64 * HD), lds, s, pp); } while (0)
+#define KVP_HEADS(T, DM_) do { if (heads == 4) KVP_LAUNCH(T, DM_, 4); else KVP_LAUNCH(T, DM_, 8); } while (0)
+#define KVP_SWITCH(T) switch (DM) { case 32: KVP_HEADS(T, 32); break; case 64: KVP_HEADS(T, 64); break; default: KVP_HEADS(T, 128); break; }
+  if (dtype == CFP_BF16) { KVP_SWITCH(bf16_t) } else { KVP_SWITCH(f16_t) }
+#undef KVP_SWITCH
+#undef KVP_HEADS
+#undef KVP_LAUNCH
+  if (pp.r.nsplit > 1) kv_finalize_launch(pp.r, s);
+  return cfp_check_launch(who);
+}
+
+}
+
+extern "C" int cfp_attn_kv_project_fits(int NB, int Hk, int Wk, int th, int tw, int heads, int d, int dtype) {
+  return proj_fits(NB, Hk, Wk, th, tw, heads, d, dtype) ? 1 : 0;
+}
+
+extern "C" int cfp_attn_kv_project_reduce(const void* x, int x_ld, const void* w_kv, float* kv, float* ksum, float* ws,
+                                          int NB, int Hk, int Wk, int th, int tw, int cy0, int cy1, int cx0, int cx1,
+                                          int count_pad, float v_length, int heads, int d, int dtype, cfp_stream_t stream) {
+  return project_reduce_impl(x, x_ld, w_kv, kv, ksum, ws, NB, Hk, Wk, th, tw, cy0, cy1, cx0, cx1, count_pad, v_length, nullptr, heads, d, dtype,
+                             stream, "cfp_attn_kv_project_reduce");
+}
+
+extern "C" int cfp_attn_kv_project_reduce_dev(const void* x, int x_ld, const void* w_kv, float* kv, float* ksum, float* ws,
+                                              int NB, int Hk, int Wk, int th, int tw, const int* rec, int count_pad, int heads, int d, int dtype,
+                                              cfp_stream_t stream) {
+  CFP_REQUIRE(rec && (reinterpret_cast<uintptr_t>(rec) & 3) == 0, CFP_EINVAL, "cfp_attn_kv_project_reduce_dev: bad record pointer");
+  return project_reduce_impl(x, x_ld, w_kv, kv, ksum, ws, NB, Hk, Wk, th, tw, 0, 0, 0, 0, count_pad, 1.f, rec, heads, d, dtype, stream,
+                             "cfp_attn_kv_project_reduce_dev");
+}
diff --git a/cfpnet_amd/csrc/kv_reduce_core.h b/cfpnet_amd/csrc/kv_reduce_core.h
--- /dev/null
+++ b/cfpnet_amd/csrc/kv_reduce_core.h
@@ -0,0 +1,166 @@
+#pragma once
+#include "common.h"
+
+struct KvP {
+  const void* k; const void* v;
+  float* kv; float* ksum; float* ws;
+  int k_ld, v_ld;
+  int NB, Hk, Wk, th, tw, gy, gx;
+  int cy0, cy1, cx0, cx1;
+  int count_pad, heads, d, nsplit;
+  float inv_len;
+  const int* rec;
+};
+
+template <int D> struct KvCfg;
+template <> struct KvCfg<4>  { static constexpr int IC = 1; };
+template <> struct KvCfg<8>  { static constexpr int IC = 2; };
+template <> struct KvCfg<16> { static constexpr int IC = 2; };
+template <> struct KvCfg<32> { static constexpr int IC = 2; };
+
+struct KvGeom { int b, y0, x0, rw, S, s_begin, s_end; float inv_len; };
+
+template <bool DEV>
+__device__ __forceinline__ KvGeom kv_group_geom(const KvP& p, int g, int sp) {
+  KvGeom q;
+  const int gpb = p.gy * p.gx;
+  const int gi = g % gpb;
+  q.b = g / gpb;
+  const int ty = gi / p.gx, tx = gi % p.gx;
+  int cy0 = p.cy0, cy1 = p.cy1, cx0 = p.cx0, cx1 = p.cx1;
+  q.inv_len = p.inv_len;
+  if constexpr (DEV) {
+    const int* __restrict__ rec = p.rec;
+    cy0 = rec[4]; cy1 = rec[5]; cx0 = rec[6]; cx1 = rec[7];
+    q.inv_len = 1.0f / (float)max(rec[8], 1);
+  }
+  q.y0 = max(max(ty * p.th, cy0), 0);
+  q.x0 = max(max(tx * p.tw, cx0), 0);
+  const int y1 = min(min((ty + 1) * p.th, cy1), p.Hk);
+  const int x1 = min(min((tx + 1) * p.tw, cx1), p.Wk);
+  const int rh = max(y1 - q.y0, 0);
+  q.rw = max(x1 - q.x0, 0);
+  q.S = rh * q.rw;
+  const int per = (q.S + p.nsplit - 1) / p.nsplit;
+  q.s_begin = sp * per;
+  q.s_end = min(q.S, q.s_begin + per);
+  return q;
+}
+
+template <typename T>
+struct KvGlobalKeys {
+  const T* K; const T* V;
+  long long k_ld, v_ld;
+  int b, Hk, Wk, y0, x0, rwd, step_q, step_r, cy, cx, ly, lx;
+  __device__ __forceinline__ KvGlobalKeys(const KvP& p, const KvGeom& q, int kl, int KL)
+      : K(reinterpret_cast<const T*>(p.k)), V(reinterpret_cast<const T*>(p.v)), k_ld(p.k_ld), v_ld(p.v_ld), b(q.b), Hk(p.Hk), Wk(p.Wk),
+        y0(q.y0), x0(q.x0) {
+    rwd = max(q.rw, 1);
+    step_q = KL / rwd; step_r = KL - step_q * rwd;
+    const int s_first = min(q.s_begin + kl, max(q.s_end - 1, 0));
+    cy = s_first / rwd; cx = s_first - cy * rwd;
+    ly = max(q.s_end - 1, 0) / rwd; lx = max(q.s_end - 1, 0) - ly * rwd;
+  }
+  __device__ __forceinline__ void next(bool in, const T*& kp, const T*& vp) {
+    const int yy = y0 + (in ? cy : ly), xx = x0 + (in ? cx : lx);
+    cx += step_r; cy += step_q;
+    if (cx >= rwd) { cx -= rwd; ++cy; }
+    const long long row = ((long long)b * Hk + yy) * Wk + xx;
+    kp = K + row * k_ld;
+    vp = V + row * v_ld;
+  }
+};
+
+template <typename T>
+struct KvTileKeys {
+  const T* tile;
+  int ld, dm, cur, step, last;
+  __device__ __forceinline__ KvTileKeys(const T* tile_, int ld_, int dm_, const KvGeom& q, int kl, int KL)
+      : tile(tile_), ld(ld_), dm(dm_), cur(kl), step(KL), last(max(q.s_end - 1 - q.s_begin, 0)) {}
+  __device__ __forceinline__ void next(bool in, const T*& kp, const T*& vp) {
+    const int r = in ? cur : last;
+    cur += step;
+    kp = tile + r * ld;
+    vp = kp + dm;
+  }
+};
+
+template <typename T, int D, typename KEYS>
+__device__ __forceinline__ void kv_reduce_body(const KvP& p, const KvGeom& q, int g, int h, int sp, int lane, KEYS& keys) {
+  constexpr int IC = KvCfg<D>::IC;
+  constexpr int TPK = D / IC;
+  constexpr int KL = 64 / TPK;
+  const int ip = lane % TPK, kl = lane / TPK;
+  const int s_begin = q.s_begin, s_end = q.s_end;
+  const float inv_len = q.inv_len;
+
+  float acc[IC][D];
+  float ks[IC];
+#pragma unroll
+  for (int i = 0; i < IC; ++i) {
+    ks[i] = 0.f;
+#pragma unroll
+    for (int j = 0; j < D; ++j) acc[i][j] = 0.f;
+  }
+  constexpr int KU = 4;
+  for (int s0 = s_begin + kl; s0 < s_end; s0 += KL * KU) {
+    float kf[KU][IC], vf[KU][D];
+#pragma unroll
+    for (int u = 0; u < KU; ++u) {
+      const bool in = s0 + u * KL < s_end;
+      const T* kr; const T* vr;
+      keys.next(in, kr, vr);
+      const T* kp = kr + h * D + ip * IC;
+      const T* vp = vr + h * D;
+#pragma unroll
+      for (int i = 0; i < IC; ++i) kf[u][i] = to_f32<T>(kp[i]);
+#pragma unroll
+      for (int j = 0; j < D; ++j) vf[u][j] = to_f32<T>(vp[j]);
+    }
+#pragma unroll
+    for (int u = 0; u < KU; ++u) {
+      if (s0 + u * KL >= s_end) continue;
+#pragma unroll
+      for (int j = 0; j < D; ++j) vf[u][j] *= inv_len;
+#pragma unroll
+      for (int i = 0; i < IC; ++i) {
+        const float kk = elu1(kf[u][i]);
+        ks[i] += kk;
+#pragma unroll
+        for (int j = 0; j < D; ++j) acc[i][j] = fmaf(kk, vf[u][j], acc[i][j]);
+      }
+    }
+  }
+#pragma unroll
+  for (int o = TPK; o < 64; o <<= 1) {
+#pragma unroll
+    for (int i = 0; i < IC; ++i) {
+      ks[i] += __shfl_xor(ks[i], o, 64);
+#pragma unroll
+      for (int j = 0; j < D; ++j) acc[i][j] += __shfl_xor(acc[i][j], o, 64);
+    }
+  }
+  if (kl == 0) {
+    float padk = 0.f;
+    if (p.count_pad && sp == 0) padk = (float)(p.th * p.tw - q.S);
+    float* dkv; float* dks;
+    if (p.nsplit == 1) {
+      dkv = p.kv + ((long long)g * p.heads + h) * D * D;
+      dks = p.ksum + ((long long)g * p.heads + h) * D;
+    } else {
+      float* base = p.ws + (((long long)g * p.heads + h) * p.nsplit + sp) * (D * D + D);
+      dkv = base; dks = base + D * D;
+    }
+#pragma unroll
+    for (int i = 0; i < IC; ++i) {
+      dks[ip * IC + i] = ks[i] + padk;
+#pragma unroll
+      for (int j = 0; j < D; ++j) dkv[(ip * IC + i) * D + j] = acc[i][j];
+    }
+  }
+}
+
+int kv_pick_nsplit(int S, long long groups_heads);
+int kv_fill_params(KvP& p, float* kv, float* ksum, float* ws, int NB, int Hk, int Wk, int th, int tw, int cy0, int cy1, int cx0, int cx1,
+                   int count_pad, float v_length, const int* rec, int heads, int d, const char* who);
+void kv_finalize_launch(const KvP& p, hipStream_t s);
diff --git a/cfpnet_amd/csrc/loftr_tail.hip b/cfpnet_amd/csrc/loftr_tail.hip
--- a/cfpnet_amd/csrc/loftr_tail.hip
+++ b/cfpnet_amd/csrc/loftr_tail.hip
@@ -45,7 +45,7 @@
   }
 }
 
-template <typename H, int D, int HEADS, int WAVES>
+template <typename H, int D, int HEADS, int WAVES, bool MAP = false>
 __global__ __launch_bounds__(64 * WAVES) void loftr_tail_kernel(TailP<H, H> p) {
   constexpr int PA = D + 8, PH = 2 * D + 8;
   constexpr int WAVE_LDS = (2 * PA + PH) * 16 * 2;
@@ -61,7 +61,8 @@
   H* tH = tX + 16 * PA;
   const long long row0 = (long long)blockIdx.x * (16 * WAVES) + wave * 16;
 
-  tail_tile_load<H, D, PA>(tX, p.x, p.x_ld, row0, p.rows, lane);
+  if constexpr (MAP) tail_tile_load_mapped<H, D, PA>(tX, p, row0, lane);
+  else tail_tile_load<H, D, PA>(tX, p.x, p.x_ld, row0, p.rows, lane);
 
   const bool own_q = p.wq != nullptr;
   if (own_q) {
@@ -115,7 +116,8 @@
       }
   }
   asm volatile("s_waitcnt lgkmcnt(0)" ::: "memory");
-  tail_tile_store<H, D, PA>(p.out, p.out_ld, tMsg, row0, p.rows, lane);
+  if constexpr (MAP) tail_tile_store_mapped<H, D, PA>(p, tMsg, row0, lane);
+  else tail_tile_store<H, D, PA>(p.out, p.out_ld, tMsg, row0, p.rows, lane);
 }
 
 template <typename H, int D>
@@ -189,11 +191,11 @@
 
 void cfp_tail16_debug_set(int value) { g_tail16_waves = value; }
 
-extern "C" int cfp_loftr_tail(const void* q, int q_ld, const float* kv, const float* ksum, const void* x, int x_ld,
-                              void* out, int out_ld, const void* w_q, const void* w_merge, const void* w_mlp0, const void* w_mlp2,
-                              const float* ln1_g, const float* ln1_b, const float* ln2_g, const float* ln2_b, float ln_eps,
-                              int NB, int Hq, int Wq, int qth, int qtw, float v_length, float eps, int heads, int D,
-                              int dtype, cfp_stream_t stream) {
+static int loftr_tail_impl(const void* q, int q_ld, const float* kv, const float* ksum, const void* x, int x_ld,
+                           void* out, int out_ld, const void* w_q, const void* w_merge, const void* w_mlp0, const void* w_mlp2,
+                           const float* ln1_g, const float* ln1_b, const float* ln2_g, const float* ln2_b, float ln_eps,
+                           int NB, int Hq, int Wq, int qth, int qtw, float v_length, float eps, int heads, int D,
+                           int dtype, cfp_stream_t stream, const TailMap* map) {
   const bool x3 = dtype == CFP_F32X3;
   const int vec = x3 ? 4 : 8;
   const bool rows_ok = (long long)NB * Hq * Wq < (1ll << 31);
@@ -214,17 +216,43 @@
   };
   auto run = [&](auto tag) {
     using H = decltype(tag);
-    const TailP<H, H> p = params(tag, tag);
+    TailP<H, H> p = params(tag, tag);
+    if (map) p.map = *map;
     return tail_pick<32, 64, 128>(D, [&](auto d) { return tail_pick<4, 8>(heads, [&](auto h) {
       return tail_pick<1, 2, 4>(tail_waves(p.rows, g_tail16_waves), [&](auto w) {
         constexpr int D_ = d, W_ = w;
         constexpr size_t lds = 2 * (2 * D_ * 128) + W_ * ((2 * (D_ + 8) + 2 * D_ + 8) * 16 * 2);
+        if (map) return tail_launch<loftr_tail_kernel<H, D_, h, W_, true>, lds>(p, W_, s);
         return tail_launch<loftr_tail_kernel<H, D_, h, W_>, lds>(p, W_, s);
       }); }); });
   };
   const int rc = x3 ? loftr_tail_x3_launch(params(float{}, f16_t{}), heads, D, s) : dtype == CFP_F16 ? run(f16_t{}) : run(bf16_t{});
   CFP_REQUIRE(rc == 0, CFP_EHIP, x3 ? "cfp_loftr_tail: f16x3 launch failed" : "cfp_loftr_tail: launch failed");
   return cfp_check_launch("cfp_loftr_tail");
+}
+
+extern "C" int cfp_loftr_tail(const void* q, int q_ld, const float* kv, const float* ksum, const void* x, int x_ld,
+                              void* out, int out_ld, const void* w_q, const void* w_merge, const void* w_mlp0, const void* w_mlp2,
+                              const float* ln1_g, const float* ln1_b, const float* ln2_g, const float* ln2_b, float ln_eps,
+                              int NB, int Hq, int Wq, int qth, int qtw, float v_length, float eps, int heads, int D,
+                              int dtype, cfp_stream_t stream) {
+  return loftr_tail_impl(q, q_ld, kv, ksum, x, x_ld, out, out_ld, w_q, w_merge, w_mlp0, w_mlp2, ln1_g, ln1_b, ln2_g, ln2_b, ln_eps, NB, Hq, Wq, qth, qtw,
+                         v_length, eps, heads, D, dtype, stream, nullptr);
+}
+
+extern "C" int cfp_loftr_tail_x2i(const float* kv, const float* ksum, void* tok, int tok_ld, int H, int W, int sy, int sx,
+                                  const void* w_q, const void* w_merge, const void* w_mlp0, const void* w_mlp2,
+                                  const float* ln1_g, const float* ln1_b, const float* ln2_g, const float* ln2_b, float ln_eps,
+                                  int NB, int gh, int gw, int p1, int p2, const uint8_t* zone_valid, int zn, int accumulate,
+                                  float v_length, float eps, int heads, int D, int dtype, cfp_stream_t stream) {
+  CFP_REQUIRE(is16(dtype), CFP_EINVAL, "cfp_loftr_tail_x2i: bf16 / f16 only");
+  CFP_REQUIRE(tok && w_q, CFP_EINVAL, "cfp_loftr_tail_x2i: null pointer (the kernel projects q itself: w_q must be given)");
+  CFP_REQUIRE(H > 0 && W > 0 && p1 > 0 && p2 > 0 && (long long)NB * H * W < (1ll << 31), CFP_ESHAPE, "cfp_loftr_tail_x2i: bad token map");
+  CFP_REQUIRE(!zone_valid || (zn > 0 && gh <= zn * p1 && gw <= zn * p2), CFP_ESHAPE, "cfp_loftr_tail_x2i: zone grid smaller than the query grid");
+  TailMap map;
+  map.zone_valid = zone_valid; map.H = H; map.W = W; map.sy = sy; map.sx = sx; map.zn = zn; map.p1 = p1; map.p2 = p2; map.accumulate = accumulate;
+  return loftr_tail_impl(nullptr, 0, kv, ksum, tok, tok_ld, tok, tok_ld, w_q, w_merge, w_mlp0, w_mlp2, ln1_g, ln1_b, ln2_g, ln2_b, ln_eps, NB, gh, gw,
+                         p1, p2, v_length, eps, heads, D, dtype, stream, &map);
 }
 
 extern "C" int cfp_lkpm_tail(const void* t, int t_ld, const void* xin, int x_ld, void* out, int out_ld, const void* w1, const float* b1,
diff --git a/cfpnet_amd/csrc/tail_core.h b/cfpnet_amd/csrc/tail_core.h
--- a/cfpnet_amd/csrc/tail_core.h
+++ b/cfpnet_amd/csrc/tail_core.h
@@ -97,6 +97,10 @@
   }
 }
 
+struct TailMap {
+  const uint8_t* zone_valid;
+  int H, W, sy, sx, zn, p1, p2, accumulate;
+};
 template <typename T, typename W> struct TailP {
   const T* q; const float* kv; const float* ksum; const T* x; T* out;
   const W* wq;
@@ -106,6 +110,7 @@
   int rows, Hq, Wq, qth, qtw, ggy, ggx;
   FastDiv fwq, fhq, fqth, fqtw;
   float v_length, eps, ln_eps;
+  TailMap map;
 };
 template <typename T, typename W> struct LkpmP {
   const T* t; const T* xin; T* out;
@@ -174,6 +179,61 @@
       const T v = from_f32<T>(o[j] * zi * p.v_length);
       tMsg[r * PA + h * d + j] = ok ? v : T(0);
     }
+  }
+}
+
+template <typename T, typename W>
+__device__ __forceinline__ long long tail_map_row(const TailP<T, W>& p, long long m, int& b, int& gy, int& gx) {
+  const unsigned t = fd_div((unsigned)m, p.fwq);
+  gx = (int)((unsigned)m - t * (unsigned)p.Wq);
+  const unsigned bu = fd_div(t, p.fhq);
+  gy = (int)(t - bu * (unsigned)p.Hq);
+  b = (int)bu;
+  const int y = p.map.sy + gy, x = p.map.sx + gx;
+  if (y < 0 || y >= p.map.H || x < 0 || x >= p.map.W) return -1;
+  return ((long long)b * p.map.H + y) * p.map.W + x;
+}
+template <typename T, int D, int PA, typename W>
+__device__ __forceinline__ void tail_tile_load_mapped(T* tile, const TailP<T, W>& p, long long row0, int lane) {
+  constexpr int E = 16 / sizeof(T), XCH = D / E;
+  for (int i = lane; i < 16 * XCH; i += 64) {
+    const int r = i / XCH, ch = i - r * XCH;
+    const long long m = row0 + r;
+    u32x4 v = {0u, 0u, 0u, 0u};
+    if (m < p.rows) {
+      int b, gy, gx;
+      const long long tr = tail_map_row(p, m, b, gy, gx);
+      if (tr >= 0) v = *reinterpret_cast<const u32x4*>(p.x + tr * p.x_ld + ch * E);
+    }
+    *reinterpret_cast<u32x4*>(tile + r * PA + ch * E) = v;
+  }
+}
+template <typename T, int D, int PA, typename W>
+__device__ __forceinline__ void tail_tile_store_mapped(const TailP<T, W>& p, const T* tile, long long row0, int lane) {
+  constexpr int E = Vec<T>::N, XCH = D / E;
+  for (int i = lane; i < 16 * XCH; i += 64) {
+    const int r = i / XCH, ch = i - r * XCH;
+    const long long m = row0 + r;
+    if (m >= p.rows) continue;
+    int b, gy, gx;
+    const long long tr = tail_map_row(p, m, b, gy, gx);
+    if (tr < 0) continue;
+    bool keep = true;
+    if (p.map.zone_valid)
+      keep = p.map.zone_valid[(long long)b * p.map.zn * p.map.zn + min(max(gy / p.map.p1, 0), p.map.zn - 1) * p.map.zn +
+                              min(max(gx / p.map.p2, 0), p.map.zn - 1)] != 0;
+    float o[E];
+    Vec<T>::load(tile + r * PA + ch * E, o);
+#pragma unroll
+    for (int e = 0; e < E; ++e) o[e] = keep ? o[e] : 0.f;
+    T* dp = p.out + tr * p.out_ld + ch * E;
+    if (p.map.accumulate) {
+      float d[E];
+      Vec<T>::load(dp, d);
+#pragma unroll
+      for (int e = 0; e < E; ++e) o[e] += d[e];
+    }
+    Vec<T>::store(dp, o);
   }
 }
 
@@ -189,6 +249,7 @@
   p.rows = NB * Hq * Wq; p.Hq = Hq; p.Wq = Wq; p.qth = qth; p.qtw = qtw; p.ggy = cdiv(Hq, qth); p.ggx = cdiv(Wq, qtw);
   p.fwq = make_fastdiv((unsigned)Wq); p.fhq = make_fastdiv((unsigned)Hq); p.fqth = make_fastdiv((unsigned)qth); p.fqtw = make_fastdiv((unsigned)qtw);
   p.v_length = v_length; p.eps = eps; p.ln_eps = ln_eps;
+  p.map = TailMap{};
   return p;
 }
 template <typename T, typename W>
diff --git a/cfpnet_amd/engine.py b/cfpnet_amd/engine.py
--- a/cfpnet_amd/engine.py
+++ b/cfpnet_amd/engine.py
@@ -106,6 +106,8 @@
         self.cat_pad = os.environ.get("CFP_CAT_PAD", "1") == "1" and not self.up_fused_x3
         self.lkpm_fused = os.environ.get("CFP_LKPM_FUSED", "1") != "0"
         self.tail_q = os.environ.get("CFP_TAIL_Q", "1") == "1"
+        self.kv_project = os.environ.get("CFP_KV_PROJECT", "1") == "1"
+        self.x2i_inplace = os.environ.get("CFP_X2I_INPLACE", "1") == "1"
         self.lkpm_min_rows = int(os.environ.get("CFP_LKPM_MIN_ROWS", "30000"))
         self.sr_ln_fused = os.environ.get("CFP_SR_LN_FUSED", "1") == "1"
         self.head_fused = os.environ.get("CFP_HEAD_FUSED", "1") != "0"
@@ -462,22 +464,32 @@
 
     def _kv_state(self, plan, tag, p, src: Act, rows_s, D, heads, kvmode: dict):
         d = D // heads
-        kvb = self._act(plan, f"{tag}.kvsrc", rows_s, 2 * D)
-        self._lin(p + ".kv", src, kvb, rows_s)
         G = kvmode["groups"]
         kv = self._f32(plan, f"{tag}.kv", G * heads * d * d)
         ks = self._f32(plan, f"{tag}.ks", G * heads * d)
         nws = ops.attn_kv_ws_floats(kvmode["NB"], kvmode["Hk"], kvmode["Wk"], kvmode["th"], kvmode["tw"], heads, d)
         ws = self._f32(plan, f"{tag}.kvws", nws)
+        if self._kv_projects(kvmode, heads, d):
+            self._kv_project(p, src, kv, ks, ws, kvmode, heads, d)
+            return kv, ks
+        kvb = self._act(plan, f"{tag}.kvsrc", rows_s, 2 * D)
+        self._lin(p + ".kv", src, kvb, rows_s)
         ops.attn_kv_reduce(kvb.slice(0, D), kvb.slice(D, D), kv, ks, ws, kvmode["NB"], kvmode["Hk"], kvmode["Wk"], kvmode["th"], kvmode["tw"],
                            kvmode["clip"], kvmode["count_pad"], kvmode["v_length"], heads, d)
         return kv, ks
+
+    def _kv_projects(self, kvmode: dict, heads, d) -> bool:
+        return (self.kv_project and self.half and not self.weights2
+                and ops.attn_kv_project_fits(kvmode["NB"], kvmode["Hk"], kvmode["Wk"], kvmode["th"], kvmode["tw"], heads, d, self.dtype))
+
+    def _kv_project(self, p, src: Act, kv, ks, ws, kvmode: dict, heads, d):
+        ops.attn_kv_project_reduce(src, self.P[p + ".kv"], kv, ks, ws, kvmode["NB"], kvmode["Hk"], kvmode["Wk"], kvmode["th"], kvmode["tw"],
+                                   kvmode["clip"], kvmode["count_pad"], kvmode["v_length"], heads, d)
 
     def _loftr(self, plan, tag, p, xb: Act, rows_q, src: Optional[Act], rows_s, heads, out: Act, kvmode: dict, apmode: dict, pre=None):
         D = xb.C // 2
         d = D // heads
         x = xb.slice(0, D)
-        qb = self._act(plan, f"{tag}.qkv", rows_q, 3 * D)
         fused_tail = self.half or (self.x3 and os.environ.get("CFP_X3_TAIL", "1") != "0")
         tail_q = fused_tail and self.tail_q
         if pre is not None and tail_q:
@@ -486,7 +498,11 @@
                            (self.P[p + ".norm1.g"], self.P[p + ".norm1.b"]), (self.P[p + ".norm2.g"], self.P[p + ".norm2.b"]),
                            apmode["NB"], apmode["Hq"], apmode["Wq"], apmode["qth"], apmode["qtw"], kvmode["v_length"], heads)
             return
-        if src is None and tail_q:
+        project = tail_q and self._kv_projects(kvmode, heads, d)
+        qb = None if project else self._act(plan, f"{tag}.qkv", rows_q, 3 * D)
+        if project:
+            kA = vA = None
+        elif src is None and tail_q:
             self._lin(p + ".kv", x, qb.slice(D, 2 * D), rows_q)
             kA, vA = qb.slice(D, D), qb.slice(2 * D, D)
         elif src is None:
@@ -503,8 +519,11 @@
         ks = self._f32(plan, f"{tag}.ks", G * heads * d)
         nws = ops.attn_kv_ws_floats(kvmode["NB"], kvmode["Hk"], kvmode["Wk"], kvmode["th"], kvmode["tw"], heads, d)
         ws = self._f32(plan, f"{tag}.kvws", nws)
-        ops.attn_kv_reduce(kA, vA, kv, ks, ws, kvmode["NB"], kvmode["Hk"], kvmode["Wk"], kvmode["th"], kvmode["tw"],
-                           kvmode["clip"], kvmode["count_pad"], kvmode["v_length"], heads, d)
+        if project:
+            self._kv_project(p, x if src is None else src, kv, ks, ws, kvmode, heads, d)
+        else:
+            ops.attn_kv_reduce(kA, vA, kv, ks, ws, kvmode["NB"], kvmode["Hk"], kvmode["Wk"], kvmode["th"], kvmode["tw"],
+                               kvmode["clip"], kvmode["count_pad"], kvmode["v_length"], heads, d)
         if fused_tail:
             ops.loftr_tail(None if tail_q else qb.slice(0, D), kv, ks, x, out, self.P[p + ".q1"] if tail_q else None,
                            self.P[p + ".merge"], self.P[p + ".mlp0"], self.P[p + ".mlp2"],
@@ -518,6 +537,10 @@
         hid = self._act(plan, f"{tag}.hid", rows_q, 2 * D)
         self._lin(p + ".mlp0", xb, hid, rows_q, hip.ACT_RELU)
         self._lin(p + ".mlp2", hid, out, rows_q, residual=x, ln=(self.P[p + ".norm2.g"], self.P[p + ".norm2.b"], 1e-5))
+
+    def _x2i_in_place(self, geo: FusionGeometry, rec) -> bool:
+        return (self.x2i_inplace and self.half and self.tail_q and not geo.interpolate and rec is None
+                and self.change_embedding)
 
     def _piw_ws(self, plan, bi: int, B: int, hw: int, cout: int, k: int):
         if not self.x3:
@@ -571,22 +594,31 @@
             tag = f"{name}.L{i}"
             final_dst = out if (i == last and taps is None and os.environ.get("CFP_NO_DIRECT_OUT", "0") != "1") else None
             if ln == "hist2image":
-                zin = self._act(plan, f"{name}.zin", Mz, 2 * D)
-                zsrc = tok[cur].slice(0, D) if self.change_embedding else emb0
-                if rec is None:
-                    ops.resize_bilinear(zsrc, H, W, rect, zin.slice(0, D), gh, gw, (0, 0, gh, gw), B)
+                x2i_kv = dict(groups=B * Z, NB=B * Z, Hk=1, Wk=N, th=1, tw=N, clip=(0, 1, 0, N), count_pad=False, v_length=float(N))
+                x2i_pre = plan.get("x2i_kv", {}).get((name, i))
+                if self._x2i_in_place(geo, rec):
+                    assert (geo.tzh, geo.tzw) == (gh, gw)
+                    kvs = x2i_pre if x2i_pre is not None else self._kv_state(plan, f"{name}.x2i{i}", l, src, B * Z * N, D, spec.X2I_HEADS, x2i_kv)
+                    ops.loftr_tail_x2i(kvs[0], kvs[1], tok[cur].slice(0, D), H, W, geo.sy_wo, geo.sx_wo, self.P[l + ".q1"], self.P[l + ".merge"],
+                                       self.P[l + ".mlp0"], self.P[l + ".mlp2"], (self.P[l + ".norm1.g"], self.P[l + ".norm1.b"]),
+                                       (self.P[l + ".norm2.g"], self.P[l + ".norm2.b"]), B, gh, gw, geo.p1, geo.p2, zone_valid, geo.zone_num,
+                                       not self.no_skip_inside, float(N), spec.X2I_HEADS)
                 else:
-                    ops.resize_bilinear(zsrc, H, W, None, zin.slice(0, D), gh, gw, (0, 0, gh, gw), B, rec=rec, rec_side=0)
-                zout = self._act(plan, f"{name}.zout", Mz, D)
-                self._loftr(plan, f"{name}.x2i", l, zin, Mz, src, B * Z * N, spec.X2I_HEADS, zout,
-                            dict(groups=B * Z, NB=B * Z, Hk=1, Wk=N, th=1, tw=N, clip=(0, 1, 0, N), count_pad=False, v_length=float(N)),
-                            dict(NB=B, Hq=gh, Wq=gw, qth=geo.p1, qtw=geo.p2), pre=plan.get("x2i_kv", {}).get((name, i)))
-                if rec is None:
-                    ops.resize_bilinear(zout, gh, gw, (0, 0, gh, gw), tok[cur].slice(0, D), H, W, rect, B, zone_valid=zone_valid,
-                                        zn=geo.zone_num, p1=geo.p1, p2=geo.p2, accumulate=not self.no_skip_inside)
-                else:
-                    ops.resize_bilinear(zout, gh, gw, (0, 0, gh, gw), tok[cur].slice(0, D), H, W, None, B, zone_valid=zone_valid,
-                                        zn=geo.zone_num, p1=geo.p1, p2=geo.p2, accumulate=not self.no_skip_inside, rec=rec, rec_side=1)
+                    zin = self._act(plan, f"{name}.zin", Mz, 2 * D)
+                    zsrc = tok[cur].slice(0, D) if self.change_embedding else emb0
+                    if rec is None:
+                        ops.resize_bilinear(zsrc, H, W, rect, zin.slice(0, D), gh, gw, (0, 0, gh, gw), B)
+                    else:
+                        ops.resize_bilinear(zsrc, H, W, None, zin.slice(0, D), gh, gw, (0, 0, gh, gw), B, rec=rec, rec_side=0)
+                    zout = self._act(plan, f"{name}.zout", Mz, D)
+                    self._loftr(plan, f"{name}.x2i", l, zin, Mz, src, B * Z * N, spec.X2I_HEADS, zout, x2i_kv,
+                                dict(NB=B, Hq=gh, Wq=gw, qth=geo.p1, qtw=geo.p2), pre=x2i_pre)
+                    if rec is None:
+                        ops.resize_bilinear(zout, gh, gw, (0, 0, gh, gw), tok[cur].slice(0, D), H, W, rect, B, zone_valid=zone_valid,
+                                            zn=geo.zone_num, p1=geo.p1, p2=geo.p2, accumulate=not self.no_skip_inside)
+                    else:
+                        ops.resize_bilinear(zout, gh, gw, (0, 0, gh, gw), tok[cur].slice(0, D), H, W, None, B, zone_valid=zone_valid,
+                                            zn=geo.zone_num, p1=geo.p1, p2=geo.p2, accumulate=not self.no_skip_inside, rec=rec, rec_side=1)
             elif ln == "image":
                 nh, nw = math.ceil(H / ws), math.ceil(W / ws)
                 self._loftr(plan, f"{name}.lsa", l + ".lga.encoder_layer", tok[cur], M, None, 0, spec.TWINS_HEADS, tok[cur ^ 1].slice(0, D),
diff --git a/cfpnet_amd/hip.py b/cfpnet_amd/hip.py
--- a/cfpnet_amd/hip.py
+++ b/cfpnet_amd/hip.py
@@ -55,9 +55,13 @@
     "cfp_attn_kv_reduce": (_i, [_p, _i, _p, _i, _p, _p, _p] + [_i] * 10 + [_f, _i, _i, _i, _p]),
     "cfp_attn_apply": (_i, [_p, _i, _p, _p, _p, _i] + [_i] * 9 + [_f, _f, _i, _i, _i, _p]),
     "cfp_loftr_tail": (_i, [_p, _i, _p, _p, _p, _i, _p, _i, _p, _p, _p, _p, _p, _p, _p, _p, _f] + [_i] * 5 + [_f, _f, _i, _i, _i, _p]),
+    "cfp_loftr_tail_x2i": (_i, [_p, _p, _p, _i, _i, _i, _i, _i] + [_p] * 8 + [_f] + [_i] * 5 + [_p, _i, _i, _f, _f, _i, _i, _i, _p]),
     "cfp_resize_bilinear": (_i, [_p, _i] + [_i] * 6 + [_p, _i] + [_i] * 6 + [_p] + [_i] * 7 + [_p]),
     "cfp_resize_bilinear_dev": (_i, [_p, _i, _i, _i, _p, _i, _i, _i, _p, _i, _p] + [_i] * 6 + [_i, _p]),
     "cfp_attn_kv_reduce_dev": (_i, [_p, _i, _p, _i, _p, _p, _p] + [_i] * 5 + [_p, _i, _i, _i, _i, _p]),
+    "cfp_attn_kv_project_fits": (_i, [_i] * 8),
+    "cfp_attn_kv_project_reduce": (_i, [_p, _i, _p, _p, _p, _p] + [_i] * 10 + [_f, _i, _i, _i, _p]),
+    "cfp_attn_kv_project_reduce_dev": (_i, [_p, _i, _p, _p, _p, _p] + [_i] * 5 + [_p, _i, _i, _i, _i, _p]),
     "cfp_attn_apply_dev": (_i, [_p, _i, _p, _p, _p, _i] + [_i] * 5 + [_p, _f, _i, _i, _i, _p]),
     "cfp_add_rowtable": (_i, [_p, _i, _p, _p, _i] + [_i] * 8 + [_p]),
     "cfp_upsample_cat_conv3x3": (_i, [_p, _i, _i, _i, _i, _p, _i, _i, _p, _p, _p, _p, _i] + [_i] * 6 + [_p]),
diff --git a/cfpnet_amd/ops.py b/cfpnet_amd/ops.py
--- a/cfpnet_amd/ops.py
+++ b/cfpnet_amd/ops.py
@@ -348,6 +348,21 @@
              NB, Hk, Wk, th, tw, cy0, cy1, cx0, cx1, int(count_pad), float(v_length), heads, d, k.dt, _s())
 
 
+def attn_kv_project_fits(NB, Hk, Wk, th, tw, heads, d, dtype) -> bool:
+    return bool(hip.load().cfp_attn_kv_project_fits(NB, Hk, Wk, th, tw, heads, d, DT.get(dtype, -1)))
+
+
+def attn_kv_project_reduce(x: Act, w_kv: torch.Tensor, kv, ksum, ws, NB, Hk, Wk, th, tw, clip, count_pad, v_length, heads, d, rec=None):
+    assert x.C == heads * d and w_kv.shape == (2 * x.C, x.C) and w_kv.dtype == x.buf.dtype and w_kv.is_contiguous()
+    if rec is not None:
+        hip.call("cfp_attn_kv_project_reduce_dev", x.ptr, x.ld, w_kv.data_ptr(), kv.data_ptr(), ksum.data_ptr(), hip.ptr(ws),
+                 NB, Hk, Wk, th, tw, _rec_ptr(rec), int(count_pad), heads, d, x.dt, _s())
+        return
+    cy0, cy1, cx0, cx1 = clip
+    hip.call("cfp_attn_kv_project_reduce", x.ptr, x.ld, w_kv.data_ptr(), kv.data_ptr(), ksum.data_ptr(), hip.ptr(ws),
+             NB, Hk, Wk, th, tw, cy0, cy1, cx0, cx1, int(count_pad), float(v_length), heads, d, x.dt, _s())
+
+
 def attn_apply(q: Act, kv, ksum, out: Act, NB, Hq, Wq, qth, qtw, excl, v_length, heads, d, eps=1e-6, rec=None):
     if rec is not None:
         hip.call("cfp_attn_apply_dev", q.ptr, q.ld, kv.data_ptr(), ksum.data_ptr(), out.ptr, out.ld,
@@ -373,6 +388,16 @@
              float(ln_eps), NB, Hq, Wq, qth, qtw, float(v_length), float(eps), heads, D, hip.F32X3 if x3 else x.dt, _s())
 
 
+def loftr_tail_x2i(kv, ksum, tok: Act, H, W, sy, sx, w_q, w_merge, w_mlp0, w_mlp2, ln1, ln2, NB, gh, gw, p1, p2, zone_valid, zn, accumulate,
+                   v_length, heads, eps=1e-6, ln_eps=1e-5):
+    D = tok.C
+    assert w_q.shape == (D, D) and w_merge.shape == (D, D) and w_mlp0.shape == (2 * D, 2 * D) and w_mlp2.shape == (D, 2 * D)
+    assert tok.rows >= NB * H * W and (zone_valid is None or (zone_valid.dtype == torch.uint8 and zone_valid.numel() >= NB * zn * zn))
+    hip.call("cfp_loftr_tail_x2i", kv.data_ptr(), ksum.data_ptr(), tok.ptr, tok.ld, H, W, sy, sx, w_q.data_ptr(), w_merge.data_ptr(),
+             w_mlp0.data_ptr(), w_mlp2.data_ptr(), ln1[0].data_ptr(), ln1[1].data_ptr(), ln2[0].data_ptr(), ln2[1].data_ptr(), float(ln_eps),
+             NB, gh, gw, p1, p2, hip.ptr(zone_valid), zn, int(accumulate), float(v_length), float(eps), heads, D, tok.dt, _s())
+
+
 def _rec_ptr(rec) -> int:
     assert rec.dtype == torch.int32 and rec.numel() == 9 and rec.is_cuda and rec.is_contiguous(), "zone record: int32[9] on the device"
     return rec.data_ptr()
diff --git a/include/cfpnet_hip.h b/include/cfpnet_hip.h
--- a/include/cfpnet_hip.h
+++ b/include/cfpnet_hip.h
@@ -118,6 +118,14 @@
                            int NB, int Hk, int Wk, int th, int tw, const int* rec, int count_pad, int heads, int d, int dtype,
                            cfp_stream_t stream);
 
+int cfp_attn_kv_project_fits(int NB, int Hk, int Wk, int th, int tw, int heads, int d, int dtype);
+int cfp_attn_kv_project_reduce(const void* x, int x_ld, const void* w_kv, float* kv, float* ksum, float* ws,
+                               int NB, int Hk, int Wk, int th, int tw, int cy0, int cy1, int cx0, int cx1,
+                               int count_pad, float v_length, int heads, int d, int dtype, cfp_stream_t stream);
+int cfp_attn_kv_project_reduce_dev(const void* x, int x_ld, const void* w_kv, float* kv, float* ksum, float* ws,
+                                   int NB, int Hk, int Wk, int th, int tw, const int* rec, int count_pad, int heads, int d, int dtype,
+                                   cfp_stream_t stream);
+
 int cfp_attn_apply(const void* q, int q_ld, const float* kv, const float* ksum, void* out, int out_ld,
                    int NB, int Hq, int Wq, int qth, int qtw, int ey0, int ey1, int ex0, int ex1,
                    float v_length, float eps, int heads, int d, int dtype, cfp_stream_t stream);
@@ -131,6 +139,12 @@
                    const float* ln1_g, const float* ln1_b, const float* ln2_g, const float* ln2_b, float ln_eps,
                    int NB, int Hq, int Wq, int qth, int qtw, float v_length, float eps, int heads, int D,
                    int dtype, cfp_stream_t stream);
+
+int cfp_loftr_tail_x2i(const float* kv, const float* ksum, void* tok, int tok_ld, int H, int W, int sy, int sx,
+                       const void* w_q, const void* w_merge, const void* w_mlp0, const void* w_mlp2,
+                       const float* ln1_g, const float* ln1_b, const float* ln2_g, const float* ln2_b, float ln_eps,
+                       int NB, int gh, int gw, int p1, int p2, const uint8_t* zone_valid, int zn, int accumulate,
+                       float v_length, float eps, int heads, int D, int dtype, cfp_stream_t stream);
 
 int cfp_resize_bilinear(const void* src, int src_ld, int Hs, int Ws, int sy0, int sx0, int sh, int sw,
                         void* dst, int dst_ld, int Hd, int Wd, int dy0, int dx0, int dh, int dw,
```

Result: faster. 4042 maps/s, median of 6 (+3.7%).
